# prs-eth/PCAccumulation

Hardware: AMD Instinct MI355X
Metric: LiDAR-frames/sec (5-frame seq, 160k pts) fwd+bwd (higher is better)
Workload: dtype mixed

## Files before the change

### include/pcacc.h

```cpp
#ifndef PCACC_H_
#define PCACC_H_

#include <stddef.h>
#include <stdint.h>

#ifdef __cplusplus
extern "C" {
#endif

#define PCACC_OK 0
#define PCACC_E_ARG (-1)
#define PCACC_E_WORKSPACE (-2)
#define PCACC_E_LAUNCH (-3)

#define PCACC_F32 0
#define PCACC_BF16 1

const char *pcacc_target(void);

int pcacc_cat2_rows(const void *a, int32_t a_row_bytes, const void *b, int32_t b_row_bytes, int64_t rows, void *out, void *stream);

int pcacc_reload_switches(void);

int pcacc_voxelize_workspace_bytes(int64_t n, int nx, int ny, int nz, int nt, size_t *bytes );
// ... 204 lines not shown
#define PCACC_ACCUM_TOO_SMALL 1
#define PCACC_ACCUM_BAD_STATE 2
int pcacc_accum_add_workspace_bytes(int64_t n, size_t *bytes );
int pcacc_accum_add(const float *points, int64_t n, const double *pose, const uint8_t *moving, int32_t stamp, double voxel_size,
                    const int64_t *in_keys, const int64_t *in_acc, const int32_t *in_stamps, int64_t in_capacity,
                    int64_t *out_keys, int64_t *out_acc, int32_t *out_stamps, int64_t out_capacity,
                    int64_t *state, void *workspace, size_t workspace_bytes, void *stream);
int pcacc_accum_extract_workspace_bytes(int64_t m, size_t *bytes );
int pcacc_accum_extract(const int64_t *keys, const int64_t *acc, const int32_t *stamps, int64_t capacity, int64_t m, int64_t min_count,
                        int32_t use_fraction, double max_moving_fraction, float *out_points, int32_t *out_coords, int64_t *out_count,
                        int64_t *out_moving, int32_t *out_t_first, int32_t *out_t_last, int64_t *out_n,
                        void *workspace, size_t workspace_bytes, void *stream);

int pcacc_conv3x3_prepare_weights(const float *w, int32_t c_out, int32_t c_in, int32_t kt, int32_t transpose,
                                  uint16_t *out, void *stream);
int pcacc_conv3x3_prepare_weights_pair(const float *w, int32_t c_out, int32_t c_in, int32_t kt, const int64_t *strides ,
                                       uint16_t *out_fwd, uint16_t *out_bwd, void *stream);
int pcacc_conv3x3_bf16(const uint16_t *in, const uint16_t *wp, const float *bias, uint16_t *out, int32_t n_img,
                       int32_t frames, int32_t h, int32_t w, int32_t c_in, int32_t c_out, int32_t kt, int32_t relu,
                       void *stream);
int pcacc_conv3x3_deep_supported(int32_t h, int32_t w, int32_t c_in, int32_t c_out);
int pcacc_conv3x3_deep_bf16(const uint16_t *in, const uint16_t *in_mask, const uint16_t *wp, const float *bias, uint16_t *out, int32_t n_img,
                            int32_t h, int32_t w, int32_t c_in, int32_t c_out, int32_t relu, void *stream);
int pcacc_conv3x3_masked_bf16(const uint16_t *in, const uint16_t *in_mask, const uint16_t *wp, const float *bias, uint16_t *out,
                              int32_t n_img, int32_t frames, int32_t h, int32_t w, int32_t c_in, int32_t c_out, int32_t kt,
                              int32_t relu, void *stream);
int pcacc_conv3x3_outmask_supported(int32_t h, int32_t w, int32_t c_in, int32_t c_out, int32_t kt);
int pcacc_conv3x3_outmask_bf16(const uint16_t *in, const uint16_t *wp, const uint16_t *out_mask, uint16_t *out, int32_t n_img, int32_t frames,
                               int32_t h, int32_t w, int32_t c_in, int32_t c_out, int32_t kt, void *stream);
int pcacc_conv3x3_wgrad_deep_supported(int32_t h, int32_t w, int32_t c_in, int32_t c_out);
int pcacc_conv3x3_wgrad_deep_workspace_bytes(int32_t n_img, int32_t h, int32_t w, int32_t c_in, int32_t c_out, size_t *bytes );
int pcacc_conv3x3_wgrad_deep_bf16(const uint16_t *dy, const uint16_t *dy_mask, const uint16_t *x, float *dw, float *db, int32_t n_img,
                                  int32_t h, int32_t w, int32_t c_in, int32_t c_out, void *workspace, size_t workspace_bytes, void *stream);
int pcacc_absmax256(const float *x, int64_t n, float *parts, void *stream);
int pcacc_conv3x3_split_prepare_weights(const float *w, int32_t c_out, int32_t c_in, int32_t kt, const int64_t *strides ,
                                        uint16_t *out_fwd, float *scale_fwd, uint16_t *out_bwd, float *scale_bwd, void *stream);
int pcacc_conv3x3_split_supported(int32_t h, int32_t w, int32_t c_in, int32_t c_out);
int pcacc_conv3x3_split(const float *in, const float *in_amax, const float *in_mask, const uint16_t *wp, const float *wscale,
                        const float *bias, float *out, float *out_amax, int32_t n_img, int32_t frames, int32_t h, int32_t w, int32_t c_in,
                        int32_t c_out, int32_t kt, int32_t relu, void *stream);
int pcacc_conv3x3_split_dual(const float *in, const float *in_amax, const float *in_mask, const uint16_t *wp, const float *wscale,
                             const float *bias, float *out, float *out_amax, uint16_t *out16, int32_t n_img, int32_t frames, int32_t h,
                             int32_t w, int32_t c_in, int32_t c_out, int32_t kt, int32_t relu, void *stream);

int pcacc_conv3x3_split_cat(const float *in_a, const float *in_b, int32_t c_a, const float *in_amax, const uint16_t *wp, const float *wscale,
                            const float *bias, float *out, float *out_amax, uint16_t *out16, int32_t n_img, int32_t h, int32_t w, int32_t c_in,
                            int32_t c_out, int32_t relu, void *stream);
int pcacc_conv3x3_split_outmask(const float *in, const float *in_amax, const float *in_mask, const uint16_t *wp, const float *wscale,
                                const float *out_mask, float *out, float *out_amax, int32_t n_img, int32_t frames, int32_t h, int32_t w,
                                int32_t c_in, int32_t c_out, int32_t kt, void *stream);
int pcacc_conv3x3_wgrad_split_workspace_bytes(int32_t n_img, int32_t h, int32_t w, int32_t c_in, int32_t c_out, size_t *bytes );
int pcacc_conv3x3_wgrad_split(const float *dy, const float *dy_amax, const float *dy_mask, const float *x, const float *x_amax, float *dw,
                              float *db, int32_t n_img, int32_t frames, int32_t dt, int32_t h, int32_t w, int32_t c_in, int32_t c_out,
                              void *workspace, size_t workspace_bytes, void *stream);
int pcacc_upconv2x2_split_prepare_weights(const float *w, int32_t c_in, int32_t c_up, const int64_t *strides , uint16_t *out_fwd,
                                          float *scale_fwd, uint16_t *out_bwd, float *scale_bwd, void *stream);
int pcacc_upconv2x2_split_supported(int32_t h, int32_t w, int32_t c_in, int32_t c_up);

int pcacc_upconv2x2_bf16_supported(int32_t c_in, int32_t c_up);
int pcacc_upconv2x2_bf16_prepare_weights(const float *w, int32_t c_in, int32_t c_up, const int64_t *strides , uint16_t *out_fwd,
                                         uint16_t *out_bwd, void *stream);
int pcacc_upconv2x2_bf16(const uint16_t *in, const uint16_t *wp, const float *bias, uint16_t *out, int32_t n_img, int32_t h, int32_t w,
                         int32_t c_in, int32_t c_up, int32_t direction, int32_t in_pitch, int32_t out_pitch, void *stream);
int pcacc_upconv2x2_bf16_wgrad_workspace_bytes(int32_t n_img, int32_t h, int32_t w, int32_t c_in, int32_t c_up, size_t *bytes);
int pcacc_upconv2x2_bf16_wgrad(const uint16_t *dy, int32_t dy_pitch, const uint16_t *x, int32_t x_pitch, float *dw, const int64_t *dw_strides ,
                               float *db, int32_t n_img, int32_t h, int32_t w, int32_t c_in, int32_t c_up, void *workspace, size_t workspace_bytes,
                               void *stream);

int pcacc_prepare_weights_batch(const int64_t *jobs, int32_t n_jobs, int32_t total_blocks, void *stream);
int pcacc_upconv2x2_split(const float *in, const float *in_amax, const uint16_t *wp, const float *wscale, const float *bias, float *out,
                          float *out_amax, int32_t n_img, int32_t h, int32_t w, int32_t c_in, int32_t c_up, int32_t direction, void *stream);
int pcacc_upconv2x2_split_dual(const float *in, const float *in_amax, const uint16_t *wp, const float *wscale, const float *bias, float *out,
                               float *out_amax, uint16_t *out16, int32_t n_img, int32_t h, int32_t w, int32_t c_in, int32_t c_up,
                               int32_t out_pitch, void *stream);
int pcacc_upconv2x2_wgrad_split_workspace_bytes(int32_t n_img, int32_t h, int32_t w, int32_t c_in, int32_t c_up, size_t *bytes );
int pcacc_upconv2x2_wgrad_split(const float *dy, const float *dy_amax, const float *x, const float *x_amax, float *dw, float *db4, int32_t n_img,
                                int32_t h, int32_t w, int32_t c_in, int32_t c_up, void *workspace, size_t workspace_bytes, void *stream);
int pcacc_head_conv3x3_supported(int32_t c_in, int32_t c_out);
int pcacc_head_conv3x3_forward(const void *x, int32_t x_dtype, const float *w, const int64_t *w_strides , const float *bias, float *y,
                               int32_t n_img, int32_t h, int32_t wd, int32_t c_in, int32_t c_out, void *stream);
int pcacc_head_conv3x3_dgrad(const float *dy, const float *w, const int64_t *w_strides , void *dx, int32_t dx_dtype, int32_t n_img,
                             int32_t h, int32_t wd, int32_t c_in, int32_t c_out, void *stream);
int pcacc_head_conv3x3_wgrad_workspace_bytes(int32_t n_img, int32_t h, int32_t wd, int32_t c_in, int32_t c_out, size_t *bytes );
int pcacc_head_conv3x3_wgrad(const float *dy, const void *x, int32_t x_dtype, float *dw, float *db, int32_t n_img, int32_t h, int32_t wd,
                             int32_t c_in, int32_t c_out, void *workspace, size_t workspace_bytes, void *stream);
int pcacc_rows_linear_split(const float *x, const float *x_amax, const float *in_mask, const float *w, const float *bias,
                            const float *residual, const float *out_mask, float *y, float *y_amax, int64_t rows, int32_t k, int32_t n,
                            int32_t flags, void *stream);
int pcacc_rows_linear_split_dual(const float *x, const float *x_amax, const float *in_mask, const float *w, const float *bias,
                                 const float *residual, const float *out_mask, float *y, uint16_t *y16, float *y_amax, int64_t rows, int32_t k,
                                 int32_t n, int32_t flags, void *stream);
int pcacc_rows_linear_cat_split(const float *xa, const float *xa_amax, const float *xb, const float *xb_amax, const int32_t *b_index,
                                int32_t ka, const float *in_mask, const float *w, const float *bias, const float *residual,
                                const float *out_mask_a, const float *out_mask_b, float *y, float *y2, int32_t na, float *y_amax, int64_t rows,
                                int32_t k, int32_t n, int32_t flags, void *stream);
int pcacc_rows_wgrad_split_workspace_bytes(int64_t rows, int32_t k, int32_t n, size_t *bytes );
int pcacc_rows_wgrad_split(const float *dy, const float *dy_amax, const float *dy_mask, const float *x, const float *x_amax, int32_t x_relu,
                           int64_t rows, int32_t k, int32_t n, float *dw_aug, void *workspace, size_t workspace_bytes, void *stream);
int pcacc_rows_wgrad_cat_split(const float *dy, const float *dy_amax, const float *dy_mask, const float *xa, const float *xa_amax,
                               const float *xb, const float *xb_amax, const int32_t *b_index, int32_t ka, int32_t x_relu, int64_t rows,
                               int32_t k, int32_t n, float *dw_aug, void *workspace, size_t workspace_bytes, void *stream);
int pcacc_conv3x3_wgrad_workspace_bytes(int32_t n_img, int32_t h, int32_t w, int32_t c_in, int32_t c_out, size_t *bytes );
int pcacc_conv3x3_wgrad_bf16(const uint16_t *dy, const uint16_t *x, float *dw, int32_t n_img, int32_t frames, int32_t dt,
                             int32_t h, int32_t w, int32_t c_in, int32_t c_out, void *workspace, size_t workspace_bytes,
                             void *stream);

int pcacc_prep_points(const double *points, const double *tsfm12, const double *noise, double noise_scale, double scale,
                      double crop_xy, double z_min, double z_max, int32_t remove_ground, double ground_z, int64_t m,
                      double *out_points, uint8_t *keep, void *stream);

int pcacc_seg_loss_workspace_bytes(int64_t n, size_t *bytes );
int pcacc_seg_loss_forward(const void *logits, int logits_dtype, int64_t plane, const int64_t *labels, const int64_t *rows,
                           int64_t n, float *out_loss, double *out_metric, float *lovasz_grad, float *saved,
                           void *workspace, size_t workspace_bytes, void *stream);
int pcacc_seg_loss_backward(const void *logits, int logits_dtype, int64_t plane, const int64_t *labels, const int64_t *rows,
                            int64_t n, int64_t n_total, const float *lovasz_grad, const float *saved, const float *grad_bce,
                            const float *grad_lovasz, void *grad_logits, void *stream);

int pcacc_offset_loss_workspace_bytes(int64_t m, int64_t k, size_t *bytes );
int pcacc_offset_loss_forward(const float *points, const int64_t *time_indice, const int64_t *inst_labels,
                              const int64_t *label_base, const float *ego_motion, const float *inst_motion, int32_t n_frames,
                              int64_t n, int64_t k, const float *transformed_points, const float *offset_est,
                              const int64_t *rows, int64_t m, float *out, float *offset_gt, void *workspace,
                              size_t workspace_bytes, void *stream);
int pcacc_offset_loss_backward(const float *offset_gt, const float *offset_est, const int64_t *rows, int64_t m, int64_t n,
                               const float *grad_norm, const float *grad_dir, float *grad_est, void *stream);

int pcacc_frames_max(const void *x, int dtype, int64_t n_seq, int32_t frames, int64_t plane, void *out, uint8_t *arg, void *stream);
int pcacc_frames_max_backward(const void *grad_out, const uint8_t *arg, int dtype, int64_t n_seq, int32_t frames, int64_t plane,
                              void *grad_x, void *stream);

int pcacc_bn_rows_workspace_bytes(int64_t rows, int32_t c, size_t *bytes );
int pcacc_bn_rows_forward(const void *x, int dtype, int64_t rows, int32_t c, const float *gamma, const float *beta, float eps,
                          float momentum, float *running_mean, float *running_var, void *y, float *save_mean,
                          float *save_invstd, void *workspace, size_t workspace_bytes, void *stream);
int pcacc_bn_rows_backward(const void *grad_y, const void *x, int dtype, int64_t rows, int32_t c, const float *gamma,
                           const float *save_mean, const float *save_invstd, void *grad_x, float *grad_gamma, float *grad_beta,
                           void *workspace, size_t workspace_bytes, void *stream);

int pcacc_bn_relu_rows_forward(const void *x, int dtype, int64_t rows, int32_t c, const float *gamma, const float *beta, float eps,
                               float momentum, float *running_mean, float *running_var, void *y, float *save_mean, float *save_invstd,
                               void *workspace, size_t workspace_bytes, void *stream);
int pcacc_bn_relu_rows_backward(const void *grad_y, const void *x, int dtype, int64_t rows, int32_t c, const float *gamma, const float *beta,
                                const float *save_mean, const float *save_invstd, void *grad_x, float *grad_gamma, float *grad_beta,
                                void *workspace, size_t workspace_bytes, void *stream);
int pcacc_bn_rows_forward_dual(const float *x, int64_t rows, int32_t c, const float *gamma, const float *beta, float eps, float momentum,
                               float *running_mean, float *running_var, int32_t relu, float *y, uint16_t *y16, float *y_amax, float *save_mean,
                               float *save_invstd, void *workspace, size_t workspace_bytes, void *stream);

int pcacc_bn_rows_backward_m(const void *grad_y, const void *x, int dtype, int64_t rows, int32_t c, const float *gamma, const float *beta,
                             int32_t relu, const float *save_mean, const float *save_invstd, void *grad_x, float *grad_x_amax, float *grad_gamma,
                             float *grad_beta, void *workspace, size_t workspace_bytes, void *stream);

int pcacc_pfn_block_forward(const uint16_t *xa, const uint16_t *pooled, const int32_t *p2v, const float *w0, const float *b0,
                            const float *ws, const float *w1, const float *b1, uint16_t *out, uint16_t *relu_h, int64_t rows, void *stream);
int pcacc_pfn_block_backward_workspace_bytes(int64_t rows, size_t *bytes );
int pcacc_pfn_block_backward(const uint16_t *xa, const uint16_t *pooled, const int32_t *p2v, const uint16_t *relu_h,
                             const uint16_t *grad_out, const float *w0, const float *ws, const float *w1, uint16_t *grad_xa,
                             uint16_t *grad_xb, float *grad_params, int64_t rows, void *workspace, size_t workspace_bytes, void *stream);

int pcacc_pfn_block_split_forward(const float *xa, const float *xa_amax, const float *pooled, const float *pooled_amax, const int32_t *p2v,
                                  const float *w0, const float *b0, const float *ws, const float *w1, const float *b1, float *out,
                                  float *relu_h, uint64_t *xmask, uint32_t *hmask, float *out_amax, float *hr_amax, int64_t rows,
                                  void *stream);
int pcacc_pfn_block_split_forward_dual(const float *xa, const float *xa_amax, const float *pooled, const float *pooled_amax, const int32_t *p2v,
                                       const float *w0, const float *b0, const float *ws, const float *w1, const float *b1, float *out,
                                       uint16_t *out16, uint16_t *hr16, float *out_amax, int64_t rows, void *stream);
int pcacc_pfn_block_split_dgrad(const float *grad_out, const float *grad_out_amax, const uint64_t *xmask, const uint32_t *hmask,
                                const float *w0, const float *ws, const float *w1, float *grad_xa, float *grad_xb, float *grad_h,
                                float *gx_amax, float *dh_amax, int64_t rows, void *stream);

int pcacc_maxpool2x2_bf16(const uint16_t *x, int64_t n_img, int32_t h, int32_t w, int32_t c, uint16_t *out, void *stream);
int pcacc_pool_skip_relu_backward_bf16(const uint16_t *y, const uint16_t *grad_pooled, const uint16_t *grad_skip, int64_t n_img, int32_t h,
                                       int32_t w, int32_t c, uint16_t *grad_y, void *stream);
int pcacc_maxpool2x2_f32(const float *x, int64_t n_img, int32_t h, int32_t w, int32_t c, float *out, void *stream);
int pcacc_pool_skip_relu_backward_f32(const float *y, const float *grad_pooled, const float *grad_skip, int64_t n_img, int32_t h, int32_t w,
                                      int32_t c, float *grad_y, float *out_amax, void *stream);
int pcacc_pool_skip_relu_backward_strided_bf16(const uint16_t *y, const uint16_t *grad_pooled, const uint16_t *grad_skip, int64_t skip_pitch,
                                               int64_t n_img, int32_t h, int32_t w, int32_t c, uint16_t *grad_y, void *stream);
int pcacc_pool_skip_relu_backward_strided_f32(const float *y, const float *grad_pooled, const float *grad_skip, int64_t skip_pitch,
                                              int64_t n_img, int32_t h, int32_t w, int32_t c, float *grad_y, float *out_amax, void *stream);
int pcacc_pool_skip_relu_backward_strided_y32(const float *y, const uint16_t *grad_pooled, const uint16_t *grad_skip, int64_t skip_pitch,
                                              int64_t n_img, int32_t h, int32_t w, int32_t c, uint16_t *grad_y, void *stream);

int pcacc_inv4x4(const float *m, int64_t n, float *out, void *stream);

int pcacc_rows_wgrad_few_supported(int32_t k, int32_t n);
int pcacc_rows_wgrad_few_workspace_bytes(int64_t rows, int32_t k, int32_t n, size_t *bytes );
int pcacc_rows_wgrad_few(const void *dy, const void *dy_mask, const void *x, int32_t x_relu, int64_t rows, int32_t k, int32_t n,
                         float *dw_aug, int32_t dtypes, void *workspace, size_t workspace_bytes, void *stream);

int pcacc_tube_rows(const float *xyz, const int32_t *slot, const float *slot_centre, int64_t n, int32_t n_frames, float *rows, void *stream);
int pcacc_tube_code(const float *geo, const float *motion, const float *frame, int64_t n_inst, int32_t n_frames, int32_t c, float *code,
                    void *stream);
int pcacc_tube_code_backward(const float *grad_code, int64_t n_inst, int32_t n_frames, int32_t c, float *grad_geo, float *grad_motion,
                             float *grad_frame, void *stream);
int pcacc_tube_pose_forward(const float *pose_vec, const float *remaining, const float *total_in, const float *slot_centre,
                            const float *weights, int32_t n_slots, int32_t n_frames, float *pose_c, float *gt_c, float *step,
                            float *remaining_out, float *total_out, double *loss_rt, float *wsum, void *stream);
int pcacc_tube_gap_forward(const float *rows, const int32_t *slot, const float *pose_c, const float *gt_c, int64_t n, float *pp, void *stream);
int pcacc_tube_finish(const float *slot_sums, int32_t stride, const float *count, const float *weights, const float *wsum, int32_t n_slots,
                      float *l12, void *stream);
int pcacc_tube_gap_backward(const float *rows, const int32_t *slot, const float *pose_c, const float *gt_c, const float *weights,
                            const float *count, const float *wsum, const float *grad_l1, const float *grad_l2, int64_t n,
                            float *grad_rows16, void *stream);
int pcacc_tube_pose_backward(const float *pose_vec, const float *remaining, const float *slot_centre, const float *weights, const float *wsum,
                             const float *grad_pose, int32_t stride, const double *grad_rot, const double *grad_trans, int32_t n_slots,
                             int32_t n_frames, float *grad_vec, void *stream);

int pcacc_upload_words(const uint32_t *host_words, int64_t n, uint32_t *dst, void *stream);

#ifdef __cplusplus
}
#endif
#endif
```

### pcaccumulation_amd/csrc/bn.hip

```cpp
#include "common.h"

#define BN_MAX_C 256

template <bool BF>
__device__ __forceinline__ void bn_load(const void *p, int64_t vec_index, float (&v)[BF ? 8 : 4])
{
    if (BF) {
        const uint4 r = reinterpret_cast<const uint4 *>(p)[vec_index];
        v[0] = pcacc_bf16_lo(r.x), v[1] = pcacc_bf16_hi(r.x), v[2] = pcacc_bf16_lo(r.y), v[3] = pcacc_bf16_hi(r.y);
        v[(BF ? 8 : 4) - 4] = pcacc_bf16_lo(r.z), v[(BF ? 8 : 4) - 3] = pcacc_bf16_hi(r.z);
        v[(BF ? 8 : 4) - 2] = pcacc_bf16_lo(r.w), v[(BF ? 8 : 4) - 1] = pcacc_bf16_hi(r.w);
    } else {
        const float4 r = reinterpret_cast<const float4 *>(p)[vec_index];
        v[0] = r.x, v[1] = r.y, v[2] = r.z, v[3] = r.w;
    }
}

template <bool BF>
__device__ __forceinline__ void bn_store(void *p, int64_t vec_index, const float (&v)[BF ? 8 : 4])
{
    if (BF)
        reinterpret_cast<uint4 *>(p)[vec_index] = make_uint4(pcacc_pack_bf16x2(v[0], v[1]), pcacc_pack_bf16x2(v[2], v[3]),
                                                             pcacc_pack_bf16x2(v[(BF ? 8 : 4) - 4], v[(BF ? 8 : 4) - 3]),
                                                             pcacc_pack_bf16x2(v[(BF ? 8 : 4) - 2], v[(BF ? 8 : 4) - 1]));
// ... 142 lines not shown
        rsh[k] = ((relu && relu_beta) ? relu_beta[sub * V + k] : 0.f) - mean[sub * V + k] * is_[k] * g;
    }
    for (int64_t e = (int64_t)blockIdx.x * 256 + threadIdx.x; e < total; e += (int64_t)gridDim.x * 256) {
        float x[V], o[V];
        bn_load<BF>(X, e, x);
        if (!DY) {
#pragma unroll
            for (int k = 0; k < V; ++k) o[k] = x[k] * scale[k] + shift[k];
            if (relu) {
#pragma unroll
                for (int k = 0; k < V; ++k) o[k] = fmaxf(o[k], 0.f);
            }
        } else {
            float g[V];
            bn_load<BF>(DY, e, g);
            if (relu) {
#pragma unroll
                for (int k = 0; k < V; ++k) g[k] = (x[k] * rsc[k] + rsh[k] > 0.f) ? g[k] : 0.f;
            }
#pragma unroll
            for (int k = 0; k < V; ++k) o[k] = g[k] * scale[k] + (x[k] * is_[k] - mis[k]) * kx[k] + shift[k];
        }
        bn_store<BF>(out, e, o);
        if (!BF && out16) reinterpret_cast<uint2 *>(out16)[e] = make_uint2(pcacc_pack_bf16x2(o[0], o[1]), pcacc_pack_bf16x2(o[2], o[3]));
        if (out_amax) {
#pragma unroll
            for (int k = 0; k < V; ++k) {
                omax = fmaxf(omax, fabsf(o[k]));
                if (o[k] != o[k]) omax = __builtin_inff();
            }
        }
    }
    if (out_amax) {
#pragma unroll
        for (int d = 32; d >= 1; d >>= 1) omax = fmaxf(omax, __shfl_xor(omax, d, 64));
        if ((threadIdx.x & 63) == 0) atomicMax(reinterpret_cast<unsigned *>(out_amax) + ((blockIdx.x * 4 + (threadIdx.x >> 6)) & 255), __float_as_uint(omax));
    }
}

static int bn_blocks(int64_t rows, int c, int v)
{
    const int rows_per_pass = 256 / (c / v);
    int64_t nb = (rows + (int64_t)rows_per_pass * 8 - 1) / ((int64_t)rows_per_pass * 8);
    if (nb > PCACC_CUS * 4) nb = PCACC_CUS * 4;
    return nb < 1 ? 1 : (int)nb;
}

static int bn_args(int dtype, int64_t rows, int c)
{
    if (dtype != PCACC_F32 && dtype != PCACC_BF16) return PCACC_E_ARG;
    const int v = dtype == PCACC_BF16 ? 8 : 4;
    if (rows < 1 || c < v || c > BN_MAX_C || c % v || 256 % (c / v)) return PCACC_E_ARG;
    return PCACC_OK;
}

extern "C" int pcacc_bn_rows_workspace_bytes(int64_t rows, int32_t c, size_t *bytes)
{
    if (!bytes || rows < 1 || c < 4 || c > BN_MAX_C) return PCACC_E_ARG;
    *bytes = (size_t)PCACC_CUS * 4 * 2 * c * sizeof(float);
    return PCACC_OK;
}

static int bn_forward_any(const void *x, int dtype, int64_t rows, int32_t c, const float *gamma, const float *beta, float eps,
                          float momentum, float *running_mean, float *running_var, void *y, float *save_mean,
                          float *save_invstd, void *workspace, size_t workspace_bytes, void *stream, bool relu, uint16_t *y16 = nullptr,
                          float *y_amax = nullptr)
{
    if ((y16 || y_amax) && dtype != PCACC_F32) return PCACC_E_ARG;
    if (bn_args(dtype, rows, c) != PCACC_OK || !x || !y || !save_mean || !save_invstd || !workspace) return PCACC_E_ARG;
    const bool bf = dtype == PCACC_BF16;
    const int nb = bn_blocks(rows, c, bf ? 8 : 4);
    if (workspace_bytes < (size_t)nb * 2 * c * sizeof(float)) return PCACC_E_WORKSPACE;
    hipStream_t s = pcacc_stream(stream);
    float *partial = reinterpret_cast<float *>(workspace);
    if (bf) bn_sums_kernel<true><<<nb, 256, 0, s>>>(x, nullptr, nullptr, nullptr, rows, c, partial);
    else bn_sums_kernel<false><<<nb, 256, 0, s>>>(x, nullptr, nullptr, nullptr, rows, c, partial);
    bn_finalize_fwd_kernel<<<c, 256, 0, s>>>(partial, nb, c, rows, eps, momentum, running_mean, running_var, save_mean, save_invstd);
    const int grid = pcacc_grid(rows * (c / (bf ? 8 : 4)), 256, PCACC_CUS * 16);
    if (bf) bn_apply_kernel<true><<<grid, 256, 0, s>>>(x, nullptr, save_mean, save_invstd, gamma, beta, nullptr, rows, c, y, relu);
    else bn_apply_kernel<false><<<grid, 256, 0, s>>>(x, nullptr, save_mean, save_invstd, gamma, beta, nullptr, rows, c, y, relu, nullptr, y_amax, y16);
    PCACC_CHECK_LAUNCH();
    return PCACC_OK;
}

extern "C" int pcacc_bn_rows_forward_dual(const float *x, int64_t rows, int32_t c, const float *gamma, const float *beta, float eps, float momentum,
                                          float *running_mean, float *running_var, int32_t relu, float *y, uint16_t *y16, float *y_amax,
                                          float *save_mean, float *save_invstd, void *workspace, size_t workspace_bytes, void *stream)
{
    return bn_forward_any(x, PCACC_F32, rows, c, gamma, beta, eps, momentum, running_mean, running_var, y, save_mean, save_invstd, workspace,
                          workspace_bytes, stream, relu != 0, y16, y_amax);
}

extern "C" int pcacc_bn_rows_forward(const void *x, int dtype, int64_t rows, int32_t c, const float *gamma, const float *beta, float eps,
                                     float momentum, float *running_mean, float *running_var, void *y, float *save_mean,
                                     float *save_invstd, void *workspace, size_t workspace_bytes, void *stream)
{
    return bn_forward_any(x, dtype, rows, c, gamma, beta, eps, momentum, running_mean, running_var, y, save_mean, save_invstd, workspace,
                          workspace_bytes, stream, false);
}

extern "C" int pcacc_bn_relu_rows_forward(const void *x, int dtype, int64_t rows, int32_t c, const float *gamma, const float *beta, float eps,
                                          float momentum, float *running_mean, float *running_var, void *y, float *save_mean,
                                          float *save_invstd, void *workspace, size_t workspace_bytes, void *stream)
{
    return bn_forward_any(x, dtype, rows, c, gamma, beta, eps, momentum, running_mean, running_var, y, save_mean, save_invstd, workspace,
                          workspace_bytes, stream, true);
}

static int bn_backward_any(const void *grad_y, const void *x, int dtype, int64_t rows, int32_t c, const float *gamma,
                           const float *save_mean, const float *save_invstd, void *grad_x, float *grad_gamma, float *grad_beta,
                           void *workspace, size_t workspace_bytes, void *stream, bool relu, const float *beta, float *grad_x_amax = nullptr)
{
    if (bn_args(dtype, rows, c) != PCACC_OK || !grad_y || !x || !save_mean || !save_invstd || !grad_x || !grad_gamma || !grad_beta || !workspace)
        return PCACC_E_ARG;
    const bool bf = dtype == PCACC_BF16;
    const int nb = bn_blocks(rows, c, bf ? 8 : 4);
    if (workspace_bytes < (size_t)nb * 2 * c * sizeof(float)) return PCACC_E_WORKSPACE;
    hipStream_t s = pcacc_stream(stream);
    float *partial = reinterpret_cast<float *>(workspace);
    if (bf) bn_sums_kernel<true><<<nb, 256, 0, s>>>(grad_y, x, save_mean, save_invstd, rows, c, partial, relu, gamma, beta);
    else bn_sums_kernel<false><<<nb, 256, 0, s>>>(grad_y, x, save_mean, save_invstd, rows, c, partial, relu, gamma, beta);
    bn_finalize_bwd_kernel<<<c, 256, 0, s>>>(partial, nb, c, grad_beta, grad_gamma);
    const int grid = pcacc_grid(rows * (c / (bf ? 8 : 4)), 256, PCACC_CUS * 16);
    if (bf) bn_apply_kernel<true><<<grid, 256, 0, s>>>(x, grad_y, save_mean, save_invstd, gamma, grad_beta, grad_gamma, rows, c, grad_x, relu, beta, grad_x_amax);
    else bn_apply_kernel<false><<<grid, 256, 0, s>>>(x, grad_y, save_mean, save_invstd, gamma, grad_beta, grad_gamma, rows, c, grad_x, relu, beta, grad_x_amax);
    PCACC_CHECK_LAUNCH();
    return PCACC_OK;
}

extern "C" int pcacc_bn_rows_backward_m(const void *grad_y, const void *x, int dtype, int64_t rows, int32_t c, const float *gamma, const float *beta,
                                        int32_t relu, const float *save_mean, const float *save_invstd, void *grad_x, float *grad_x_amax,
                                        float *grad_gamma, float *grad_beta, void *workspace, size_t workspace_bytes, void *stream)
{
    if (!grad_x_amax) return PCACC_E_ARG;
    return bn_backward_any(grad_y, x, dtype, rows, c, gamma, save_mean, save_invstd, grad_x, grad_gamma, grad_beta, workspace, workspace_bytes, stream,
                           relu != 0, relu ? beta : nullptr, grad_x_amax);
}

extern "C" int pcacc_bn_rows_backward(const void *grad_y, const void *x, int dtype, int64_t rows, int32_t c, const float *gamma,
                                      const float *save_mean, const float *save_invstd, void *grad_x, float *grad_gamma, float *grad_beta,
                                      void *workspace, size_t workspace_bytes, void *stream)
{
    return bn_backward_any(grad_y, x, dtype, rows, c, gamma, save_mean, save_invstd, grad_x, grad_gamma, grad_beta, workspace, workspace_bytes, stream,
                           false, nullptr);
}

extern "C" int pcacc_bn_relu_rows_backward(const void *grad_y, const void *x, int dtype, int64_t rows, int32_t c, const float *gamma,
                                           const float *beta, const float *save_mean, const float *save_invstd, void *grad_x, float *grad_gamma,
                                           float *grad_beta, void *workspace, size_t workspace_bytes, void *stream)
{
    return bn_backward_any(grad_y, x, dtype, rows, c, gamma, save_mean, save_invstd, grad_x, grad_gamma, grad_beta, workspace, workspace_bytes, stream,
                           true, beta);
}
```

### pcaccumulation_amd/csrc/canvas.hip

```cpp
#include <hip/hip_ext.h>

#include "scan.h"

template <typename T>
__global__ __launch_bounds__(256) void cell_index_kernel(const T *__restrict__ coords, int64_t m, int nx, int ny, int nt,
                                                         int64_t n_cells, int32_t *__restrict__ cell, int32_t *cell2pillar)
{
    for (int64_t i = (int64_t)blockIdx.x * 256 + threadIdx.x; i < m; i += (int64_t)gridDim.x * 256) {
        const int64_t b = (int64_t)coords[i * 5 + 0];
        const int64_t y = (int64_t)coords[i * 5 + 2];
        const int64_t x = (int64_t)coords[i * 5 + 3];
        const int64_t t = (int64_t)coords[i * 5 + 4];
        const int64_t c = ((b * nt + t) * ny + y) * nx + x;
        const bool ok = c >= 0 && c < n_cells && x >= 0 && x < nx && y >= 0 && y < ny && t >= 0 && t < nt;
        cell[i] = ok ? (int32_t)c : -1;
        if (ok) atomicMax(&cell2pillar[c], (int32_t)i);
    }
}

extern "C" int pcacc_cell_index(const void *coords, int coords_is_f64, int64_t m, int nx, int ny, int nt, int n_batch,
                                int32_t *cell, int32_t *cell2pillar, void *stream)
{
    if (m < 0 || nx <= 0 || ny <= 0 || nt <= 0 || n_batch <= 0 || !cell2pillar) return PCACC_E_ARG;
    const int64_t n_cells = (int64_t)n_batch * nt * ny * nx;
// ... 247 lines not shown
}

template <int OUT_BF16>
__global__ __launch_bounds__(256) void pillar_scatter_scalar(const float *__restrict__ feats, const int32_t *__restrict__ c2p,
                                                             int64_t n_elems, int c, void *__restrict__ canvas)
{
    for (int64_t e = (int64_t)blockIdx.x * 256 + threadIdx.x; e < n_elems; e += (int64_t)gridDim.x * 256) {
        const int64_t cell = e / c;
        const int k = (int)(e - cell * c);
        const int p = c2p[cell];
        const float v = (p >= 0) ? feats[(int64_t)p * c + k] : 0.f;
        if (OUT_BF16) static_cast<uint16_t *>(canvas)[e] = f32_to_bf16(v);
        else static_cast<float *>(canvas)[e] = v;
    }
}

static int pillar_scatter_launch(const void *feats, int feats_dtype, const int32_t *cell2pillar, int64_t n_cells, int c, void *canvas,
                                 int dtype, hipEvent_t start, hipEvent_t stop, hipStream_t s)
{
    if (n_cells < 0 || c <= 0 || !cell2pillar || !canvas || (dtype != PCACC_F32 && dtype != PCACC_BF16)) return PCACC_E_ARG;
    if (feats_dtype != PCACC_F32 && !(feats_dtype == PCACC_BF16 && dtype == PCACC_BF16 && c % 8 == 0)) return PCACC_E_ARG;
    if (n_cells == 0) return PCACC_OK;
    int64_t n;
    int width, per_lane = 1;
    const void *fn;
    if (feats_dtype == PCACC_BF16) {
        width = c / 8;
        n = n_cells * width;
        fn = reinterpret_cast<const void *>(pillar_scatter_rows16_k<1, true>);
        per_lane = 1;
        switch (pcacc_switches().scatter_variant) {
        case '0': fn = reinterpret_cast<const void *>(pillar_scatter_rows16); per_lane = 2; break;
        case '1': fn = reinterpret_cast<const void *>(pillar_scatter_rows16_k<4, true>); per_lane = 4; break;
        case '2': fn = reinterpret_cast<const void *>(pillar_scatter_rows16_k<2, true>); per_lane = 2; break;
        case '3': fn = reinterpret_cast<const void *>(pillar_scatter_rows16_k<4, false>); per_lane = 4; break;
        case '4': fn = reinterpret_cast<const void *>(pillar_scatter_rows16_k<8, true>); per_lane = 8; break;
        case '5': fn = reinterpret_cast<const void *>(pillar_scatter_rows16_k<1, true>); per_lane = 1; break;
        case '6': fn = reinterpret_cast<const void *>(pillar_scatter_rows16_k<1, true, false>); per_lane = 1; break;
        case '7': fn = reinterpret_cast<const void *>(pillar_scatter_rows16_k<2, true, false>); per_lane = 2; break;
        default: break;
        }
    } else if (dtype == PCACC_F32 ? (c % 4 == 0) : (c % 8 == 0)) {
        width = c / 4;
        n = dtype == PCACC_F32 ? n_cells * width : n_cells * (width / 2);
        fn = dtype == PCACC_F32 ? reinterpret_cast<const void *>(pillar_scatter_vec4<0>) : reinterpret_cast<const void *>(pillar_scatter_vec4<1>);
        if (dtype == PCACC_F32 && pcacc_switches().scatter_variant == 'f')
            fn = reinterpret_cast<const void *>(pillar_scatter_f32_nt);
    } else {
        width = c;
        n = n_cells * c;
        fn = dtype == PCACC_F32 ? reinterpret_cast<const void *>(pillar_scatter_scalar<0>) : reinterpret_cast<const void *>(pillar_scatter_scalar<1>);
    }
    void *args[] = {(void *)&feats, (void *)&cell2pillar, (void *)&n, (void *)&width, (void *)&canvas};
    const int64_t items = (n + per_lane - 1) / per_lane;
    const int blocks_per_cu = pcacc_switches().scatter_blocks > 0 ? pcacc_switches().scatter_blocks : 8;
    if (hipExtLaunchKernel(fn, dim3(pcacc_grid(items, 256, PCACC_CUS * blocks_per_cu)), dim3(256), args, 0, s, start, stop, 0) != hipSuccess) return PCACC_E_LAUNCH;
    PCACC_CHECK_LAUNCH();
    return PCACC_OK;
}

extern "C" int pcacc_pillar_scatter(const float *feats, const int32_t *cell2pillar, int64_t n_cells, int c,
                                    void *canvas, int dtype, void *stream)
{
    return pillar_scatter_launch(feats, PCACC_F32, cell2pillar, n_cells, c, canvas, dtype, nullptr, nullptr, pcacc_stream(stream));
}

extern "C" int pcacc_pillar_scatter_timed(const float *feats, const int32_t *cell2pillar, int64_t n_cells, int c, void *canvas, int dtype,
                                          void *start_event, void *stop_event, void *stream)
{
    if (!start_event || !stop_event) return PCACC_E_ARG;
    return pillar_scatter_launch(feats, PCACC_F32, cell2pillar, n_cells, c, canvas, dtype, reinterpret_cast<hipEvent_t>(start_event),
                                 reinterpret_cast<hipEvent_t>(stop_event), pcacc_stream(stream));
}

extern "C" int pcacc_pillar_scatter_t(const void *feats, int feats_dtype, const int32_t *cell2pillar, int64_t n_cells, int c, void *canvas,
                                      int dtype, void *start_event, void *stop_event, void *stream)
{
    if ((start_event == nullptr) != (stop_event == nullptr)) return PCACC_E_ARG;
    return pillar_scatter_launch(feats, feats_dtype, cell2pillar, n_cells, c, canvas, dtype, reinterpret_cast<hipEvent_t>(start_event),
                                 reinterpret_cast<hipEvent_t>(stop_event), pcacc_stream(stream));
}

extern "C" int pcacc_timer_create(void **start_event, void **stop_event)
{
    if (!start_event || !stop_event) return PCACC_E_ARG;
    hipEvent_t a, b;
    if (hipEventCreate(&a) != hipSuccess) return PCACC_E_LAUNCH;
    if (hipEventCreate(&b) != hipSuccess) { (void)hipEventDestroy(a); return PCACC_E_LAUNCH; }
    *start_event = a;
    *stop_event = b;
    return PCACC_OK;
}

extern "C" int pcacc_timer_elapsed_us(void *start_event, void *stop_event, float *us)
{
    if (!start_event || !stop_event || !us) return PCACC_E_ARG;
    float ms = 0.f;
    if (hipEventElapsedTime(&ms, reinterpret_cast<hipEvent_t>(start_event), reinterpret_cast<hipEvent_t>(stop_event)) != hipSuccess)
        return PCACC_E_LAUNCH;
    *us = ms * 1e3f;
    return PCACC_OK;
}

extern "C" int pcacc_timer_destroy(void *start_event, void *stop_event)
{
    if (start_event) (void)hipEventDestroy(reinterpret_cast<hipEvent_t>(start_event));
    if (stop_event) (void)hipEventDestroy(reinterpret_cast<hipEvent_t>(stop_event));
    return PCACC_OK;
}

__global__ __launch_bounds__(256) void gather_rows_kernel(const uint32_t *__restrict__ src, int words, const int32_t *__restrict__ idx,
                                                          int64_t n_idx, uint32_t *__restrict__ out)
{
    const int64_t total = n_idx * words;
    for (int64_t e = (int64_t)blockIdx.x * 256 + threadIdx.x; e < total; e += (int64_t)gridDim.x * 256) {
        const int64_t r = e / words;
        const int k = (int)(e - r * words);
        const int64_t j = idx[r];
        out[e] = (j >= 0) ? src[j * words + k] : 0u;
    }
}

__global__ __launch_bounds__(256) void gather_rows_kernel16(const uint4 *__restrict__ src, int pieces, const int32_t *__restrict__ idx,
                                                            int64_t n_idx, uint4 *__restrict__ out)
{
    const int64_t total = n_idx * pieces;
    for (int64_t e = (int64_t)blockIdx.x * 256 + threadIdx.x; e < total; e += (int64_t)gridDim.x * 256) {
        const int64_t r = e / pieces;
        const int k = (int)(e - r * pieces);
        const int64_t j = idx[r];
        out[e] = (j >= 0) ? src[j * pieces + k] : make_uint4(0u, 0u, 0u, 0u);
    }
}

extern "C" int pcacc_gather_rows(const void *src, int row_bytes, const int32_t *idx, int64_t n_idx, void *out, void *stream)
{
    if (n_idx < 0 || row_bytes <= 0 || (row_bytes % 4)) return PCACC_E_ARG;
    if (n_idx > 0 && (!src || !idx || !out)) return PCACC_E_ARG;
    if (n_idx == 0) return PCACC_OK;
    hipStream_t s = pcacc_stream(stream);
    if (row_bytes % 16 == 0 && (reinterpret_cast<uintptr_t>(src) % 16 == 0) && (reinterpret_cast<uintptr_t>(out) % 16 == 0)) {
        const int pieces = row_bytes / 16;
        gather_rows_kernel16<<<pcacc_grid(n_idx * pieces, 256), 256, 0, s>>>(static_cast<const uint4 *>(src), pieces, idx, n_idx,
                                                                            static_cast<uint4 *>(out));
    } else {
        const int words = row_bytes / 4;
        gather_rows_kernel<<<pcacc_grid(n_idx * words, 256), 256, 0, s>>>(static_cast<const uint32_t *>(src), words, idx, n_idx,
                                                                         static_cast<uint32_t *>(out));
    }
    PCACC_CHECK_LAUNCH();
    return PCACC_OK;
}

__global__ __launch_bounds__(256) void cat2_rows_kernel(const uint4 *__restrict__ a, int pa, const uint4 *__restrict__ b, int pb, int64_t rows,
                                                        uint4 *__restrict__ out)
{
    const int pr = pa + pb;
    const int64_t total = rows * pr, stride = (int64_t)gridDim.x * 256;
    for (int64_t e = (int64_t)blockIdx.x * 256 + threadIdx.x; e < total; e += 2 * stride) {
        const int64_t e2 = e + stride;
        const int64_t r0 = e / pr, r1 = e2 / pr;
        const int c0 = (int)(e - r0 * pr), c1 = (int)(e2 - r1 * pr);
        const uint4 v0 = c0 < pa ? a[r0 * pa + c0] : b[r0 * pb + (c0 - pa)];
        uint4 v1 = make_uint4(0, 0, 0, 0);
        if (e2 < total) v1 = c1 < pa ? a[r1 * pa + c1] : b[r1 * pb + (c1 - pa)];
        out[e] = v0;
        if (e2 < total) out[e2] = v1;
    }
}

extern "C" int pcacc_cat2_rows(const void *a, int32_t a_row_bytes, const void *b, int32_t b_row_bytes, int64_t rows, void *out, void *stream)
{
    if (rows < 0 || a_row_bytes <= 0 || b_row_bytes <= 0 || (a_row_bytes % 16) || (b_row_bytes % 16)) return PCACC_E_ARG;
    if (rows == 0) return PCACC_OK;
    if (!a || !b || !out || (reinterpret_cast<uintptr_t>(a) % 16) || (reinterpret_cast<uintptr_t>(b) % 16) || (reinterpret_cast<uintptr_t>(out) % 16)) return PCACC_E_ARG;
    const int pa = a_row_bytes / 16, pb = b_row_bytes / 16;
    const int64_t total = rows * (pa + pb);
    cat2_rows_kernel<<<pcacc_grid((total + 1) / 2, 256, PCACC_CUS * 16), 256, 0, pcacc_stream(stream)>>>(static_cast<const uint4 *>(a), pa, static_cast<const uint4 *>(b), pb,
                                                                                                         rows, static_cast<uint4 *>(out));
    PCACC_CHECK_LAUNCH();
    return PCACC_OK;
}

extern "C" const char *pcacc_target(void) { return "gfx950"; }

static PcaccSwitches g_switches;
static bool g_switches_read = false;

static void switches_read()
{
    const char *e = getenv("PCACC_CONV_RES");
    g_switches.conv_frame_major = getenv("PCACC_CONV_FRAME_MAJOR") != nullptr;
    g_switches.conv_swz_off = getenv("PCACC_CONV_SWZ_OFF") != nullptr;
    g_switches.rows_fm_off = getenv("PCACC_ROWS_FM_OFF") != nullptr;
    g_switches.conv_plan = getenv("PCACC_CONV_PLAN") != nullptr;
    g_switches.conv_res = e ? e[0] : 0;
    const char *xr = getenv("PCACC_XCD_REMAP");
    g_switches.xcd_off = xr && xr[0] == '0';
    const char *v = getenv("PCACC_SCATTER_VARIANT");
    g_switches.scatter_variant = v ? v[0] : 0;
    const char *b = getenv("PCACC_SCATTER_BLOCKS");
    g_switches.scatter_blocks = b ? atoi(b) : 0;
    g_switches_read = true;
}

const PcaccSwitches &pcacc_switches()
{
    if (!g_switches_read) switches_read();
    return g_switches;
}

extern "C" int pcacc_reload_switches(void)
{
    switches_read();
    return 0;
}

struct UploadWords { uint32_t w[240]; };

__global__ void upload_words_kernel(UploadWords words, int n, uint32_t *dst)
{
    if ((int)threadIdx.x < n) dst[threadIdx.x] = words.w[threadIdx.x];
}

extern "C" int pcacc_upload_words(const uint32_t *host_words, int64_t n, uint32_t *dst, void *stream)
{
    if (n < 0 || (n > 0 && (!host_words || !dst))) return PCACC_E_ARG;
    for (int64_t off = 0; off < n; off += 240) {
        UploadWords words;
        const int m = (int)((n - off) < 240 ? (n - off) : 240);
        for (int i = 0; i < m; ++i) words.w[i] = host_words[off + i];
        upload_words_kernel<<<1, 256, 0, pcacc_stream(stream)>>>(words, m, dst + off);
    }
    PCACC_CHECK_LAUNCH();
    return PCACC_OK;
}

__global__ __launch_bounds__(256) void prep_points_kernel(const double *__restrict__ pts, const double *__restrict__ tsfm,
                                                          const double *__restrict__ noise, double noise_scale, double scale,
                                                          double crop_xy, double z_min, double z_max, int remove_ground, double ground_z,
                                                          int64_t m, double *__restrict__ out, uint8_t *__restrict__ keep)
{
#pragma clang fp contract(off)
    for (int64_t i = (int64_t)blockIdx.x * 256 + threadIdx.x; i < m; i += (int64_t)gridDim.x * 256) {
        double x = pts[3 * i], y = pts[3 * i + 1], z = pts[3 * i + 2];
        if (tsfm) {
            const double nx = fma(tsfm[2], z, fma(tsfm[1], y, tsfm[0] * x)) + tsfm[9];
            const double ny = fma(tsfm[5], z, fma(tsfm[4], y, tsfm[3] * x)) + tsfm[10];
            const double nz = fma(tsfm[8], z, fma(tsfm[7], y, tsfm[6] * x)) + tsfm[11];
            x = nx; y = ny; z = nz;
        }
        if (noise) {
            x = x + (noise[3 * i] - 0.5) * noise_scale;
            y = y + (noise[3 * i + 1] - 0.5) * noise_scale;
            z = z + (noise[3 * i + 2] - 0.5) * noise_scale;
        }
        if (tsfm || noise) { x = x * scale; y = y * scale; z = z * scale; }
        out[3 * i] = x; out[3 * i + 1] = y; out[3 * i + 2] = z;
        bool k = fabs(x) < crop_xy && fabs(y) < crop_xy && z < z_max && z > z_min;
        if (remove_ground) k = k && z > ground_z;
        keep[i] = k ? 1 : 0;
    }
}

extern "C" int pcacc_prep_points(const double *points, const double *tsfm12, const double *noise, double noise_scale, double scale,
                                 double crop_xy, double z_min, double z_max, int32_t remove_ground, double ground_z, int64_t m,
                                 double *out_points, uint8_t *keep, void *stream)
{
    if (m < 0) return PCACC_E_ARG;
    if (m == 0) return PCACC_OK;
    if (!points || !out_points || !keep) return PCACC_E_ARG;
    prep_points_kernel<<<pcacc_grid(m, 256), 256, 0, pcacc_stream(stream)>>>(points, tsfm12, noise, noise_scale, scale, crop_xy, z_min,
                                                                            z_max, remove_ground, ground_z, m, out_points, keep);
    PCACC_CHECK_LAUNCH();
    return PCACC_OK;
}

template <bool BF>
__global__ __launch_bounds__(256) void frames_max_kernel(const void *__restrict__ x, int64_t n_seq, int frames, int64_t plane_vec,
                                                         void *__restrict__ out, uint8_t *__restrict__ arg)
{
    constexpr int V = BF ? 8 : 4;
    const int64_t total = n_seq * plane_vec;
    for (int64_t e = (int64_t)blockIdx.x * 256 + threadIdx.x; e < total; e += (int64_t)gridDim.x * 256) {
        const int64_t s = e / plane_vec, p = e - s * plane_vec;
        float best[V];
        uint8_t who[V];
        for (int t = 0; t < frames; ++t) {
            const uint4 raw = reinterpret_cast<const uint4 *>(x)[(s * frames + t) * plane_vec + p];
            float v[V];
            if (BF) {
                v[0] = pcacc_bf16_lo(raw.x), v[1] = pcacc_bf16_hi(raw.x), v[2] = pcacc_bf16_lo(raw.y), v[3] = pcacc_bf16_hi(raw.y);
                v[V - 4] = pcacc_bf16_lo(raw.z), v[V - 3] = pcacc_bf16_hi(raw.z), v[V - 2] = pcacc_bf16_lo(raw.w), v[V - 1] = pcacc_bf16_hi(raw.w);
            } else {
                v[0] = __uint_as_float(raw.x), v[1] = __uint_as_float(raw.y), v[2] = __uint_as_float(raw.z), v[3] = __uint_as_float(raw.w);
            }
#pragma unroll
            for (int k = 0; k < V; ++k) {
                const bool take = t == 0 || v[k] > best[k] || (v[k] != v[k] && best[k] == best[k]);
                best[k] = take ? v[k] : best[k];
                who[k] = take ? (uint8_t)t : who[k];
            }
        }
        if (BF) {
            reinterpret_cast<uint4 *>(out)[e] = make_uint4(pcacc_pack_bf16x2(best[0], best[1]), pcacc_pack_bf16x2(best[2], best[3]),
                                                           pcacc_pack_bf16x2(best[V - 4], best[V - 3]), pcacc_pack_bf16x2(best[V - 2], best[V - 1]));
// ... 77 lines not shown
```

### pcaccumulation_amd/csrc/common.h

```cpp
#pragma once
#include <hip/hip_runtime.h>
#include <stdint.h>

#include "../../include/pcacc.h"

#define PCACC_WAVE 64
#define PCACC_CUS 256

#define PCACC_CHECK_LAUNCH()                                   \
    do {                                                       \
        if (hipGetLastError() != hipSuccess) return PCACC_E_LAUNCH; \
    } while (0)

struct PcaccSwitches {
    bool conv_frame_major;
    bool conv_swz_off;
    bool rows_fm_off;
    bool conv_plan;
    char conv_res;
    bool xcd_off;
    char scatter_variant;
    int scatter_blocks;
};
const PcaccSwitches &pcacc_switches();

static inline hipStream_t pcacc_stream(void *s) { return reinterpret_cast<hipStream_t>(s); }

static inline int pcacc_grid(int64_t work_items, int block, int max_blocks = PCACC_CUS * 8)
{
    int64_t b = (work_items + block - 1) / block;
    if (b < 1) b = 1;
    if (b > max_blocks) b = max_blocks;
    return (int)b;
}

static inline size_t pcacc_align(size_t x, size_t a = 256) { return (x + a - 1) / a * a; }

__device__ __forceinline__ int pcacc_xcd_block(int b, int n)
{
    const int per = (n + 7) >> 3, rem = n & 7, x = b & 7, i = b >> 3;
    return (rem == 0 || x < rem) ? x * per + i : rem * per + (x - rem) * (per - 1) + i;
}

__device__ __forceinline__ float bf16_to_f32(uint16_t h) { return __uint_as_float(((uint32_t)h) << 16); }
__device__ __forceinline__ uint16_t f32_to_bf16(float f)
{
    uint32_t u = __float_as_uint(f);
    if ((u & 0x7fffffffu) > 0x7f800000u) return (uint16_t)((u >> 16) | 0x40);
    u += 0x7fffu + ((u >> 16) & 1u);
    return (uint16_t)(u >> 16);
}

typedef __bf16 pcacc_bf16x2 __attribute__((ext_vector_type(2)));
typedef float pcacc_f32x2 __attribute__((ext_vector_type(2)));
__device__ __forceinline__ uint32_t pcacc_pack_bf16x2(float lo, float hi)
{
    const pcacc_f32x2 f = {lo, hi};
    const pcacc_bf16x2 r = __builtin_convertvector(f, pcacc_bf16x2);
    return *reinterpret_cast<const uint32_t *>(&r);
}
__device__ __forceinline__ float pcacc_bf16_lo(uint32_t v) { return __uint_as_float(v << 16); }
__device__ __forceinline__ float pcacc_bf16_hi(uint32_t v) { return __uint_as_float(v & 0xffff0000u); }
__device__ __forceinline__ float4 pcacc_ld4(const void *p, bool bf16, int64_t i4)
{
    if (!bf16) return reinterpret_cast<const float4 *>(p)[i4];
    const uint2 v = reinterpret_cast<const uint2 *>(p)[i4];
    return make_float4(pcacc_bf16_lo(v.x), pcacc_bf16_hi(v.x), pcacc_bf16_lo(v.y), pcacc_bf16_hi(v.y));
}
__device__ __forceinline__ void pcacc_st4(void *p, bool bf16, int64_t i4, float4 v)
{
    if (!bf16) reinterpret_cast<float4 *>(p)[i4] = v;
    else reinterpret_cast<uint2 *>(p)[i4] = make_uint2(pcacc_pack_bf16x2(v.x, v.y), pcacc_pack_bf16x2(v.z, v.w));
}

__device__ __forceinline__ uint32_t pcacc_relu_mask2(uint32_t g, uint32_t y)
{
    const uint32_t lo = ((int32_t)(y << 16) > 0) ? 0x0000ffffu : 0u;
    const uint32_t hi = ((int32_t)(y & 0xffff0000u) > 0) ? 0xffff0000u : 0u;
    return g & (lo | hi);
}
__device__ __forceinline__ uint4 pcacc_relu_mask8(uint4 g, uint4 y)
{
    return make_uint4(pcacc_relu_mask2(g.x, y.x), pcacc_relu_mask2(g.y, y.y), pcacc_relu_mask2(g.z, y.z), pcacc_relu_mask2(g.w, y.w));
}

__host__ __device__ constexpr int pcacc_tr_stride(int c)
{
    return c == 32 ? 32 : (c == 64 ? 96 : (c == 96 ? 96 : (c == 128 ? 160 : c + 4)));
}

#ifdef PCACC_X3_EXPERIMENT
__device__ __forceinline__ float pcacc_x_round_bf16(float v) { return bf16_to_f32(f32_to_bf16(v)); }
__device__ __forceinline__ bool pcacc_x_apply(int f, float &a, float &b)
{
    if (f & 4) { a = pcacc_x_round_bf16(a); b = pcacc_x_round_bf16(b); }
    return (f & 5) != 0;
}
#define PCACC_X_ACT(word) ((word) & 5)
#define PCACC_X_W(word) (((word) >> 1) & 5)
#endif

__device__ __forceinline__ int lane_id() { return threadIdx.x & 63; }

template <int EL, class Store>
__device__ __forceinline__ void pcacc_reduce_partials(const float *__restrict__ partial, int n_parts, int elems, Store store)
{
    constexpr int SL = 1024 / EL;
    __shared__ float red[SL][EL + 1];
    const int el = threadIdx.x % EL, slice = threadIdx.x / EL;
    const int e = blockIdx.x * EL + el;
    float s0 = 0.f, s1 = 0.f, s2 = 0.f, s3 = 0.f;
    if (e < elems) {
        int p = slice;
        for (; p + 3 * SL < n_parts; p += 4 * SL) {
            s0 += partial[(int64_t)p * elems + e];
            s1 += partial[(int64_t)(p + SL) * elems + e];
            s2 += partial[(int64_t)(p + 2 * SL) * elems + e];
            s3 += partial[(int64_t)(p + 3 * SL) * elems + e];
        }
        for (; p < n_parts; p += SL) s0 += partial[(int64_t)p * elems + e];
    }
    red[slice][el] = (s0 + s1) + (s2 + s3);
    __syncthreads();
    if (slice == 0 && e < elems) {
        float v = 0.f;
#pragma unroll 8
        for (int k = 0; k < SL; ++k) v += red[k][el];
        store(e, v);
    }
}
static inline int pcacc_reduce_el(int elems) { return elems >= 8192 ? 64 : 16; }

__device__ __forceinline__ int wave_inclusive_scan(int v)
{
#pragma unroll
    for (int d = 1; d < 64; d <<= 1) {
        int t = __shfl_up(v, d, 64);
        if (lane_id() >= d) v += t;
    }
    return v;
}

__device__ __forceinline__ int block256_exclusive_scan(int v, int *lds, int *total)
{
    const int incl = wave_inclusive_scan(v);
    const int w = threadIdx.x >> 6;
    if (lane_id() == 63) lds[w] = incl;
    __syncthreads();
    int base = 0;
#pragma unroll
    for (int i = 0; i < 4; ++i) base += (i < w) ? lds[i] : 0;
    *total = lds[0] + lds[1] + lds[2] + lds[3];
    __syncthreads();
    return base + incl - v;
}

struct ConvTile { int img, fr, y0, x0; };
#define PCACC_WALK_OK(n_img, frames, tiles_y, tiles_x) ((n_img) < (1 << 24) && (frames) < 128 && (tiles_y) < 32768 && (tiles_x) < 65536)
struct ConvTileWalk {
    int first, stride, count;
    int tyx, tiles_x, frames, frame_fastest, th, tw;
    int v_if, v_yx;
    __device__ __forceinline__ void init(int lo, int hi, int slot, int slots, int tiles_y, int tiles_x_, int frames_, int ff, int th_, int tw_)
    {
        first = lo + slot; stride = slots; count = first < hi ? (hi - first + slots - 1) / slots : 0;
        tyx = tiles_y * tiles_x_; tiles_x = tiles_x_; frames = frames_; frame_fastest = ff; th = th_; tw = tw_;
        v_if = v_yx = 0;
    }
    __device__ __forceinline__ void refill(int k0)
    {
        const int t = first + (k0 + (int)(threadIdx.x & 63)) * stride;
        int img, pos, fr;
        if (frame_fastest) {
            const int q = t / frames, smp = q / tyx;
            fr = t - q * frames; pos = q - smp * tyx; img = smp * frames + fr;
        } else {
            img = t / tyx; pos = t - img * tyx; fr = frames > 1 ? img % frames : 0;
        }
        const int ty = pos / tiles_x;
// ... 13 lines not shown
```

### pcaccumulation_amd/csrc/head_conv.hip

```cpp
#include <type_traits>
#include "common.h"

#define HC_THREADS 256
#define HC_MAXCO 4

__device__ __forceinline__ float4 hc_ld4(const void *p, int bf16, int64_t i4) { return pcacc_ld4(p, bf16 != 0, i4); }

#define HC_TR 8
#define HC_TC 32
#define HC_PW (HC_TC + 2)
#define HC_PH (HC_TR + 2)

struct HcTile { int img, y0, x0; };
__device__ __forceinline__ HcTile hc_tile(int t, int tiles_y, int tiles_x)
{
    const int per_img = tiles_y * tiles_x, img = t / per_img, r = t - img * per_img;
    return HcTile{img, (r / tiles_x) * HC_TR, (r % tiles_x) * HC_TC};
}

template <int CI>
__device__ __forceinline__ void hc_stage(const void *__restrict__ x, int x_bf16, const HcTile &t, int h, int wd, float *patch)
{
    constexpr int LPP = CI / 4;
    for (int e = threadIdx.x; e < HC_PH * HC_PW * LPP; e += HC_THREADS) {
        const int pp = e / LPP, l4 = e - pp * LPP;
        const int py = pp / HC_PW, pxx = pp - py * HC_PW;
        const int y = t.y0 - 1 + py, xx = t.x0 - 1 + pxx;
        const bool ok = (unsigned)y < (unsigned)h && (unsigned)xx < (unsigned)wd;
        const int yc = min(max(y, 0), h - 1), xc = min(max(xx, 0), wd - 1);
        float4 v = hc_ld4(x, x_bf16, (((int64_t)t.img * h + yc) * wd + xc) * LPP + l4);
        if (!ok) v = make_float4(0.f, 0.f, 0.f, 0.f);
        *reinterpret_cast<float4 *>(patch + pp * CI + l4 * 4) = v;
    }
}

template <int CI, bool BF> struct HcRaw { typedef typename std::conditional<BF, uint2, float4>::type T; };
template <int CI> struct HcPieces { static constexpr int N = (HC_PH * HC_PW * (CI / 4) + HC_THREADS - 1) / HC_THREADS; };

template <int CI, bool BF>
__device__ __forceinline__ void hc_fetch(const void *__restrict__ x, const HcTile &t, int h, int wd, typename HcRaw<CI, BF>::T (&r)[HcPieces<CI>::N])
{
    constexpr int LPP = CI / 4;
    const typename HcRaw<CI, BF>::T *src = static_cast<const typename HcRaw<CI, BF>::T *>(x);
#pragma unroll
    for (int q = 0; q < HcPieces<CI>::N; ++q) {
        const int e = min((int)threadIdx.x + q * HC_THREADS, HC_PH * HC_PW * LPP - 1);
        const int pp = e / LPP, l4 = e - pp * LPP;
        const int py = pp / HC_PW, pxx = pp - py * HC_PW;
        const int yc = min(max(t.y0 - 1 + py, 0), h - 1), xc = min(max(t.x0 - 1 + pxx, 0), wd - 1);
        r[q] = src[(((int64_t)t.img * h + yc) * wd + xc) * LPP + l4];
    }
}

template <int CI, bool BF>
__device__ __forceinline__ void hc_put(const typename HcRaw<CI, BF>::T (&r)[HcPieces<CI>::N], const HcTile &t, int h, int wd, float *patch)
{
    constexpr int LPP = CI / 4;
#pragma unroll
    for (int q = 0; q < HcPieces<CI>::N; ++q) {
        const int e = threadIdx.x + q * HC_THREADS;
        if (e >= HC_PH * HC_PW * LPP) break;
        const int pp = e / LPP, l4 = e - pp * LPP;
        const int py = pp / HC_PW, pxx = pp - py * HC_PW;
        const int y = t.y0 - 1 + py, xx = t.x0 - 1 + pxx;
        const bool ok = (unsigned)y < (unsigned)h && (unsigned)xx < (unsigned)wd;
        float4 v;
        if constexpr (BF) v = make_float4(pcacc_bf16_lo(r[q].x), pcacc_bf16_hi(r[q].x), pcacc_bf16_lo(r[q].y), pcacc_bf16_hi(r[q].y));
        else v = r[q];
        if (!ok) v = make_float4(0.f, 0.f, 0.f, 0.f);
        *reinterpret_cast<float4 *>(patch + pp * CI + l4 * 4) = v;
    }
}

template <int CI, int COM, bool BF>
__global__ __launch_bounds__(HC_THREADS) void head_conv_fwd_kernel(const void *__restrict__ x, int x_bf16, const float *__restrict__ w,
                                                                   const float *__restrict__ bias, float *__restrict__ y, int n_img, int h,
                                                                   int wd, int co, int64_t ws_o, int64_t ws_i, int64_t ws_y, int64_t ws_x,
                                                                   int tiles_y, int tiles_x)
{
    constexpr int LPP = CI / 4, PPB = HC_THREADS / LPP;
    extern __shared__ __attribute__((aligned(16))) float hc_lds[];
    float *patch = hc_lds;
    const int l = threadIdx.x % LPP, slot = threadIdx.x / LPP;
    float4 wr[9][COM];
#pragma unroll
    for (int tap = 0; tap < 9; ++tap)
#pragma unroll
        for (int c = 0; c < COM; ++c) {
            const float *wp = w + c * ws_o + (4 * l) * ws_i + (tap / 3) * ws_y + (tap % 3) * ws_x;
            wr[tap][c] = c < co ? make_float4(wp[0], wp[ws_i], wp[2 * ws_i], wp[3 * ws_i]) : make_float4(0.f, 0.f, 0.f, 0.f);
        }
    const int n_tiles = n_img * tiles_y * tiles_x;
    constexpr bool PIPE = CI == 32;
    typename HcRaw<CI, BF>::T raw[HcPieces<CI>::N];
    if (PIPE && (int)blockIdx.x < n_tiles) hc_fetch<CI, BF>(x, hc_tile(blockIdx.x, tiles_y, tiles_x), h, wd, raw);
    for (int t = blockIdx.x; t < n_tiles; t += gridDim.x) {
        const HcTile tl = hc_tile(t, tiles_y, tiles_x);
        __syncthreads();
        if constexpr (PIPE) hc_put<CI, BF>(raw, tl, h, wd, patch); else hc_stage<CI>(x, x_bf16, tl, h, wd, patch);
        __syncthreads();
        if (PIPE && t + (int)gridDim.x < n_tiles) hc_fetch<CI, BF>(x, hc_tile(t + gridDim.x, tiles_y, tiles_x), h, wd, raw);
        for (int q = slot; q < HC_TR * HC_TC; q += PPB) {
            const int row = q / HC_TC, col = q % HC_TC;
            float acc[COM];
#pragma unroll
            for (int c = 0; c < COM; ++c) acc[c] = 0.f;
#pragma unroll
            for (int tap = 0; tap < 9; ++tap) {
                const float4 v = *reinterpret_cast<const float4 *>(patch + ((row + tap / 3) * HC_PW + col + tap % 3) * CI + 4 * l);
#pragma unroll
                for (int c = 0; c < COM; ++c) acc[c] += v.x * wr[tap][c].x + v.y * wr[tap][c].y + v.z * wr[tap][c].z + v.w * wr[tap][c].w;
            }
#pragma unroll
            for (int d = 1; d < LPP; d <<= 1)
#pragma unroll
                for (int c = 0; c < COM; ++c) acc[c] += __shfl_xor(acc[c], d, 64);
            const int yy = tl.y0 + row, xx = tl.x0 + col;
            if (l < co && yy < h && xx < wd) {
                float r = acc[0];
#pragma unroll
                for (int c = 1; c < COM; ++c) r = l == c ? acc[c] : r;
                y[(((int64_t)tl.img * h + yy) * wd + xx) * co + l] = r + (bias ? bias[l] : 0.f);
            }
        }
    }
}

template <int CI, int COM>
__global__ __launch_bounds__(HC_THREADS) void head_conv_dgrad_kernel(const float *__restrict__ dy, const float *__restrict__ w, void *__restrict__ dx,
                                                                     int dx_bf16, int n_img, int h, int wd, int co, int64_t ws_o, int64_t ws_i,
                                                                     int64_t ws_y, int64_t ws_x, int tiles_y, int tiles_x)
{
    constexpr int LPP = CI / 4, PPB = HC_THREADS / LPP;
    __shared__ float gp[HC_PH * HC_PW * COM];
    const int l = threadIdx.x % LPP, slot = threadIdx.x / LPP;
    float4 wr[9][COM];
#pragma unroll
    for (int tap = 0; tap < 9; ++tap)
#pragma unroll
        for (int c = 0; c < COM; ++c) {
            const float *wp = w + c * ws_o + (4 * l) * ws_i + (tap / 3) * ws_y + (tap % 3) * ws_x;
            wr[tap][c] = c < co ? make_float4(wp[0], wp[ws_i], wp[2 * ws_i], wp[3 * ws_i]) : make_float4(0.f, 0.f, 0.f, 0.f);
        }
    const int n_tiles = n_img * tiles_y * tiles_x;
    for (int t = blockIdx.x; t < n_tiles; t += gridDim.x) {
        const HcTile tl = hc_tile(t, tiles_y, tiles_x);
        __syncthreads();
        for (int e = threadIdx.x; e < HC_PH * HC_PW * COM; e += HC_THREADS) {
            const int pp = e / COM, c = e - pp * COM;
            const int py = pp / HC_PW, pxx = pp - py * HC_PW;
            const int y = tl.y0 - 1 + py, xx = tl.x0 - 1 + pxx;
            const bool ok = (unsigned)y < (unsigned)h && (unsigned)xx < (unsigned)wd && c < co;
            const int yc = min(max(y, 0), h - 1), xc = min(max(xx, 0), wd - 1);
            const float v = dy[(((int64_t)tl.img * h + yc) * wd + xc) * co + (c < co ? c : 0)];
            gp[e] = ok ? v : 0.f;
        }
        __syncthreads();
        for (int q = slot; q < HC_TR * HC_TC; q += PPB) {
            const int row = q / HC_TC, col = q % HC_TC;
            const int yy = tl.y0 + row, xx = tl.x0 + col;
            float4 acc = make_float4(0.f, 0.f, 0.f, 0.f);
#pragma unroll
            for (int tap = 0; tap < 9; ++tap) {
                const float *g = gp + ((row + 2 - tap / 3) * HC_PW + col + 2 - tap % 3) * COM;
#pragma unroll
                for (int c = 0; c < COM; ++c) {
                    const float gv = g[c];
                    acc.x += gv * wr[tap][c].x; acc.y += gv * wr[tap][c].y; acc.z += gv * wr[tap][c].z; acc.w += gv * wr[tap][c].w;
                }
            }
            if (yy < h && xx < wd) pcacc_st4(dx, dx_bf16 != 0, (((int64_t)tl.img * h + yy) * wd + xx) * LPP + l, acc);
        }
    }
}

template <int CI, int COM, bool BF>
__global__ __launch_bounds__(HC_THREADS) void head_conv_wgrad_kernel(const float *__restrict__ dy, const void *__restrict__ x, int x_bf16,
                                                                     float *__restrict__ partial, int n_img, int h, int wd, int co, int tiles_y,
                                                                     int tiles_x)
{
    constexpr int LPP = CI / 4, PPB = HC_THREADS / LPP;
    extern __shared__ __attribute__((aligned(16))) float hc_lds[];
    float *patch = hc_lds;
    constexpr int RED = 9 * COM * 4 + COM;
    static_assert(4 * LPP * RED <= HC_PH * HC_PW * CI, "reduction scratch fits the patch");
    const int l = threadIdx.x % LPP, slot = threadIdx.x / LPP, wave = threadIdx.x >> 6;
    float acc[9][COM][4], bs[COM];
#pragma unroll
    for (int c = 0; c < COM; ++c) bs[c] = 0.f;
#pragma unroll
    for (int t = 0; t < 9; ++t)
#pragma unroll
        for (int c = 0; c < COM; ++c)
#pragma unroll
            for (int q = 0; q < 4; ++q) acc[t][c][q] = 0.f;
    const int n_tiles = n_img * tiles_y * tiles_x;
    constexpr bool PIPE = CI == 32 && COM == 4;
    typename HcRaw<CI, BF>::T raw[HcPieces<CI>::N];
    if (PIPE && (int)blockIdx.x < n_tiles) hc_fetch<CI, BF>(x, hc_tile(blockIdx.x, tiles_y, tiles_x), h, wd, raw);
    for (int t = blockIdx.x; t < n_tiles; t += gridDim.x) {
        const HcTile tl = hc_tile(t, tiles_y, tiles_x);
        __syncthreads();
        if constexpr (PIPE) hc_put<CI, BF>(raw, tl, h, wd, patch); else hc_stage<CI>(x, x_bf16, tl, h, wd, patch);
        __syncthreads();
        if (PIPE && t + (int)gridDim.x < n_tiles) hc_fetch<CI, BF>(x, hc_tile(t + gridDim.x, tiles_y, tiles_x), h, wd, raw);
        auto dy_at = [&](int q) {
            const int yy = tl.y0 + q / HC_TC, xx = tl.x0 + q % HC_TC;
            return dy + (((int64_t)tl.img * h + min(yy, h - 1)) * wd + min(xx, wd - 1)) * co;
        };
#ifndef HC_DY_AHEAD
#define HC_DY_AHEAD 0
#endif
        constexpr bool AHEAD = COM == 2 && HC_DY_AHEAD;
        float2 g_next = make_float2(0.f, 0.f);
        if (AHEAD && co == 2) g_next = *reinterpret_cast<const float2 *>(dy_at(slot));
        for (int q = slot; q < HC_TR * HC_TC; q += PPB) {
            const int row = q / HC_TC, col = q % HC_TC;
            const int yy = tl.y0 + row, xx = tl.x0 + col;
            const bool ok = yy < h && xx < wd;
            const float *gp = dy_at(q);
            float g[COM];
            if (AHEAD && co == 2) {
                const float2 g2 = g_next;
                if (q + PPB < HC_TR * HC_TC) g_next = *reinterpret_cast<const float2 *>(dy_at(q + PPB));
                g[0] = ok ? g2.x : 0.f;
                g[1] = ok ? g2.y : 0.f;
            } else {
#pragma unroll
                for (int c = 0; c < COM; ++c) g[c] = (c < co && ok) ? gp[c < co ? c : 0] : 0.f;
            }
#pragma unroll
            for (int c = 0; c < COM; ++c) bs[c] += g[c];
#pragma unroll
            for (int tap = 0; tap < 9; ++tap) {
                const float4 v = *reinterpret_cast<const float4 *>(patch + ((row + tap / 3) * HC_PW + col + tap % 3) * CI + 4 * l);
#pragma unroll
                for (int c = 0; c < COM; ++c) {
                    acc[tap][c][0] += g[c] * v.x; acc[tap][c][1] += g[c] * v.y; acc[tap][c][2] += g[c] * v.z; acc[tap][c][3] += g[c] * v.w;
                }
            }
        }
    }
#pragma unroll
    for (int d = LPP; d < 64; d <<= 1) {
#pragma unroll
        for (int t = 0; t < 9; ++t)
#pragma unroll
            for (int c = 0; c < COM; ++c)
#pragma unroll
                for (int q = 0; q < 4; ++q) acc[t][c][q] += __shfl_xor(acc[t][c][q], d, 64);
#pragma unroll
        for (int c = 0; c < COM; ++c) bs[c] += __shfl_xor(bs[c], d, 64);
    }
    __syncthreads();
    float *red = patch;
    if ((threadIdx.x & 63) < LPP) {
        float *r = red + (wave * LPP + l) * RED;
#pragma unroll
        for (int t = 0; t < 9; ++t)
#pragma unroll
            for (int c = 0; c < COM; ++c)
#pragma unroll
                for (int q = 0; q < 4; ++q) r[(t * COM + c) * 4 + q] = acc[t][c][q];
#pragma unroll
        for (int c = 0; c < COM; ++c) r[9 * COM * 4 + c] = bs[c];
    }
    __syncthreads();
    float *mine = partial + (int64_t)blockIdx.x * (co * CI * 9 + co);
    for (int e = threadIdx.x; e < co * CI * 9; e += HC_THREADS) {
        const int tap = e % 9, ci = (e / 9) % CI, c = e / (9 * CI);
        float s = 0.f;
#pragma unroll
        for (int wv = 0; wv < HC_THREADS / 64; ++wv) s += red[(wv * LPP + ci / 4) * RED + (tap * COM + c) * 4 + (ci & 3)];
        mine[e] = s;
    }
    if (threadIdx.x < co) {
        float s = 0.f;
#pragma unroll
        for (int wv = 0; wv < HC_THREADS / 64; ++wv) s += red[(wv * LPP) * RED + 9 * COM * 4 + threadIdx.x];
        mine[co * CI * 9 + threadIdx.x] = s;
    }
}

__global__ __launch_bounds__(256) void head_conv_wgrad_reduce_kernel(const float *__restrict__ partial, int n_parts, int n_w, int co,
                                                                     float *__restrict__ dw, float *__restrict__ db)
{
    const int e = blockIdx.x * 64 + (threadIdx.x & 63), grp = threadIdx.x >> 6, elems = n_w + co;
    __shared__ float sm[4][64];
    float s0 = 0.f, s1 = 0.f;
    if (e < elems) {
        int p = grp;
        for (; p + 4 < n_parts; p += 8) {
            s0 += partial[(int64_t)p * elems + e];
            s1 += partial[(int64_t)(p + 4) * elems + e];
        }
        if (p < n_parts) s0 += partial[(int64_t)p * elems + e];
    }
    sm[grp][threadIdx.x & 63] = s0 + s1;
    __syncthreads();
    if (grp == 0 && e < elems) {
        const float t = (sm[0][threadIdx.x] + sm[1][threadIdx.x]) + (sm[2][threadIdx.x] + sm[3][threadIdx.x]);
        if (e < n_w) dw[e] = t;
        else if (db) db[e - n_w] = t;
    }
}

static bool hc_ok(int n_img, int h, int w, int c_in, int c_out)
{
    return n_img >= 1 && h >= 1 && w >= 1 && (int64_t)n_img * h * w < 0x7fffffffLL && (c_in == 32 || c_in == 64) && c_out >= 1 && c_out <= HC_MAXCO;
}

extern "C" int pcacc_head_conv3x3_supported(int32_t c_in, int32_t c_out) { return hc_ok(1, 1, 1, c_in, c_out) ? 1 : 0; }

extern "C" int pcacc_head_conv3x3_forward(const void *x, int32_t x_dtype, const float *w, const int64_t *w_strides, const float *bias, float *y,
                                          int32_t n_img, int32_t h, int32_t wd, int32_t c_in, int32_t c_out, void *stream)
{
    if (!x || !w || !w_strides || !y || !hc_ok(n_img, h, wd, c_in, c_out)) return PCACC_E_ARG;
    const int tiles_y = (h + HC_TR - 1) / HC_TR, tiles_x = (wd + HC_TC - 1) / HC_TC;
    const int64_t n_tiles = (int64_t)n_img * tiles_y * tiles_x;
    const int grid = (int)(n_tiles < PCACC_CUS * 6 ? n_tiles : PCACC_CUS * 6);
#define HC_FWD(CIV, COV)                                                                                                                        \
    do {                                                                                                                                        \
        const size_t lds = (size_t)(HC_PH * HC_PW * CIV) * sizeof(float);                                                       \
        auto kern = x_dtype ? head_conv_fwd_kernel<CIV, COV, true> : head_conv_fwd_kernel<CIV, COV, false>;                                     \
        if (hipFuncSetAttribute(reinterpret_cast<const void *>(kern), hipFuncAttributeMaxDynamicSharedMemorySize, (int)lds) != hipSuccess)     \
            return PCACC_E_LAUNCH;                                                                                                              \
        hipLaunchKernelGGL(kern, dim3(grid), dim3(HC_THREADS), lds, pcacc_stream(stream), x, x_dtype, w, bias, y, n_img, h, wd, c_out, w_strides[0], \
                           w_strides[1], w_strides[2], w_strides[3], tiles_y, tiles_x);                                                         \
    } while (0)
    if (c_in == 32 && c_out <= 2) HC_FWD(32, 2); else if (c_in == 32) HC_FWD(32, 4); else if (c_out <= 2) HC_FWD(64, 2); else HC_FWD(64, 4);
#undef HC_FWD
    PCACC_CHECK_LAUNCH();
    return PCACC_OK;
}

extern "C" int pcacc_head_conv3x3_dgrad(const float *dy, const float *w, const int64_t *w_strides, void *dx, int32_t dx_dtype, int32_t n_img, int32_t h,
                                        int32_t wd, int32_t c_in, int32_t c_out, void *stream)
{
    if (!dy || !w || !w_strides || !dx || !hc_ok(n_img, h, wd, c_in, c_out)) return PCACC_E_ARG;
    const int tiles_y = (h + HC_TR - 1) / HC_TR, tiles_x = (wd + HC_TC - 1) / HC_TC;
    const int64_t n_tiles = (int64_t)n_img * tiles_y * tiles_x;
    const int grid = (int)(n_tiles < PCACC_CUS * 8 ? n_tiles : PCACC_CUS * 8);
#define HC_DG(CIV, COV) hipLaunchKernelGGL((head_conv_dgrad_kernel<CIV, COV>), dim3(grid), dim3(HC_THREADS), 0, pcacc_stream(stream), dy, w, dx, dx_dtype, n_img, \
                                           h, wd, c_out, w_strides[0], w_strides[1], w_strides[2], w_strides[3], tiles_y, tiles_x)
    if (c_in == 32 && c_out <= 2) HC_DG(32, 2); else if (c_in == 32) HC_DG(32, 4); else if (c_out <= 2) HC_DG(64, 2); else HC_DG(64, 4);
#undef HC_DG
    PCACC_CHECK_LAUNCH();
    return PCACC_OK;
}

static int hc_wgrad_grid(int n_img, int h, int wd)
{
    const int64_t n_tiles = (int64_t)n_img * ((h + HC_TR - 1) / HC_TR) * ((wd + HC_TC - 1) / HC_TC);
    return (int)(n_tiles < PCACC_CUS * 3 ? n_tiles : PCACC_CUS * 3);
}

extern "C" int pcacc_head_conv3x3_wgrad_workspace_bytes(int32_t n_img, int32_t h, int32_t wd, int32_t c_in, int32_t c_out, size_t *bytes)
{
    if (!bytes || !hc_ok(n_img, h, wd, c_in, c_out)) return PCACC_E_ARG;
    *bytes = (size_t)hc_wgrad_grid(n_img, h, wd) * (c_out * c_in * 9 + c_out) * sizeof(float);
    return PCACC_OK;
}

extern "C" int pcacc_head_conv3x3_wgrad(const float *dy, const void *x, int32_t x_dtype, float *dw, float *db, int32_t n_img, int32_t h, int32_t wd,
                                        int32_t c_in, int32_t c_out, void *workspace, size_t workspace_bytes, void *stream)
{
    size_t need;
    if (!dy || !x || !dw || !workspace || pcacc_head_conv3x3_wgrad_workspace_bytes(n_img, h, wd, c_in, c_out, &need) != PCACC_OK) return PCACC_E_ARG;
    if (workspace_bytes < need) return PCACC_E_WORKSPACE;
    hipStream_t st = pcacc_stream(stream);
    const int grid = hc_wgrad_grid(n_img, h, wd);
    const int tiles_y = (h + HC_TR - 1) / HC_TR, tiles_x = (wd + HC_TC - 1) / HC_TC;
    float *partial = static_cast<float *>(workspace);
#define HC_WG(CIV, COV)                                                                                                                         \
    do {                                                                                                                                        \
        const size_t lds = (size_t)(HC_PH * HC_PW * CIV) * sizeof(float);                                                                       \
        auto kern = x_dtype ? head_conv_wgrad_kernel<CIV, COV, true> : head_conv_wgrad_kernel<CIV, COV, false>;                                 \
        if (hipFuncSetAttribute(reinterpret_cast<const void *>(kern), hipFuncAttributeMaxDynamicSharedMemorySize, (int)lds) != hipSuccess)     \
            return PCACC_E_LAUNCH;                                                                                                              \
        hipLaunchKernelGGL(kern, dim3(grid), dim3(HC_THREADS), lds, st, dy, x, x_dtype, partial, n_img, h, wd, c_out, tiles_y, tiles_x);        \
    } while (0)
    if (c_in == 32 && c_out <= 2) HC_WG(32, 2); else if (c_in == 32) HC_WG(32, 4); else if (c_out <= 2) HC_WG(64, 2); else HC_WG(64, 4);
#undef HC_WG
    const int n_w = c_out * c_in * 9;
    hipLaunchKernelGGL(head_conv_wgrad_reduce_kernel, dim3((n_w + c_out + 63) / 64), dim3(256), 0, st, partial, grid, n_w, c_out, dw, db);
    PCACC_CHECK_LAUNCH();
    return PCACC_OK;
}
```

### pcaccumulation_amd/native.py

```python
import ctypes
import os
import re

import torch

_HERE = os.path.dirname(os.path.abspath(__file__))
LIB_PATH = os.environ.get('PCACC_LIB') or os.path.join(_HERE, 'csrc', 'libpcacc_hip.so')

F32, BF16 = 0, 1
_ERR = {-1: 'PCACC_E_ARG', -2: 'PCACC_E_WORKSPACE', -3: 'PCACC_E_LAUNCH'}

_lib = None


class NativeError(RuntimeError):
    pass


_CTYPES = {'int': ctypes.c_int, 'int32_t': ctypes.c_int, 'int64_t': ctypes.c_int64, 'uint64_t': ctypes.c_uint64, 'size_t': ctypes.c_size_t,
           'float': ctypes.c_float, 'double': ctypes.c_double}


def _prototypes():
    text = re.sub(r'/\*.*?\*/', '', open(os.path.join(_HERE, os.pardir, 'include', 'pcacc.h')).read(), flags=re.S)
# ... 196 lines not shown
    offs = torch.empty((m + 1,), dtype=torch.int32, device=dev)
    order = torch.empty((n,), dtype=torch.int32, device=dev)
    ws = _workspace(lib().pcacc_csr_workspace_bytes, dev, n, m)
    _check(lib().pcacc_csr_build(_dev(p2v, torch.int32, 'p2v'), n, m, _dev(offs), _dev(order), _dev(ws), ws.numel(), _stream()), 'csr_build')
    return offs, order


def segment_mean3_maxlabel(points, labels, offs, order, m):
    dev = points.device
    mean = torch.empty((m, 3), dtype=torch.float32, device=dev)
    lab_out = torch.empty((m,), dtype=torch.int64, device=dev) if labels is not None else None
    _check(lib().pcacc_segment_mean3_maxlabel(
        _dev(points, torch.float32, 'points'), _dev(labels, torch.int64, 'labels') if labels is not None else None,
        _dev(offs, torch.int32), _dev(order, torch.int32), m, _dev(mean), _dev(lab_out) if lab_out is not None else None, _stream()), 'segment_mean3_maxlabel')
    return mean, lab_out


def _segment_ws(n, m, c, dev):
    return _workspace(lib().pcacc_segment_workspace_bytes, dev, n, m, int(c))


def _seg_two_level(n, m):
    return m > 0 and n // m > 16


def segment_max(src, offs, order, m):
    n, c = src.shape
    if src.dtype not in (torch.float32, torch.bfloat16):
        src = src.float()
    out_dtype = torch.float32 if _seg_two_level(n, m) else src.dtype
    out = torch.empty((m, c), dtype=out_dtype, device=src.device)
    arg = torch.empty((m, c), dtype=torch.int32, device=src.device)
    ws = _segment_ws(n, m, c, src.device)
    _check(lib().pcacc_segment_max_t(_dev(src, None, 'src'), _dtype_code(src), int(c), _dev(offs, torch.int32), _dev(order, torch.int32),
                                     n, m, _dev(out), _dev(arg), _dev(ws), ws.numel(), _stream()), 'segment_max')
    return out, arg


def segment_max_dual(src, offs, order, m):
    n, c = src.shape
    if _seg_two_level(n, m):
        raise NativeError('segment_max_dual: long segments (n / m > 16) have no second output')
    out = torch.empty((m, c), dtype=torch.float32, device=src.device)
    out16 = torch.empty((m, c), dtype=torch.bfloat16, device=src.device)
    arg = torch.empty((m, c), dtype=torch.int32, device=src.device)
    ws = _segment_ws(n, m, c, src.device)
    _check(lib().pcacc_segment_max_dual(_dev(src, torch.float32, 'src'), int(c), _dev(offs, torch.int32), _dev(order, torch.int32), n, m,
                                        _dev(out), _dev(out16), _dev(arg), _dev(ws), ws.numel(), _stream()), 'segment_max_dual')
    return out, out16, arg


def segment_max_backward(grad_out, arg, p2v, n, out_dtype=None):
    c = grad_out.shape[1]
    if grad_out.dtype not in (torch.float32, torch.bfloat16):
        grad_out = grad_out.float()
    out_dtype = out_dtype or grad_out.dtype
    g = torch.empty((n, c), dtype=out_dtype, device=grad_out.device)
    _check(lib().pcacc_segment_max_backward_t(_dev(grad_out, None, 'grad_out'), _dtype_code(grad_out), _dev(arg, torch.int32),
                                              _dev(p2v, torch.int32), n, int(c), _dev(g), _dtype_code(g), _stream()), 'segment_max_backward')
    return g


def segment_max_backward_acc(grad_out, arg, p2v, grad_src, want_amax=False):
    n, c = grad_src.shape
    if grad_out.dtype not in (torch.float32, torch.bfloat16):
        grad_out = grad_out.float()
    amax = _zero256(grad_src.device) if want_amax else None
    _check(lib().pcacc_segment_max_backward_acc(_dev(grad_out, None, 'grad_out'), _dtype_code(grad_out), _dev(arg, torch.int32), _dev(p2v, torch.int32),
                                                n, int(c), _dev(grad_src, None, 'grad_src'), _dtype_code(grad_src),
                                                _dev(amax) if want_amax else None, _stream()), 'segment_max_backward_acc')
    return amax


def segment_max_canvas(src, offs, order, m, cell2pillar):
    n, c = src.shape
    n_cells = cell2pillar.numel()
    dev = src.device
    canvas32 = torch.empty((n_cells, c), dtype=torch.float32, device=dev)
    canvas16 = torch.empty((n_cells, c), dtype=torch.bfloat16, device=dev)
    arg = torch.empty((m, c), dtype=torch.int32, device=dev)
    t = None
    if scatter_timer is not None and c >= 32:
        t = KernelTimer()
        scatter_timer.append((t, n_cells, c, m, 'fused', n))
    _check(lib().pcacc_segment_max_canvas(_dev(src, torch.float32, 'src'), int(c), _dev(offs, torch.int32), _dev(order, torch.int32), n, m,
                                          _dev(cell2pillar, torch.int32), n_cells, _dev(canvas32), _dev(canvas16), _dev(arg),
                                          t.start if t else None, t.stop if t else None, _stream()), 'segment_max_canvas')
    return canvas32, canvas16, arg


def segment_max_canvas_backward(grad_canvas, arg, p2v, cell, n, out_dtype=None):
    c = grad_canvas.shape[1]
    out_dtype = out_dtype or grad_canvas.dtype
    out = torch.empty((n, c), dtype=out_dtype, device=grad_canvas.device)
    _check(lib().pcacc_segment_max_canvas_backward(_dev(grad_canvas, None, 'grad_canvas'), _dtype_code(grad_canvas), _dev(arg, torch.int32), _dev(p2v, torch.int32),
                                                   _dev(cell, torch.int32), n, int(c), _dev(out), _dtype_code(out), _stream()), 'segment_max_canvas_backward')
    return out


def segment_sum(src, offs, order, m):
    n, c = src.shape
    if src.dtype not in (torch.float32, torch.bfloat16):
        src = src.float()
    out_dtype = torch.float32 if _seg_two_level(n, m) else src.dtype
    out = torch.empty((m, c), dtype=out_dtype, device=src.device)
    ws = _segment_ws(n, m, c, src.device)
    _check(lib().pcacc_segment_sum_t(_dev(src, None, 'src'), _dtype_code(src), int(c), _dev(offs, torch.int32), _dev(order, torch.int32),
                                     n, m, _dev(out), _dev(ws), ws.numel(), _stream()), 'segment_sum')
    return out


scatter_timer = None


class KernelTimer(object):

    def __init__(self):
        self.start, self.stop = ctypes.c_void_p(), ctypes.c_void_p()
        _check(lib().pcacc_timer_create(ctypes.byref(self.start), ctypes.byref(self.stop)), 'timer_create')

    def elapsed_us(self):
        us = ctypes.c_float(0.0)
        _check(lib().pcacc_timer_elapsed_us(self.start, self.stop, ctypes.byref(us)), 'timer_elapsed_us')
        return us.value

    def __del__(self):
        try:
            lib().pcacc_timer_destroy(self.start, self.stop)
        except Exception:
            pass


def pillar_scatter(feats, cell2pillar, out_dtype=torch.float32):
    c = feats.shape[1]
    n_cells = cell2pillar.numel()
    canvas = torch.empty((n_cells, c), dtype=out_dtype, device=feats.device)
    t = None
    if scatter_timer is not None and c >= 32:
        t = KernelTimer()
        scatter_timer.append((t, n_cells, c, feats.shape[0], out_dtype, feats.dtype))
    _check(lib().pcacc_pillar_scatter_t(_dev(feats, None, 'feats'), _dtype_code(feats), _dev(cell2pillar, torch.int32), n_cells,
                                        int(c), _dev(canvas), _dtype_code(canvas), t.start if t else None, t.stop if t else None, _stream()), 'pillar_scatter')
    return canvas


def cat2_rows(a, b):
    ca, cb = a.shape[-1], b.shape[-1]
    rows = a.numel() // ca
    if a.dtype != b.dtype or tuple(a.shape[:-1]) != tuple(b.shape[:-1]) or not a.is_contiguous() or not b.is_contiguous():
        raise NativeError('cat2_rows: two contiguous tensors of one dtype and equal leading dimensions expected')
    out = torch.empty(tuple(a.shape[:-1]) + (ca + cb,), dtype=a.dtype, device=a.device)
    _check(lib().pcacc_cat2_rows(_dev(a, None, 'a'), int(ca * a.element_size()), _dev(b, None, 'b'), int(cb * b.element_size()), rows, _dev(out),
                                 _stream()), 'cat2_rows')
    return out


def gather_rows(src, idx):
    row_bytes = src.shape[1] * src.element_size()
    out = torch.empty((idx.shape[0], src.shape[1]), dtype=src.dtype, device=src.device)
    _check(lib().pcacc_gather_rows(_dev(src, None, 'src'), int(row_bytes), _dev(idx, torch.int32, 'idx'), idx.shape[0], _dev(out), _stream()), 'gather_rows')
    return out


def bilinear_gather(fmap, points, map_idx, x_scale, y_scale):
    n_maps, h, w, c = fmap.shape
    k = points.shape[0]
    out = torch.empty((k, c), dtype=torch.float32, device=fmap.device)
    _check(lib().pcacc_bilinear_gather(_dev(fmap, None, 'fmap'), _dtype_code(fmap), n_maps, h, w, c,
                                       _dev(points, torch.float32, 'points'), _dev(map_idx, torch.int32, 'map_idx'), k, x_scale, y_scale, _dev(out), _stream()),
           'bilinear_gather')
    return out


def bilinear_gather_backward(grad_out, shape, points, map_idx, x_scale, y_scale):
    n_maps, h, w, c = shape
    g = torch.zeros(shape, dtype=torch.float32, device=grad_out.device)
    _check(lib().pcacc_bilinear_gather_backward(_dev(grad_out, torch.float32, 'grad_out'), n_maps, h, w, c, _dev(points, torch.float32), _dev(map_idx, torch.int32),
                                                points.shape[0], x_scale, y_scale, _dev(g), _stream()), 'bilinear_gather_backward')
    return g


def bev_warp(bev, inv_pose, x_reso, y_reso, x_min, y_min):
    b, t, h, w, c = bev.shape
    out = torch.empty_like(bev)
    _check(lib().pcacc_bev_warp(_dev(bev, None, 'bev'), _dtype_code(bev), b, t, h, w, c, _dev(inv_pose, torch.float32, 'inv_pose'), x_reso, y_reso,
                                x_min, y_min, _dev(out), _stream()), 'bev_warp')
    return out



def bev_warp_dual(bev, inv_pose, x_reso, y_reso, x_min, y_min):
    b, nt, h, w, c = bev.shape
    out = torch.empty_like(bev)
    out16 = torch.empty(bev.shape, dtype=torch.bfloat16, device=bev.device)
    _check(lib().pcacc_bev_warp_dual(_dev(bev, torch.float32, 'bev'), b, nt, h, w, c, _dev(inv_pose, torch.float32, 'inv_pose'), x_reso,
                                     y_reso, x_min, y_min, _dev(out), _dev(out16), _stream()), 'bev_warp_dual')
    return out, out16


def rigid_transform(points, frame_idx, tsfm):
    out = torch.empty_like(points)
    _check(lib().pcacc_rigid_transform(_dev(points, torch.float32, 'points'), _dev(frame_idx, torch.int32, 'frame_idx'),
                                       _dev(tsfm, torch.float32, 'tsfm'), points.shape[0], _dev(out), _stream()), 'rigid_transform')
    return out


def chamfer_forward(xyz1, xyz2):
    b, n, _ = xyz1.shape
    m = xyz2.shape[1]
    dev = xyz1.device
    d1 = torch.empty((b, n), dtype=torch.float32, device=dev)
    d2 = torch.empty((b, m), dtype=torch.float32, device=dev)
    i1 = torch.empty((b, n), dtype=torch.int32, device=dev)
    i2 = torch.empty((b, m), dtype=torch.int32, device=dev)
    ws = _workspace(lib().pcacc_chamfer_workspace_bytes, dev, b, n, m)
    _check(lib().pcacc_chamfer_forward(_dev(xyz1, torch.float32, 'xyz1'), _dev(xyz2, torch.float32, 'xyz2'), b, n, m,
                                       _dev(d1), _dev(i1), _dev(d2), _dev(i2), _dev(ws), ws.numel(), _stream()), 'chamfer_forward')
    return d1, d2, i1, i2


def chamfer_backward(xyz1, xyz2, gd1, gd2, i1, i2):
    b, n, _ = xyz1.shape
    m = xyz2.shape[1]
    g1 = torch.empty_like(xyz1)
    g2 = torch.empty_like(xyz2)
    _check(lib().pcacc_chamfer_backward(_dev(xyz1, torch.float32), _dev(xyz2, torch.float32), b, n, m,
                                        _dev(gd1, torch.float32, 'grad_dist1'), _dev(i1, torch.int32),
                                        _dev(gd2, torch.float32, 'grad_dist2'), _dev(i2, torch.int32),
                                        _dev(g1), _dev(g2), _stream()), 'chamfer_backward')
    return g1, g2


ROWS_LINEAR_K = (2, 3, 4, 9, 32, 64, 128)


def rows_linear_supported(k, n):
    return k in ROWS_LINEAR_K and 1 <= n <= 128


def _row_dtype_bit(t, bit, what):
    if t is None or t.dtype == torch.float32:
        return 0
    if t.dtype == torch.bfloat16:
        return bit
    raise NativeError('%s must be float32 or bfloat16, got %s' % (what, t.dtype))


def rows_linear(x, w, bias=None, residual=None, pre_relu=False, post_relu=False, in_mask=None, out_mask=None, out_dtype=None):
    rows, k = x.shape
    n = w.shape[0]
    out_dtype = out_dtype or x.dtype
    y = torch.empty((rows, n), dtype=out_dtype, device=x.device)
    opt = lambda t, what: _dev(t, None, what) if t is not None else None
    flags = (1 if pre_relu else 0) | (2 if post_relu else 0)
    tensors = (x, in_mask, residual, out_mask, y)
    all_bf16 = all(t is None or t.dtype == torch.bfloat16 for t in tensors)
    if all_bf16 and k in (32, 64, 128) and n in (32, 64, 128):
        _check(lib().pcacc_rows_linear_bf16(_dev(x, torch.bfloat16, 'x'), opt(in_mask, 'in_mask'), _dev(w, torch.float32, 'w'),
                                            _dev(bias, torch.float32, 'bias') if bias is not None else None, opt(residual, 'residual'),
                                            opt(out_mask, 'out_mask'), _dev(y), rows, int(k), int(n), flags, _stream()), 'rows_linear_bf16')
        return y
    dt = (_row_dtype_bit(x, 1, 'x') | _row_dtype_bit(in_mask, 2, 'in_mask') | _row_dtype_bit(residual, 4, 'residual')
          | _row_dtype_bit(out_mask, 8, 'out_mask') | _row_dtype_bit(y, 16, 'y'))
    _check(lib().pcacc_rows_linear_mixed(_dev(x, None, 'x'), opt(in_mask, 'in_mask'), _dev(w, torch.float32, 'w'),
                                         _dev(bias, torch.float32, 'bias') if bias is not None else None, opt(residual, 'residual'),
                                         opt(out_mask, 'out_mask'), _dev(y), rows, int(k), int(n), flags, dt, _stream()), 'rows_linear')
    return y


def _split_aug(out, n, k, split, native_split):
    if not split:
        return out
    if native_split:
        flat = out.view(-1)
        return flat[:n * k].view(n, k), flat[n * k:]
    return out[:, :-1], out[:, -1]


def rows_wgrad(dy, x, dy_mask=None, x_relu=False, split=False):
    rows, n = dy.shape
    k = x.shape[1]
    out = torch.empty((n, k + 1), dtype=torch.float32, device=dy.device)
    flags = (1 if x_relu else 0) | (2 if split else 0)
    if all(t is None or t.dtype == torch.bfloat16 for t in (dy, dy_mask, x)) and k % 32 == 0 and n % 32 == 0:
        ws = _workspace(lib().pcacc_rows_wgrad_bf16_workspace_bytes, dy.device, rows, int(k), int(n))
        _check(lib().pcacc_rows_wgrad_bf16(_dev(dy, torch.bfloat16, 'dy'), _dev(dy_mask, torch.bfloat16, 'dy_mask') if dy_mask is not None else None,
                                           _dev(x, torch.bfloat16, 'x'), flags, rows, int(k), int(n), _dev(out), _dev(ws), ws.numel(), _stream()), 'rows_wgrad_bf16')
        return _split_aug(out, n, k, split, True)
    dt = _row_dtype_bit(dy, 1, 'dy') | _row_dtype_bit(dy_mask, 2, 'dy_mask') | _row_dtype_bit(x, 4, 'x')
    if lib().pcacc_rows_wgrad_few_supported(int(k), int(n)):
        ws = _workspace(lib().pcacc_rows_wgrad_few_workspace_bytes, dy.device, rows, int(k), int(n))
        _check(lib().pcacc_rows_wgrad_few(_dev(dy, None, 'dy'), _dev(dy_mask, None, 'dy_mask') if dy_mask is not None else None, _dev(x, None, 'x'),
                                          flags, rows, int(k), int(n), _dev(out), dt, _dev(ws), ws.numel(), _stream()), 'rows_wgrad_few')
        return _split_aug(out, n, k, split, rows > 0)
    _check(lib().pcacc_rows_wgrad_mixed(_dev(dy, None, 'dy'), _dev(dy_mask, None, 'dy_mask') if dy_mask is not None else None,
                                        _dev(x, None, 'x'), 1 if x_relu else 0, rows, int(k), int(n), _dev(out), dt, _stream()), 'rows_wgrad')
    return _split_aug(out, n, k, split, False)


def pfn_features(points, p2v, pillar_mean, coords, time_indice, vx, vy, x_offset, y_offset, scale, n_frames, order=None):
    n = points.shape[0]
    out = torch.empty((n, 9), dtype=torch.float32, device=points.device)
    if coords.dtype == torch.float64:
        is_f64 = 1
    elif coords.dtype == torch.int32:
        is_f64 = 0
# ... 377 lines not shown
    if not weight.is_cuda or weight.dtype != torch.float32 or tuple(weight.shape[2:]) != (2, 2):
        raise NativeError('upconv2x2_bf16_prepare_weights: float32 GPU weight [c_in, c_up, 2, 2] expected')
    fwd = torch.empty((4 * cu, ci), dtype=torch.bfloat16, device=weight.device)
    bwd = torch.empty((ci, 4 * cu), dtype=torch.bfloat16, device=weight.device)
    strides = (ctypes.c_int64 * 4)(*weight.stride())
    _check(lib().pcacc_upconv2x2_bf16_prepare_weights(ctypes.c_void_p(weight.data_ptr()), int(ci), int(cu), strides, _dev(fwd), _dev(bwd), _stream()),
           'upconv2x2_bf16_prepare_weights')
    return fwd, bwd


def _rows_pitch(rows, what):
    n, h, w, c = rows.shape
    st = rows.stride()
    pitch = st[2]
    if st[3] != 1 or pitch < c or st[1] != w * pitch or st[0] != h * w * pitch or pitch % 8 or rows.data_ptr() % 16:
        return None
    return pitch


def upconv2x2_bf16(x_rows, wp, bias, direction):
    if x_rows.dtype != torch.bfloat16 or not x_rows.is_cuda:
        raise NativeError('upconv2x2_bf16: bf16 GPU rows expected')
    pitch = _rows_pitch(x_rows, 'x')
    if pitch is None:
        x_rows = x_rows.contiguous()
        pitch = x_rows.shape[3]
    n = x_rows.shape[0]
    if direction == 0:
        h, w, c_in = x_rows.shape[1:]
        c_up = wp.shape[0] // 4
        out = torch.empty((n, 2 * h, 2 * w, c_up), dtype=torch.bfloat16, device=x_rows.device)
        out_pitch = c_up
    else:
        h, w, c_up = x_rows.shape[1] // 2, x_rows.shape[2] // 2, x_rows.shape[3]
        c_in = wp.shape[0]
        out = torch.empty((n, h, w, c_in), dtype=torch.bfloat16, device=x_rows.device)
        out_pitch = c_in
    _check(lib().pcacc_upconv2x2_bf16(ctypes.c_void_p(x_rows.data_ptr()), _dev(wp, torch.bfloat16, 'wp'), _opt(bias, torch.float32, 'bias') if direction == 0 else None,
                                      _dev(out), int(n), int(h), int(w), int(c_in), int(c_up), int(direction), int(pitch), int(out_pitch), _stream()),
           'upconv2x2_bf16')
    return out


def upconv2x2_bf16_wgrad(dy_rows, x_rows, want_bias=True, like=None):
    n, h, w, c_in = x_rows.shape
    c_up = dy_rows.shape[3]
    dp, xp = _rows_pitch(dy_rows, 'dy'), _rows_pitch(x_rows, 'x')
    if dp is None:
        dy_rows, dp = dy_rows.contiguous(), c_up
    if xp is None:
        x_rows, xp = x_rows.contiguous(), c_in
    if dy_rows.dtype != torch.bfloat16 or x_rows.dtype != torch.bfloat16 or tuple(dy_rows.shape[:3]) != (n, 2 * h, 2 * w):
        raise NativeError('upconv2x2_bf16_wgrad: bf16 rows [n,2h,2w,c_up] and [n,h,w,c_in] expected')
    if like is not None and tuple(like.shape) == (c_in, c_up, 2, 2):
        dw = torch.empty_strided(like.shape, like.stride(), dtype=torch.float32, device=x_rows.device)
    else:
        dw = torch.empty((c_in, c_up, 2, 2), dtype=torch.float32, device=x_rows.device)
    dws = (ctypes.c_int64 * 4)(*dw.stride())
    db = torch.empty((c_up,), dtype=torch.float32, device=x_rows.device) if want_bias else None
    ws = _workspace(lib().pcacc_upconv2x2_bf16_wgrad_workspace_bytes, x_rows.device, int(n), int(h), int(w), int(c_in), int(c_up))
    _check(lib().pcacc_upconv2x2_bf16_wgrad(ctypes.c_void_p(dy_rows.data_ptr()), int(dp), ctypes.c_void_p(x_rows.data_ptr()), int(xp), ctypes.c_void_p(dw.data_ptr()),
                                            dws, _dev(db) if db is not None else None, int(n), int(h), int(w), int(c_in), int(c_up), _dev(ws),
                                            ws.numel(), _stream()), 'upconv2x2_bf16_wgrad')
    return dw, db


def prepare_weights_batch(jobs, n_jobs, total_blocks):
    if not jobs.is_cuda or jobs.dtype != torch.int64 or not jobs.is_contiguous() or jobs.numel() != 16 * n_jobs:
        raise NativeError('prepare_weights_batch: jobs must be a contiguous int64 GPU tensor [n_jobs, 16]')
    _check(lib().pcacc_prepare_weights_batch(ctypes.c_void_p(jobs.data_ptr()), int(n_jobs), int(total_blocks), _stream()), 'prepare_weights_batch')


def upconv2x2_split(x_rows, amax, wps, bias, direction, want_bf16=False, into=None):
    wp, wscale = wps
    n = x_rows.shape[0]
    if direction == 0:
        h, w, c_in = x_rows.shape[1:]
        c_up = wp.shape[1] // 4
        out = torch.empty((n, 2 * h, 2 * w, c_up), dtype=torch.float32, device=x_rows.device) if into is None else None
    else:
        h, w, c_up = x_rows.shape[1] // 2, x_rows.shape[2] // 2, x_rows.shape[3]
        c_in = wp.shape[1]
        out = torch.empty((n, h, w, c_in), dtype=torch.float32, device=x_rows.device)
    out_amax = _zero256(x_rows.device)
    if want_bf16:
        if direction != 0:
            raise NativeError('upconv2x2_split: the bf16 second output goes with direction 0')
        pitch = 0
        if into is not None:
            out, out16 = into
            pitch = out.shape[3]
            if tuple(out.shape) != (n, 2 * h, 2 * w, pitch) or tuple(out16.shape) != tuple(out.shape) or not out.is_contiguous() or not out16.is_contiguous():
                raise NativeError('upconv2x2_split: concatenation buffers must be contiguous [n,2h,2w,wide] tensors of one shape')
        else:
            out16 = torch.empty(out.shape, dtype=torch.bfloat16, device=x_rows.device)
        _check(lib().pcacc_upconv2x2_split_dual(_dev(x_rows, torch.float32, 'x'), _dev(amax, torch.float32, 'amax'), _dev(wp, torch.float16, 'wp'),
                                                _dev(wscale, torch.float32, 'wscale'), _opt(bias, torch.float32, 'bias'), _dev(out), _dev(out_amax),
                                                _dev(out16), int(n), int(h), int(w), int(c_in), int(c_up), int(pitch), _stream()), 'upconv2x2_split_dual')
        return out, out_amax, out16
    _check(lib().pcacc_upconv2x2_split(_dev(x_rows, torch.float32, 'x'), _dev(amax, torch.float32, 'amax'), _dev(wp, torch.float16, 'wp'),
                                       _dev(wscale, torch.float32, 'wscale'), _opt(bias, torch.float32, 'bias'), _dev(out), _dev(out_amax), int(n),
                                       int(h), int(w), int(c_in), int(c_up), int(direction), _stream()), 'upconv2x2_split')
    return out, out_amax


def upconv2x2_wgrad_split(dy_rows, dy_amax, x_rows, x_amax):
    n, h, w, c_in = x_rows.shape
    c_up = dy_rows.shape[3]
    dw = torch.empty((4 * c_up, c_in), dtype=torch.float32, device=x_rows.device)
    db4 = torch.empty((4 * c_up,), dtype=torch.float32, device=x_rows.device)
    ws = _workspace(lib().pcacc_upconv2x2_wgrad_split_workspace_bytes, x_rows.device, int(n), int(h), int(w), int(c_in), int(c_up))
    _check(lib().pcacc_upconv2x2_wgrad_split(_dev(dy_rows, torch.float32, 'dy'), _dev(dy_amax, torch.float32, 'dy_amax'), _dev(x_rows, torch.float32, 'x'),
                                             _dev(x_amax, torch.float32, 'x_amax'), _dev(dw), _dev(db4), int(n), int(h), int(w), int(c_in), int(c_up),
                                             _dev(ws), ws.numel(), _stream()), 'upconv2x2_wgrad_split')
    return dw.view(2, 2, c_up, c_in).permute(3, 2, 0, 1), db4.view(4, c_up).sum(0)


def head_conv3x3_supported(c_in, c_out):
    return bool(lib().pcacc_head_conv3x3_supported(int(c_in), int(c_out)))


def head_conv3x3_forward(x_rows, weight, bias):
    n, h, w, c_in = x_rows.shape
    c_out = weight.shape[0]
    y = torch.empty((n, h, w, c_out), dtype=torch.float32, device=x_rows.device)
    strides = (ctypes.c_int64 * 4)(*weight.stride())
    _check(lib().pcacc_head_conv3x3_forward(_dev(x_rows, None, 'x'), _dtype_code(x_rows), ctypes.c_void_p(weight.data_ptr()), strides,
                                            _opt(bias, torch.float32, 'bias'), _dev(y), int(n), int(h), int(w), int(c_in), int(c_out), _stream()),
           'head_conv3x3_forward')
    return y


def head_conv3x3_dgrad(dy_rows, weight, c_in, out_dtype):
    n, h, w, c_out = dy_rows.shape
    dx = torch.empty((n, h, w, c_in), dtype=out_dtype, device=dy_rows.device)
    strides = (ctypes.c_int64 * 4)(*weight.stride())
    _check(lib().pcacc_head_conv3x3_dgrad(_dev(dy_rows, torch.float32, 'dy'), ctypes.c_void_p(weight.data_ptr()), strides, _dev(dx), _dtype_code(dx),
                                          int(n), int(h), int(w), int(c_in), int(c_out), _stream()), 'head_conv3x3_dgrad')
    return dx


def head_conv3x3_wgrad(dy_rows, x_rows, want_bias=True):
    n, h, w, c_out = dy_rows.shape
    c_in = x_rows.shape[3]
    dw = torch.empty((c_out, c_in, 3, 3), dtype=torch.float32, device=dy_rows.device)
    db = torch.empty((c_out,), dtype=torch.float32, device=dy_rows.device) if want_bias else None
    ws = _workspace(lib().pcacc_head_conv3x3_wgrad_workspace_bytes, dy_rows.device, int(n), int(h), int(w), int(c_in), int(c_out))
    _check(lib().pcacc_head_conv3x3_wgrad(_dev(dy_rows, torch.float32, 'dy'), _dev(x_rows, None, 'x'), _dtype_code(x_rows), _dev(dw),
                                          _dev(db) if db is not None else None, int(n), int(h), int(w), int(c_in), int(c_out), _dev(ws),
                                          ws.numel(), _stream()), 'head_conv3x3_wgrad')
    return dw, db


def rows_split_supported(k, n):
    return k in (32, 64, 128) and n in (32, 64, 128)


def rows_linear_split(x, x_amax, w, bias=None, residual=None, pre_relu=False, post_relu=False, in_mask=None, out_mask=None, want_amax=False,
                      want_bf16=False):
    rows, k = x.shape
    n = w.shape[0]
    y = torch.empty((rows, n), dtype=torch.float32, device=x.device)
    y_amax = _zero256(x.device) if want_amax or want_bf16 else None
    flags = (1 if pre_relu else 0) | (2 if post_relu else 0)
    if want_bf16:
        y16 = torch.empty((rows, n), dtype=torch.bfloat16, device=x.device)
        _check(lib().pcacc_rows_linear_split_dual(_dev(x, torch.float32, 'x'), _dev(x_amax, torch.float32, 'x_amax'), _opt(in_mask, torch.float32, 'in_mask'),
                                                  _dev(w, torch.float32, 'w'), _opt(bias, torch.float32, 'bias'), _opt(residual, torch.float32, 'residual'),
                                                  _opt(out_mask, torch.float32, 'out_mask'), _dev(y), _dev(y16), _dev(y_amax), rows, int(k),
                                                  int(n), flags, _stream()), 'rows_linear_split_dual')
        return y, y_amax, y16
    _check(lib().pcacc_rows_linear_split(_dev(x, torch.float32, 'x'), _dev(x_amax, torch.float32, 'x_amax'), _opt(in_mask, torch.float32, 'in_mask'),
                                         _dev(w, torch.float32, 'w'), _opt(bias, torch.float32, 'bias'), _opt(residual, torch.float32, 'residual'),
                                         _opt(out_mask, torch.float32, 'out_mask'), _dev(y), _opt(y_amax, torch.float32, 'y_amax'), rows, int(k),
                                         int(n), flags, _stream()), 'rows_linear_split')
    return (y, y_amax) if want_amax else y


def rows_linear_few_dual(x, w, bias=None, residual=None, pre_relu=False, post_relu=False):
    rows, k = x.shape
    n = w.shape[0]
    y = torch.empty((rows, n), dtype=torch.float32, device=x.device)
    y16 = torch.empty((rows, n), dtype=torch.bfloat16, device=x.device)
    y_amax = _zero256(x.device)
    flags = (1 if pre_relu else 0) | (2 if post_relu else 0)
    _check(lib().pcacc_rows_linear_few_dual(_dev(x, torch.float32, 'x'), _dev(w, torch.float32, 'w'), _opt(bias, torch.float32, 'bias'),
                                            _opt(residual, torch.float32, 'residual'), _dev(y), _dev(y16), _dev(y_amax), rows, int(k), int(n),
                                            flags, _stream()), 'rows_linear_few_dual')
    return y, y_amax, y16


def rows_wgrad_split(dy, dy_amax, x, x_amax, dy_mask=None, x_relu=False, split=False):
    rows, n = dy.shape
    k = x.shape[1]
    out = torch.empty((n, k + 1), dtype=torch.float32, device=dy.device)
    ws = _workspace(lib().pcacc_rows_wgrad_split_workspace_bytes, dy.device, rows, int(k), int(n))
    _check(lib().pcacc_rows_wgrad_split(_dev(dy, torch.float32, 'dy'), _dev(dy_amax, torch.float32, 'dy_amax'), _opt(dy_mask, torch.float32, 'dy_mask'),
                                        _dev(x, torch.float32, 'x'), _dev(x_amax, torch.float32, 'x_amax'), (1 if x_relu else 0) | (2 if split else 0),
                                        rows, int(k), int(n), _dev(out), _dev(ws), ws.numel(), _stream()), 'rows_wgrad_split')
    return _split_aug(out, n, k, split, rows > 0)


def rows_linear_cat_split(xa, xa_amax, xb, xb_amax, b_index, w, bias=None, residual=None, pre_relu=False, post_relu=False, want_amax=False):
    rows, ka = xa.shape
    k, n = ka + xb.shape[1], w.shape[0]
    y = torch.empty((rows, n), dtype=torch.float32, device=xa.device)
    y_amax = _zero256(xa.device) if want_amax else None
    flags = (1 if pre_relu else 0) | (2 if post_relu else 0)
    _check(lib().pcacc_rows_linear_cat_split(_dev(xa, torch.float32, 'xa'), _dev(xa_amax, torch.float32, 'xa_amax'), _dev(xb, torch.float32, 'xb'),
                                             _dev(xb_amax, torch.float32, 'xb_amax'), _opt(b_index, torch.int32, 'b_index'), int(ka), None,
                                             _dev(w, torch.float32, 'w'), _opt(bias, torch.float32, 'bias'), _opt(residual, torch.float32, 'residual'),
                                             None, None, _dev(y), None, 0, _opt(y_amax, torch.float32, 'y_amax'), rows, int(k), int(n), flags,
                                             _stream()), 'rows_linear_cat_split')
    return (y, y_amax) if want_amax else y


def rows_linear_cat_backward_split(gy, gy_amax, w_t, dy_mask, xa, xb, b_index, pre_relu):
    rows, n = gy.shape
    ka, kb = xa.shape[1], xb.shape[1]
    ga = torch.empty((rows, ka), dtype=torch.float32, device=gy.device)
    gb = torch.empty((rows, kb), dtype=torch.float32, device=gy.device)
    g_amax = _zero256(gy.device)
    _check(lib().pcacc_rows_linear_cat_split(_dev(gy, torch.float32, 'gy'), _dev(gy_amax, torch.float32, 'gy_amax'), None, None,
                                             _opt(b_index, torch.int32, 'b_index'), 0, _opt(dy_mask, torch.float32, 'dy_mask'),
                                             _dev(w_t, torch.float32, 'w_t'), None, None,
                                             _dev(xa, torch.float32, 'xa') if pre_relu else None, _dev(xb, torch.float32, 'xb') if pre_relu else None,
                                             _dev(ga), _dev(gb), int(ka), _dev(g_amax), rows, int(n), int(ka + kb), 0, _stream()), 'rows_linear_cat_backward_split')
    return ga, gb, g_amax


def rows_wgrad_cat_split(dy, dy_amax, xa, xa_amax, xb, xb_amax, b_index, dy_mask=None, x_relu=False, split=False):
    rows, n = dy.shape
    ka = xa.shape[1]
    k = ka + xb.shape[1]
    out = torch.empty((n, k + 1), dtype=torch.float32, device=dy.device)
    ws = _workspace(lib().pcacc_rows_wgrad_split_workspace_bytes, dy.device, rows, int(k), int(n))
    _check(lib().pcacc_rows_wgrad_cat_split(_dev(dy, torch.float32, 'dy'), _dev(dy_amax, torch.float32, 'dy_amax'), _opt(dy_mask, torch.float32, 'dy_mask'),
                                            _dev(xa, torch.float32, 'xa'), _dev(xa_amax, torch.float32, 'xa_amax'), _dev(xb, torch.float32, 'xb'),
                                            _dev(xb_amax, torch.float32, 'xb_amax'), _opt(b_index, torch.int32, 'b_index'), int(ka),
                                            (1 if x_relu else 0) | (2 if split else 0), rows, int(k), int(n), _dev(out), _dev(ws),
                                            ws.numel(), _stream()), 'rows_wgrad_cat_split')
    return _split_aug(out, n, k, split, rows > 0)


def upload_small(values, dtype, device):
    host = torch.as_tensor(values, dtype=dtype).contiguous()
    if device.type != 'cuda':
        return host
    out = torch.empty(host.shape, dtype=dtype, device=device)
    nbytes = host.numel() * host.element_size()
    if nbytes == 0:
        return out
    if nbytes % 4:
        raise NativeError('upload_small: byte size must be a multiple of 4')
    _check(lib().pcacc_upload_words(ctypes.c_void_p(host.data_ptr()), nbytes // 4, _dev(out), _stream()), 'upload_words')
    return out


def bilinear_gather_backward_sorted(grad_out, shape, points, map_idx, x_scale, y_scale, out_dtype=torch.float32):
    n_maps, h, w, c = shape
    k = points.shape[0]
    dev = grad_out.device
    out = torch.empty((n_maps, h, w, c), dtype=out_dtype, device=dev)
    if k == 0:
        return out.zero_()
    cells = torch.empty((k,), dtype=torch.int32, device=dev)
    _check(lib().pcacc_bilinear_base_cells(_dev(points, torch.float32, 'points'), _dev(map_idx, torch.int32, 'map_idx'), k,
                                           int(n_maps), int(h), int(w), x_scale, y_scale, _dev(cells), _stream()), 'bilinear_base_cells')
    offs, order = csr_build(cells, n_maps * h * w + 1)
    ws = _workspace(lib().pcacc_bilinear_sorted_workspace_bytes, dev, k, int(c), _dtype_code(grad_out))
    _check(lib().pcacc_bilinear_gather_backward_sorted(_dev(grad_out, None, 'grad_out'), _dtype_code(grad_out), int(n_maps), int(h),
                                                       int(w), int(c), _dev(points, torch.float32, 'points'), _dev(offs, torch.int32),
                                                       _dev(order, torch.int32), k, x_scale, y_scale, _dev(out), _dtype_code(out), _dev(ws), ws.numel(), _stream()),
           'bilinear_gather_backward_sorted')
    return out


def prep_points(points, tsfm12, noise, noise_scale, scale, crop_xy, z_min, z_max, remove_ground, ground_z):
    m = points.shape[0]
    out = torch.empty_like(points)
    keep = torch.empty((m,), dtype=torch.uint8, device=points.device)
    _check(lib().pcacc_prep_points(_dev(points, torch.float64, 'points'), _dev(tsfm12, torch.float64, 'tsfm12') if tsfm12 is not None else None,
                                   _dev(noise, torch.float64, 'noise') if noise is not None else None, noise_scale, scale, crop_xy, z_min, z_max,
                                   1 if remove_ground else 0, ground_z, m, _dev(out), _dev(keep), _stream()), 'prep_points')
    return out, keep


def _sinkhorn_ws(P, k, dev):
    return _workspace(lib().pcacc_sinkhorn_train_workspace_bytes, dev, int(P), int(k))


def sinkhorn_forward(log_alpha, n_iters):
    P, k, _ = log_alpha.shape
    dev = log_alpha.device
    out = torch.empty_like(log_alpha)
    lr = torch.empty((n_iters, P, k), dtype=torch.float32, device=dev)
    lc = torch.empty((n_iters, P, k), dtype=torch.float32, device=dev)
    ws = _sinkhorn_ws(P, k, dev)
    _check(lib().pcacc_sinkhorn_forward(_dev(log_alpha, torch.float32, 'log_alpha'), int(P), int(k), int(n_iters), _dev(out), _dev(lr),
                                        _dev(lc), _dev(ws), ws.numel(), _stream()), 'sinkhorn_forward')
    return out, lr, lc


def sinkhorn_backward(grad_log_perm, log_alpha, lse_rows, lse_cols):
    P, k, _ = log_alpha.shape
    n_iters = lse_rows.shape[0]
# ... 18 lines not shown
    ws = _workspace(lib().pcacc_seg_loss_workspace_bytes, dev, n)
    _check(lib().pcacc_seg_loss_forward(_dev(logits, None, 'logits'), _dtype_code(logits), plane, _dev(labels, torch.int64, 'labels'),
                                        _opt(rows, torch.int64, 'rows'), n, _dev(loss), _dev(metric), _dev(lov), _dev(saved), _dev(ws),
                                        ws.numel(), _stream()), 'seg_loss_forward')
    return loss, metric, lov, saved


def seg_loss_backward(logits, plane, labels, rows, n, lovasz_grad, saved, grad_bce, grad_lovasz):
    grad = torch.empty_like(logits)
    _check(lib().pcacc_seg_loss_backward(_dev(logits, None, 'logits'), _dtype_code(logits), plane, _dev(labels, torch.int64, 'labels'),
                                         _opt(rows, torch.int64, 'rows'), n, logits.numel() // 2, _dev(lovasz_grad, torch.float32),
                                         _dev(saved, torch.float32), _opt(grad_bce, torch.float32, 'grad_bce'),
                                         _opt(grad_lovasz, torch.float32, 'grad_lovasz'), _dev(grad), _stream()), 'seg_loss_backward')
    return grad


def offset_loss_forward(points, time_indice, inst_labels, label_base, ego_motion, inst_motion, n_frames, transformed_points, offset_est, rows):
    dev = points.device
    n, k = points.shape[0], inst_motion.shape[0]
    m = rows.shape[0] if rows is not None else n
    out = torch.empty((3,), dtype=torch.float32, device=dev)
    gt = torch.empty((m, 2), dtype=torch.float32, device=dev)
    ws = _workspace(lib().pcacc_offset_loss_workspace_bytes, dev, m, k)
    _check(lib().pcacc_offset_loss_forward(_dev(points, torch.float32, 'points'), _dev(time_indice, torch.int64, 'time_indice'),
                                           _dev(inst_labels, torch.int64, 'inst_labels'), _dev(label_base, torch.int64, 'label_base'),
                                           _dev(ego_motion, torch.float32, 'ego_motion'), _dev(inst_motion, torch.float32, 'inst_motion'),
                                           int(n_frames), n, k, _dev(transformed_points, torch.float32, 'transformed_points'),
                                           _dev(offset_est, torch.float32, 'offset_est'), _opt(rows, torch.int64, 'rows'), m, _dev(out),
                                           _dev(gt), _dev(ws), ws.numel(), _stream()), 'offset_loss_forward')
    return out, gt


def offset_loss_backward(offset_gt, offset_est, rows, grad_norm, grad_dir):
    grad = torch.empty_like(offset_est)
    m = offset_gt.shape[0]
    _check(lib().pcacc_offset_loss_backward(_dev(offset_gt, torch.float32), _dev(offset_est, torch.float32, 'offset_est'),
                                            _opt(rows, torch.int64, 'rows'), m, offset_est.shape[0],
                                            _opt(grad_norm, torch.float32, 'grad_norm'), _opt(grad_dir, torch.float32, 'grad_dir'), _dev(grad),
                                            _stream()), 'offset_loss_backward')
    return grad


def frames_max(x):
    S, T = x.shape[0], x.shape[1]
    plane = x[0, 0].numel()
    out = torch.empty((S,) + tuple(x.shape[2:]), dtype=x.dtype, device=x.device)
    arg = torch.empty((S,) + tuple(x.shape[2:]), dtype=torch.uint8, device=x.device)
    _check(lib().pcacc_frames_max(_dev(x, None, 'x'), _dtype_code(x), S, int(T), plane, _dev(out), _dev(arg), _stream()), 'frames_max')
    return out, arg


def frames_max_backward(grad_out, arg, frames):
    S = grad_out.shape[0]
    plane = grad_out[0].numel()
    g = torch.empty((S, frames) + tuple(grad_out.shape[1:]), dtype=grad_out.dtype, device=grad_out.device)
    _check(lib().pcacc_frames_max_backward(_dev(grad_out, None, 'grad_out'), _dev(arg, torch.uint8), _dtype_code(grad_out), S, int(frames),
                                           plane, _dev(g), _stream()), 'frames_max_backward')
    return g


def rows_linear_cat_supported(ka, kb, n):
    return (ka + kb) in (32, 64, 128) and n in (32, 64, 128) and ka % 8 == 0 and kb % 8 == 0


def rows_linear_cat(xa, xb, b_index, w, bias=None, residual=None, pre_relu=False, post_relu=False):
    rows, ka = xa.shape
    k, n = ka + xb.shape[1], w.shape[0]
    y = torch.empty((rows, n), dtype=torch.bfloat16, device=xa.device)
    flags = (1 if pre_relu else 0) | (2 if post_relu else 0)
    _check(lib().pcacc_rows_linear_cat_bf16(_dev(xa, torch.bfloat16, 'xa'), _dev(xb, torch.bfloat16, 'xb'), _opt(b_index, torch.int32, 'b_index'),
                                            int(ka), None, _dev(w, torch.float32, 'w'), _opt(bias, torch.float32, 'bias'),
                                            _opt(residual, torch.bfloat16, 'residual'), None, None, _dev(y), None, 0, rows, int(k), int(n),
                                            flags, _stream()), 'rows_linear_cat')
    return y


def rows_linear_cat_backward(gy, w_t, dy_mask, xa, xb, b_index, pre_relu):
    rows, n = gy.shape
    ka, kb = xa.shape[1], xb.shape[1]
    ga = torch.empty((rows, ka), dtype=torch.bfloat16, device=gy.device)
    gb = torch.empty((rows, kb), dtype=torch.bfloat16, device=gy.device)
    _check(lib().pcacc_rows_linear_cat_bf16(_dev(gy, torch.bfloat16, 'gy'), None, _opt(b_index, torch.int32, 'b_index'), 0,
                                            _opt(dy_mask, torch.bfloat16, 'dy_mask'), _dev(w_t, torch.float32, 'w_t'), None, None,
                                            _dev(xa, torch.bfloat16, 'xa') if pre_relu else None, _dev(xb, torch.bfloat16, 'xb') if pre_relu else None,
                                            _dev(ga), _dev(gb), int(ka), rows, int(n), int(ka + kb), 0, _stream()), 'rows_linear_cat_backward')
    return ga, gb


def rows_wgrad_cat(dy, xa, xb, b_index, dy_mask=None, x_relu=False, split=False):
    rows, n = dy.shape
    ka = xa.shape[1]
    k = ka + xb.shape[1]
    out = torch.empty((n, k + 1), dtype=torch.float32, device=dy.device)
    ws = _workspace(lib().pcacc_rows_wgrad_bf16_workspace_bytes, dy.device, rows, int(k), int(n))
    _check(lib().pcacc_rows_wgrad_cat_bf16(_dev(dy, torch.bfloat16, 'dy'), _opt(dy_mask, torch.bfloat16, 'dy_mask'), _dev(xa, torch.bfloat16, 'xa'),
                                           _dev(xb, torch.bfloat16, 'xb'), _opt(b_index, torch.int32, 'b_index'), int(ka),
                                           (1 if x_relu else 0) | (2 if split else 0),
                                           rows, int(k), int(n), _dev(out), _dev(ws), ws.numel(), _stream()), 'rows_wgrad_cat')
    return _split_aug(out, n, k, split, rows > 0)


def svd3(a):
    n = a.shape[0]
    u, v = torch.empty_like(a), torch.empty_like(a)
    s = torch.empty((n, 3), dtype=torch.float32, device=a.device)
    _check(lib().pcacc_svd3(_dev(a, torch.float32, 'a'), n, _dev(u), _dev(s), _dev(v), _stream()), 'svd3')
    return u, s, v


def svd3_backward(u, s, v, gu, gs, gv):
    ga = torch.empty_like(u)
    _check(lib().pcacc_svd3_backward(_dev(u, torch.float32), _dev(s, torch.float32), _dev(v, torch.float32), _opt(gu, torch.float32, 'grad_u'),
                                     _opt(gs, torch.float32, 'grad_s'), _opt(gv, torch.float32, 'grad_v'), u.shape[0], _dev(ga), _stream()), 'svd3_backward')
    return ga


def bn_rows_supported(x):
    c = x.shape[1] if x.dim() == 2 else 0
    v = 8 if x.dtype == torch.bfloat16 else 4
    return x.dim() == 2 and x.dtype in (torch.float32, torch.bfloat16) and x.shape[0] >= 1 and 0 < c <= 256 and c % v == 0 and 256 % (c // v) == 0


def _bn_ws(rows, c, dev):
    return _workspace(lib().pcacc_bn_rows_workspace_bytes, dev, rows, int(c))


def bn_rows_forward(x, gamma, beta, eps, momentum, running_mean, running_var, relu=False):
    rows, c = x.shape
    y = torch.empty_like(x)
    mean = torch.empty((c,), dtype=torch.float32, device=x.device)
    invstd = torch.empty((c,), dtype=torch.float32, device=x.device)
    ws = _bn_ws(rows, c, x.device)
    fn = lib().pcacc_bn_relu_rows_forward if relu else lib().pcacc_bn_rows_forward
    _check(fn(_dev(x, None, 'x'), _dtype_code(x), rows, int(c), _opt(gamma, torch.float32, 'gamma'),
                                       _opt(beta, torch.float32, 'beta'), eps, momentum,
                                       _opt(running_mean, torch.float32, 'running_mean'), _opt(running_var, torch.float32, 'running_var'),
                                       _dev(y), _dev(mean), _dev(invstd), _dev(ws), ws.numel(), _stream()), 'bn_rows_forward')
    return y, mean, invstd


def bn_rows_forward_dual(x, gamma, beta, eps, momentum, running_mean, running_var, relu=False):
    rows, c = x.shape
    y = torch.empty_like(x)
    y16 = torch.empty((rows, c), dtype=torch.bfloat16, device=x.device)
    am = _zero256(x.device)
    mean = torch.empty((c,), dtype=torch.float32, device=x.device)
    invstd = torch.empty((c,), dtype=torch.float32, device=x.device)
    ws = _bn_ws(rows, c, x.device)
    _check(lib().pcacc_bn_rows_forward_dual(_dev(x, torch.float32, 'x'), rows, int(c), _opt(gamma, torch.float32, 'gamma'), _opt(beta, torch.float32, 'beta'),
                                            eps, momentum, _opt(running_mean, torch.float32, 'running_mean'),
                                            _opt(running_var, torch.float32, 'running_var'), 1 if relu else 0, _dev(y), _dev(y16), _dev(am), _dev(mean),
                                            _dev(invstd), _dev(ws), ws.numel(), _stream()), 'bn_rows_forward_dual')
    return y, y16, am, mean, invstd


def bn_rows_backward(grad_y, x, gamma, save_mean, save_invstd, relu_beta=None, relu=False, want_amax=False):
    rows, c = x.shape
    gx = torch.empty_like(x)
    gg = torch.empty((c,), dtype=torch.float32, device=x.device)
    gb = torch.empty((c,), dtype=torch.float32, device=x.device)
    ws = _bn_ws(rows, c, x.device)
    if grad_y.dtype != x.dtype:
        raise NativeError('bn_rows_backward: grad_y must have the type of x')
    if want_amax:
        am = _zero256(x.device)
        _check(lib().pcacc_bn_rows_backward_m(_dev(grad_y, None, 'grad_y'), _dev(x, None, 'x'), _dtype_code(x), rows, int(c),
                                              _opt(gamma, torch.float32, 'gamma'), _opt(relu_beta, torch.float32, 'beta') if relu else None, 1 if relu else 0,
                                              _dev(save_mean, torch.float32), _dev(save_invstd, torch.float32), _dev(gx), _dev(am), _dev(gg), _dev(gb),
                                              _dev(ws), ws.numel(), _stream()), 'bn_rows_backward_m')
        return gx, gg, gb, am
    if relu:
        _check(lib().pcacc_bn_relu_rows_backward(_dev(grad_y, None, 'grad_y'), _dev(x, None, 'x'), _dtype_code(x), rows, int(c),
                                                 _opt(gamma, torch.float32, 'gamma'), _opt(relu_beta, torch.float32, 'beta'),
                                                 _dev(save_mean, torch.float32), _dev(save_invstd, torch.float32), _dev(gx), _dev(gg), _dev(gb),
                                                 _dev(ws), ws.numel(), _stream()), 'bn_relu_rows_backward')
        return gx, gg, gb
    _check(lib().pcacc_bn_rows_backward(_dev(grad_y, None, 'grad_y'), _dev(x, None, 'x'), _dtype_code(x), rows, int(c),
                                        _opt(gamma, torch.float32, 'gamma'), _dev(save_mean, torch.float32), _dev(save_invstd, torch.float32),
                                        _dev(gx), _dev(gg), _dev(gb), _dev(ws), ws.numel(), _stream()), 'bn_rows_backward')
    return gx, gg, gb


def tube_rows(xyz, slot, slot_centre, n_frames):
    n = xyz.shape[0]
    rows = torch.empty((n, 4), dtype=torch.float32, device=xyz.device)
    _check(lib().pcacc_tube_rows(_dev(xyz, torch.float32, 'xyz'), _dev(slot, torch.int32, 'slot'), _dev(slot_centre, torch.float32, 'slot_centre'),
                                 n, int(n_frames), _dev(rows), _stream()), 'tube_rows')
    return rows


def tube_code(geo, motion, frame, n_frames):
    n_inst, c = geo.shape
    code = torch.empty((n_inst * n_frames, 4 * c), dtype=torch.float32, device=geo.device)
    _check(lib().pcacc_tube_code(_dev(geo, torch.float32, 'geo'), _dev(motion, torch.float32, 'motion'), _dev(frame, torch.float32, 'frame'),
                                 n_inst, int(n_frames), int(c), _dev(code), _stream()), 'tube_code')
    return code


def tube_code_backward(grad_code, n_inst, n_frames, c):
    dev = grad_code.device
    g_geo = torch.empty((n_inst, c), dtype=torch.float32, device=dev)
    g_motion = torch.empty((n_inst, c), dtype=torch.float32, device=dev)
    g_frame = torch.empty((n_inst * n_frames, c), dtype=torch.float32, device=dev)
    _check(lib().pcacc_tube_code_backward(_dev(grad_code, torch.float32, 'grad_code'), n_inst, int(n_frames), int(c), _dev(g_geo),
                                          _dev(g_motion), _dev(g_frame), _stream()), 'tube_code_backward')
    return g_geo, g_motion, g_frame


def tube_pose_forward(pose_vec, remaining, total, slot_centre, weights, n_frames):
    s = pose_vec.shape[0]
    dev = pose_vec.device
    f = lambda *shape: torch.empty(shape, dtype=torch.float32, device=dev)
    pose_c, gt_c, step, rem_out, total_out, wsum = f(s, 12), f(s, 12), f(s, 4, 4), f(s, 4, 4), f(s, 4, 4), f(1)
    loss_rt = torch.empty((2,), dtype=torch.float64, device=dev)
    _check(lib().pcacc_tube_pose_forward(_dev(pose_vec, torch.float32, 'pose_vec'), _dev(remaining, torch.float32, 'remaining'),
                                         _opt(total, torch.float32, 'total'), _dev(slot_centre, torch.float32, 'slot_centre'),
                                         _dev(weights, torch.float32, 'weights'), int(s), int(n_frames), _dev(pose_c), _dev(gt_c), _dev(step),
                                         _dev(rem_out), _dev(total_out), _dev(loss_rt), _dev(wsum), _stream()), 'tube_pose_forward')
    return pose_c, gt_c, step, rem_out, total_out, loss_rt, wsum


def tube_gap_forward(rows, slot, pose_c, gt_c):
    n = rows.shape[0]
    pp = torch.empty((n, 4), dtype=torch.float32, device=rows.device)
    _check(lib().pcacc_tube_gap_forward(_dev(rows, torch.float32, 'rows'), _dev(slot, torch.int32, 'slot'), _dev(pose_c, torch.float32, 'pose_c'),
                                        _dev(gt_c, torch.float32, 'gt_c'), n, _dev(pp), _stream()), 'tube_gap_forward')
    return pp


def tube_finish(slot_sums, count, weights, wsum):
    l12 = torch.empty((2,), dtype=torch.float32, device=slot_sums.device)
    _check(lib().pcacc_tube_finish(_dev(slot_sums, torch.float32, 'slot_sums'), int(slot_sums.shape[1]), _dev(count, torch.float32, 'count'),
                                   _dev(weights, torch.float32, 'weights'), _dev(wsum, torch.float32, 'wsum'), int(slot_sums.shape[0]),
                                   _dev(l12), _stream()), 'tube_finish')
    return l12


def tube_gap_backward(rows, slot, pose_c, gt_c, weights, count, wsum, grad_l1, grad_l2):
    n = rows.shape[0]
    g16 = torch.empty((n, 16), dtype=torch.float32, device=rows.device)
    _check(lib().pcacc_tube_gap_backward(_dev(rows, torch.float32, 'rows'), _dev(slot, torch.int32, 'slot'), _dev(pose_c, torch.float32, 'pose_c'),
                                         _dev(gt_c, torch.float32, 'gt_c'), _dev(weights, torch.float32, 'weights'),
                                         _dev(count, torch.float32, 'count'), _dev(wsum, torch.float32, 'wsum'),
                                         _opt(grad_l1, torch.float32, 'grad_l1'), _opt(grad_l2, torch.float32, 'grad_l2'), n, _dev(g16),
                                         _stream()), 'tube_gap_backward')
    return g16


def tube_pose_backward(pose_vec, remaining, slot_centre, weights, wsum, grad_pose, grad_rot, grad_trans, n_frames):
    s = pose_vec.shape[0]
    g_vec = torch.empty((s, 7), dtype=torch.float32, device=pose_vec.device)
    _check(lib().pcacc_tube_pose_backward(_dev(pose_vec, torch.float32, 'pose_vec'), _dev(remaining, torch.float32, 'remaining'),
                                          _dev(slot_centre, torch.float32, 'slot_centre'), _dev(weights, torch.float32, 'weights'),
                                          _dev(wsum, torch.float32, 'wsum'), _dev(grad_pose, torch.float32, 'grad_pose'), int(grad_pose.shape[1]),
                                          _opt(grad_rot, torch.float64, 'grad_rot'), _opt(grad_trans, torch.float64, 'grad_trans'), int(s),
                                          int(n_frames), _dev(g_vec), _stream()), 'tube_pose_backward')
    return g_vec


def maxpool2x2(x_rows):
    n, h, w, c = x_rows.shape
    out = torch.empty((n, h // 2, w // 2, c), dtype=x_rows.dtype, device=x_rows.device)
    if x_rows.dtype == torch.float32:
        _check(lib().pcacc_maxpool2x2_f32(_dev(x_rows, torch.float32, 'x'), n, int(h), int(w), int(c), _dev(out), _stream()), 'maxpool2x2')
    else:
        _check(lib().pcacc_maxpool2x2_bf16(_dev(x_rows, torch.bfloat16, 'x'), n, int(h), int(w), int(c), _dev(out), _stream()), 'maxpool2x2')
    return out


def _pixel_pitch(g, shape):
    n, h, w, c = shape
    if tuple(g.shape) != tuple(shape) or g.stride(3) != 1:
        return None
    p = g.stride(2)
    if p < c or g.stride(1) != w * p or g.stride(0) != h * w * p or g.data_ptr() % 16:
        return None
    return p


def pool_skip_relu_backward(y_rows, grad_pooled, grad_skip, want_amax=False):
    n, h, w, c = y_rows.shape
    if y_rows.dtype == torch.float32 and any(g is not None and g.dtype == torch.bfloat16 for g in (grad_pooled, grad_skip)):
        out = torch.empty(y_rows.shape, dtype=torch.bfloat16, device=y_rows.device)
        pitch, gs_ptr = c, None
        if grad_skip is not None:
            pitch = _pixel_pitch(grad_skip, y_rows.shape)
            if pitch is None or pitch % 8:
                grad_skip, pitch = grad_skip.contiguous(), c
            gs_ptr = ctypes.c_void_p(grad_skip.data_ptr())
        _check(lib().pcacc_pool_skip_relu_backward_strided_y32(_dev(y_rows, torch.float32, 'y'), _opt(grad_pooled, torch.bfloat16, 'grad_pooled'), gs_ptr,
                                                               pitch, n, int(h), int(w), int(c), _dev(out), _stream()), 'pool_skip_relu_backward')
        return out
    out = torch.empty_like(y_rows)
    f32 = y_rows.dtype == torch.float32
    dt = torch.float32 if f32 else torch.bfloat16
    pitch, gs_ptr = c, None
    if grad_skip is not None:
        if grad_skip.dtype != dt or not grad_skip.is_cuda:
            raise NativeError('pool_skip_relu_backward: grad_skip must be a %s GPU tensor' % dt)
        pitch = _pixel_pitch(grad_skip, y_rows.shape)
        if pitch is None or pitch % (4 if f32 else 8):
            grad_skip, pitch = grad_skip.contiguous(), c
        gs_ptr = ctypes.c_void_p(grad_skip.data_ptr())
    if f32:
        amax = _zero256(y_rows.device) if want_amax else None
        _check(lib().pcacc_pool_skip_relu_backward_strided_f32(_dev(y_rows, torch.float32, 'y'), _opt(grad_pooled, torch.float32, 'grad_pooled'), gs_ptr,
# ... 170 lines not shown
```

### pcaccumulation_amd/ops.py

```python
import weakref

import os

import torch

from . import native


class PillarIndex(object):

    def __init__(self, coordinates, point_to_voxel_map, batch_size, input_shape, cell_order=False):
        nx, ny, nz, nt = (int(v) for v in input_shape[:4])
        self.nx, self.ny, self.nt, self.batch_size = nx, ny, nt, int(batch_size)
        self.m = int(coordinates.shape[0])
        self.n_cells = self.batch_size * nt * ny * nx
        self.cells_per_frame = ny * nx
        coords = coordinates.contiguous()
        if coords.dtype not in (torch.float64, torch.int32):
            coords = coords.to(torch.float64)
        self.cell, self.cell2pillar = native.cell_index(coords, nx, ny, nt, self.batch_size)
        self.coordinates, self.perm, self._frames = coordinates, None, None
        p2v = point_to_voxel_map
        if p2v is not None:
            p2v = (p2v[:, 0] if p2v.dim() == 2 else p2v).to(torch.int32)
# ... 1344 lines not shown
            gw = gw.to(weight.dtype)
            gb = gb if ctx.has_bias and ctx.needs_input_grad[2] else None
        return gx, gw, gb


_PREPARED_UPB = {}


def prepared_upconv_weights_bf16(weight):
    key = id(weight)
    hit = _PREPARED_UPB.get(key)
    if hit is not None and hit[0]() is weight and hit[1] == _weight_key(weight):
        return hit[2], hit[3]
    got = _batch_hit(_PREPARED_UPB, weight, 3)
    if got is not None:
        return got
    _batch_note(weight, 3)
    fwd, bwd = native.upconv2x2_bf16_prepare_weights(weight.detach())
    if len(_PREPARED_UPB) > 4096:
        _PREPARED_UPB.clear()
    _PREPARED_UPB[key] = (_weight_ref(_PREPARED_UPB, key, weight), _weight_key(weight), fwd, bwd)
    return fwd, bwd


def _upconv_bf16_backward(ctx, gy, x_rows, weight):
    c_in, c_up = weight.shape[0], weight.shape[1]
    if gy.dtype != torch.bfloat16:
        gy = gy.to(torch.bfloat16)
    if native.upconv2x2_bf16_supported(c_in, c_up) and weight.dtype == torch.float32 and os.environ.get('PCACC_UPCONV_BF16', '1') != '0':
        gx = native.upconv2x2_bf16(gy, prepared_upconv_weights_bf16(weight)[1], None, 1) if ctx.needs_input_grad[0] else None
        gw = gb = None
        if ctx.needs_input_grad[1] or (ctx.has_bias and ctx.needs_input_grad[2]):
            gw, gb = native.upconv2x2_bf16_wgrad(gy, x_rows, want_bias=ctx.has_bias and ctx.needs_input_grad[2], like=weight)
        return gx, gw, gb
    gy = gy.contiguous()
    w16 = weight.detach().to(torch.bfloat16).contiguous(memory_format=torch.channels_last)
    gx, gw, _ = torch.ops.aten.convolution_backward(
        gy.permute(0, 3, 1, 2), x_rows.permute(0, 3, 1, 2), w16, None, [2, 2], [0, 0], [1, 1], True, [0, 0], 1,
        [ctx.needs_input_grad[0], ctx.needs_input_grad[1], False])
    gb = gy.reshape(-1, gy.shape[-1]).sum(0, dtype=torch.float32) if ctx.has_bias and ctx.needs_input_grad[2] else None
    if gx is not None:
        gx = gx.permute(0, 2, 3, 1).contiguous()
    return gx, (gw.float().contiguous(memory_format=torch.channels_last) if gw is not None else None), gb


class _UpConv2x2Bf16(torch.autograd.Function):

    @staticmethod
    def forward(ctx, x_rows, weight, bias):
        ctx.save_for_backward(x_rows, weight)
        ctx.has_bias = bias is not None
        return native.upconv2x2_bf16(x_rows, prepared_upconv_weights_bf16(weight)[0], bias.detach().float() if bias is not None else None, 0)

    @staticmethod
    def backward(ctx, gy):
        x_rows, weight = ctx.saved_tensors
        return _upconv_bf16_backward(ctx, gy, x_rows, weight)


class _UpConv2x2Mixed(torch.autograd.Function):

    @staticmethod
    def forward(ctx, x_rows, weight, bias):
        x32 = twin(x_rows)
        y32, y_amax, y16 = native.upconv2x2_split(x32, amax_of(x32), prepared_upconv_weights_split(weight)[0], bias.detach() if bias is not None else None, 0,
                                                  want_bf16=True)
        set_amax_tag(y32, y_amax)
        ctx.save_for_backward(x_rows, weight)
        ctx.has_bias = bias is not None
        return shadow(y32, y16)

    @staticmethod
    def backward(ctx, gy):
        x_rows, weight = ctx.saved_tensors
        return _upconv_bf16_backward(ctx, gy, x_rows, weight)


class _UpConvCatMixed(torch.autograd.Function):

    @staticmethod
    def forward(ctx, x_rows, skip_rows, weight, bias):
        x32, s32 = twin(x_rows), twin(skip_rows)
        n, h, w, _ = x_rows.shape
        c_up, c_skip = weight.shape[1], skip_rows.shape[3]
        if c_skip != c_up or tuple(skip_rows.shape[:3]) != (n, 2 * h, 2 * w):
            raise native.NativeError('upconv + concatenation: the skip map must have the up-sampled map\'s shape')
        buf32 = torch.empty((n, 2 * h, 2 * w, 2 * c_up), dtype=torch.float32, device=x_rows.device)
        buf16 = torch.empty((n, 2 * h, 2 * w, 2 * c_up), dtype=torch.bfloat16, device=x_rows.device)
        _, up_amax, _ = native.upconv2x2_split(x32, amax_of(x32), prepared_upconv_weights_split(weight)[0], bias.detach() if bias is not None else None, 0,
                                               want_bf16=True, into=(buf32, buf16))
        buf32[..., c_up:].copy_(s32)
        if _POISON:
            buf16.fill_(float('nan'))
        else:
            buf16[..., c_up:].copy_(skip_rows)
        set_amax_tag(buf32, torch.maximum(up_amax, amax_of(s32)))
        ctx.save_for_backward(x_rows, weight)
        ctx.has_bias, ctx.c_up = bias is not None, c_up
        return shadow(buf32, buf16)

    @staticmethod
    def backward(ctx, g):
        x_rows, weight = ctx.saved_tensors
        c_up = ctx.c_up
        gy = g[..., :c_up].contiguous()
        w16 = weight.detach().to(torch.bfloat16).contiguous(memory_format=torch.channels_last)
        gx, gw, _ = torch.ops.aten.convolution_backward(
            gy.permute(0, 3, 1, 2), x_rows.permute(0, 3, 1, 2), w16, None, [2, 2], [0, 0], [1, 1], True, [0, 0], 1,
            [ctx.needs_input_grad[0], ctx.needs_input_grad[2], False])
        gb = gy.reshape(-1, c_up).sum(0, dtype=torch.float32) if ctx.has_bias and ctx.needs_input_grad[3] else None
        if gx is not None:
            gx = gx.permute(0, 2, 3, 1).contiguous()
        return (gx, g[..., c_up:] if ctx.needs_input_grad[1] else None,
                gw.float().contiguous(memory_format=torch.channels_last) if gw is not None else None, gb)


def upconv_cat(from_up, from_down, conv):
    if (_MIXED and from_up.is_cuda and from_up.dtype == torch.bfloat16 and from_down.dtype == torch.bfloat16
            and conv.kernel_size == (2, 2) and conv.stride == (2, 2) and conv.padding == (0, 0) and conv.output_padding == (0, 0) and conv.groups == 1
            and conv.dilation == (1, 1) and conv.weight.dtype == torch.float32 and conv.out_channels == from_down.shape[1]
            and os.environ.get('PCACC_UPCONV_CAT', '0') == '1'):
        xr, sr = from_up.permute(0, 2, 3, 1), from_down.permute(0, 2, 3, 1)
        if xr.is_contiguous() and sr.is_contiguous() and native.upconv2x2_split_supported(from_up.shape[-2], from_up.shape[-1], conv.in_channels, conv.out_channels):
            return _UpConvCatMixed.apply(xr, sr, conv.weight, conv.bias).permute(0, 3, 1, 2)
    return cat_maps((upconv2x2(from_up, conv), from_down), 1)


def upconv2x2(x, conv):
    plain = (conv.kernel_size == (2, 2) and conv.stride == (2, 2) and conv.padding == (0, 0) and conv.output_padding == (0, 0) and conv.groups == 1
             and conv.dilation == (1, 1) and conv.weight.dtype == torch.float32)
    if _MIXED and x.is_cuda and x.dtype == torch.bfloat16:
        xr = x.permute(0, 2, 3, 1)
        if not (plain and xr.is_contiguous() and native.upconv2x2_split_supported(x.shape[-2], x.shape[-1], conv.in_channels, conv.out_channels)):
            raise native.NativeError('mixed mode: transposed convolution outside the split kernels (%s)' % (tuple(x.shape),))
        return _UpConv2x2Mixed.apply(xr, conv.weight, conv.bias).permute(0, 3, 1, 2)
    if (_SPLIT and x.is_cuda and x.dtype == torch.float32 and not torch.is_autocast_enabled() and plain
            and native.upconv2x2_split_supported(x.shape[-2], x.shape[-1], conv.in_channels, conv.out_channels)):
        xr = x.permute(0, 2, 3, 1)
        if xr.is_contiguous():
            set_amax_tag(xr, amax_of(x))
            y = _UpConv2x2Split.apply(xr, conv.weight, conv.bias)
            return carry_amax(y, y.permute(0, 3, 1, 2))
    if (x.is_cuda and plain and (x.dtype == torch.bfloat16 or (torch.is_autocast_enabled() and torch.get_autocast_dtype('cuda') == torch.bfloat16))
            and native.upconv2x2_bf16_supported(conv.in_channels, conv.out_channels) and os.environ.get('PCACC_UPCONV_BF16', '1') != '0'):
        xr = x.permute(0, 2, 3, 1)
        if xr.is_contiguous():
            return _UpConv2x2Bf16.apply(xr if xr.dtype == torch.bfloat16 else xr.to(torch.bfloat16), conv.weight, conv.bias).permute(0, 3, 1, 2)
    return conv(x)


class _HeadConv3x3(torch.autograd.Function):

    @staticmethod
    def forward(ctx, x_rows, weight, bias):
        ctx.save_for_backward(x_rows, weight)
        ctx.has_bias = bias is not None
        return native.head_conv3x3_forward(twin_or_self(x_rows), weight.detach(), bias.detach() if bias is not None else None)

    @staticmethod
    def backward(ctx, gy):
        x_rows, weight = ctx.saved_tensors
        gy = gy.contiguous().float()
        gx = gw = gb = None
        if ctx.needs_input_grad[0]:
            gx = native.head_conv3x3_dgrad(gy, weight.detach(), x_rows.shape[3], x_rows.dtype)
        if ctx.needs_input_grad[1] or (ctx.has_bias and ctx.needs_input_grad[2]):
            gw, gb = native.head_conv3x3_wgrad(gy, x_rows, want_bias=ctx.has_bias)
            gw = gw.to(weight.dtype)
        return gx, gw, gb


def head_conv3x3_available(x, conv):
    return (x.is_cuda and x.dim() == 4 and x.dtype in (torch.float32, torch.bfloat16) and conv.kernel_size == (3, 3) and conv.stride == (1, 1)
            and conv.padding == (1, 1) and conv.dilation == (1, 1) and conv.groups == 1 and conv.weight.dtype == torch.float32
            and native.head_conv3x3_supported(conv.in_channels, conv.out_channels) and x.permute(0, 2, 3, 1).is_contiguous())


def _stack_frames(rows, frames):
    n, h, w, c = rows.shape
    r = rows.view(n // frames, frames, h, w, c)
    prev = torch.nn.functional.pad(r[:, :-1], (0, 0, 0, 0, 0, 0, 1, 0))
    nxt = torch.nn.functional.pad(r[:, 1:], (0, 0, 0, 0, 0, 0, 0, 1))
    return torch.cat([prev, r, nxt], dim=-1).view(n, h, w, 3 * c)


def conv3x3_preferred(c_in, c_out, h=None, w=None):
    if not native.conv3x3_supported(c_in, c_out):
        return False
    if c_in <= 64:
        return True
    return h is not None and native.conv3x3_deep_supported(h, w, c_in, c_out)


def conv3x3_available(x, weight):
    if not x.is_cuda:
        return None
    if _MIXED and x.dtype == torch.bfloat16:
        if not (weight.dtype == torch.float32 and native.conv3x3_split_supported(x.shape[-2], x.shape[-1], weight.shape[1], weight.shape[0])):
            raise native.NativeError('mixed mode: 3x3 convolution outside the split kernels (%s, weight %s)' % (tuple(x.shape), tuple(weight.shape)))
        return 'mixed'
    if x.dtype == torch.bfloat16 or (torch.is_autocast_enabled() and torch.get_autocast_dtype('cuda') == torch.bfloat16):
        return 'bf16' if conv3x3_preferred(weight.shape[1], weight.shape[0], x.shape[-2], x.shape[-1]) else None
    if _SPLIT and x.dtype == torch.float32 and weight.dtype == torch.float32 \
            and native.conv3x3_split_supported(x.shape[-2], x.shape[-1], weight.shape[1], weight.shape[0]):
        return 'split'
    return None


def conv3x3_rows(x_rows, weight, bias, frames=1, relu=False, premasked=False, input_relu=False):
    if _MIXED and x_rows.dtype == torch.bfloat16:
        return _Conv3x3Mixed.apply(x_rows.contiguous(), weight, bias, int(frames), bool(relu), bool(premasked), bool(input_relu))
    if _SPLIT and x_rows.dtype == torch.float32 and not torch.is_autocast_enabled():
        xc = x_rows.contiguous()
        if xc is not x_rows:
            carry_amax(x_rows, xc)
        return _Conv3x3Split.apply(xc, weight, bias, int(frames), bool(relu), bool(premasked), bool(input_relu))
    if x_rows.dtype != torch.bfloat16:
        x_rows = x_rows.to(torch.bfloat16)
    return _Conv3x3.apply(x_rows.contiguous(), weight, bias, int(frames), bool(relu), bool(premasked), bool(input_relu))


def conv3x3_native(x, conv):
    if conv.kernel_size == (3, 3) and conv.stride == (1, 1) and conv.padding == (1, 1) and conv.dilation == (1, 1) and conv.groups == 1:
        return conv3x3_available(x, conv.weight)
    return None


def conv_pair_fusable(x, conv1, conv2):
    mode = conv3x3_native(x, conv1)
    if mode not in ('bf16', 'split', 'mixed') or conv2.in_channels != conv1.out_channels or os.environ.get('PCACC_CONV_PAIR', '1') == '0':
        return False
    probe = torch.empty((0, conv1.out_channels, x.shape[-2], x.shape[-1]), dtype=torch.float32 if mode == 'split' else torch.bfloat16, device=x.device)
    return conv3x3_native(probe, conv2) == mode


def conv3x3(x, conv, relu=False, premasked=False, input_relu=False):
    if not relu and head_conv3x3_available(x, conv):
        return _HeadConv3x3.apply(x.permute(0, 2, 3, 1), conv.weight, conv.bias).permute(0, 3, 1, 2)
    mode = conv3x3_native(x, conv)
    if mode:
        xr = x.permute(0, 2, 3, 1)
        if mode == 'split' and xr.is_contiguous():
            set_amax_tag(xr, amax_of(x))
        y = conv3x3_rows(xr, conv.weight, conv.bias, 1, relu, premasked=premasked, input_relu=input_relu)
        return carry_amax(y, y.permute(0, 3, 1, 2))
    assert not premasked and not input_relu
    y = conv(x)
    return torch.relu(y) if relu else y


class _PoolSkip(torch.autograd.Function):

    @staticmethod
    def forward(ctx, y_rows):
        if _MIXED and y_rows.dtype == torch.bfloat16:
            y32 = twin(y_rows)
            ctx.save_for_backward(y32)
            ctx.mixed = True
            return shadow(carry_amax(y32, native.maxpool2x2(y32))), y_rows.view_as(y_rows)
        ctx.save_for_backward(y_rows)
        ctx.mixed = False
        pooled = native.maxpool2x2(y_rows)
        skip = y_rows.view_as(y_rows)
        if y_rows.dtype == torch.float32:
            carry_amax(y_rows, pooled)
            carry_amax(y_rows, skip)
        return pooled, skip

    @staticmethod
    def backward(ctx, g_pool, g_skip):
        y_rows, = ctx.saved_tensors
        if ctx.mixed:
            b16 = lambda g: g.to(torch.bfloat16) if g is not None else None
            return native.pool_skip_relu_backward(y_rows, b16(g_pool.contiguous() if g_pool is not None else None), b16(g_skip))
        c = lambda g: g.contiguous().to(y_rows.dtype) if g is not None else None
        gs = g_skip.to(y_rows.dtype) if g_skip is not None else None
        if y_rows.dtype == torch.float32:
            g, g_amax = native.pool_skip_relu_backward(y_rows, c(g_pool), gs, want_amax=True)
            return set_amax_tag(g, g_amax)
        return native.pool_skip_relu_backward(y_rows, c(g_pool), gs)


def conv3x3_relu_pool(x, conv, input_relu=False):
    y = conv3x3_rows(x.permute(0, 2, 3, 1), conv.weight, conv.bias, 1, True, premasked=True, input_relu=input_relu)
    pooled, skip = _PoolSkip.apply(y)
    return pooled.permute(0, 3, 1, 2), skip.permute(0, 3, 1, 2)


class _SparseConv3x3(torch.autograd.Function):

    @staticmethod
    def forward(ctx, h_rows, weight, bias, cells):
        n, H, W, C = h_rows.shape
        cells = cells.reshape(-1).long()
        x, y, img = cells % W, (cells // W) % H, cells // (W * H)
        d = torch.arange(-1, 2, device=cells.device)
        yy, xx = (y[:, None, None] + d[None, :, None]).expand(-1, 3, 3), (x[:, None, None] + d[None, None, :]).expand(-1, 3, 3)
        ok = (yy >= 0) & (yy < H) & (xx >= 0) & (xx < W)
        idx = torch.where(ok, (img[:, None, None] * H + yy) * W + xx, torch.full_like(yy, -1)).reshape(-1).to(torch.int32)
        patches = native.gather_rows(h_rows.reshape(-1, C), idx).view(-1, 9 * C)
        w2 = weight.detach().float().permute(2, 3, 1, 0).reshape(9 * C, -1)
        out = torch.addmm(bias.detach().float(), patches, w2) if bias is not None else patches @ w2
        ctx.save_for_backward(patches, w2, idx)
        ctx.meta = (tuple(h_rows.shape), tuple(weight.shape), bias is not None)
        return out

    @staticmethod
    def backward(ctx, g):
        patches, w2, idx = ctx.saved_tensors
        (n, H, W, C), wshape, has_bias = ctx.meta
        g = g.contiguous().float()
        gh = gw = gb = None
        if ctx.needs_input_grad[0]:
            gp = (g @ w2.t()).view(-1, C)
            cells = n * H * W
            if DETERMINISTIC and C % 4 == 0:
                key = torch.where(idx >= 0, idx, cells).to(torch.int32)
                offs, order = native.csr_build(key, cells + 1)
                gh = native.segment_sum(gp.contiguous(), offs, order, cells + 1)[:cells].view(n, H, W, C)
            else:
                gh = torch.zeros((cells + 1, C), dtype=torch.float32, device=g.device)
                gh.index_add_(0, torch.where(idx >= 0, idx, cells).long(), gp)
                gh = gh[:cells].view(n, H, W, C)
        if ctx.needs_input_grad[1]:
            k = g.shape[0]
            if k % 16 == 0 and k >= 4096:
                gw2 = torch.bmm(patches.view(16, k // 16, -1).transpose(1, 2), g.view(16, k // 16, -1)).sum(0)
            else:
                gw2 = patches.t() @ g
            gw = gw2.view(3, 3, wshape[1], wshape[0]).permute(3, 2, 0, 1).contiguous()
        if has_bias and ctx.needs_input_grad[2]:
            gb = g.sum(0)
        return gh, gw, gb, None


class SparseConvRows(object):

    def __init__(self, h, conv):
        self.h, self.conv = h, conv
        self.is_cuda, self.device = h.is_cuda, h.device

    def at(self, cells):
        rows = self.h.permute(0, 2, 3, 1)
        out = _SparseConv3x3.apply(rows if rows.is_contiguous() else rows.contiguous(), self.conv.weight, self.conv.bias, cells)
        return out.view(tuple(cells.shape) + (out.shape[-1],))

    def dense(self):
        return nchw_as_rows(exit_mixed(conv3x3(self.h, self.conv)))


def sparse_conv_available(h, conv):
    return (h.is_cuda and h.dtype == torch.float32 and h.dim() == 4 and conv.kernel_size == (3, 3) and conv.stride == (1, 1) and conv.padding == (1, 1)
            and conv.dilation == (1, 1) and conv.groups == 1 and conv.weight.dtype == torch.float32 and h.shape[1] % 4 == 0
            and os.environ.get('PCACC_SPARSE_EGO', '1') != '0')


class _Sinkhorn(torch.autograd.Function):

    @staticmethod
    def forward(ctx, log_alpha, n_iters):
        log_alpha = log_alpha.contiguous().float()
        out, lr, lc = native.sinkhorn_forward(log_alpha, n_iters)
        ctx.save_for_backward(log_alpha, lr, lc)
        return out

    @staticmethod
    def backward(ctx, grad):
        log_alpha, lr, lc = ctx.saved_tensors
        return native.sinkhorn_backward(grad.contiguous().float(), log_alpha, lr, lc), None


class _EgoAffinity(torch.autograd.Function):

    @staticmethod
    def forward(ctx, feats_s, feats_t, params):
        fs, ft = feats_s.contiguous().float(), feats_t.contiguous().float()
        aff = native.ego_affinity_forward(fs, ft, params)
        ctx.save_for_backward(fs, ft, aff, params)
        return aff

    @staticmethod
    def backward(ctx, g):
        fs, ft, aff, params = ctx.saved_tensors
        gd, gp = native.ego_affinity_backward(g.contiguous().float(), aff, params)
        return torch.bmm(gd, ft), torch.bmm(gd.transpose(1, 2), fs), gp


def ego_affinity(feats_s, feats_t, softplus_alpha, denom):
    params = torch.stack([softplus_alpha.reshape(()), denom.reshape(())]).float()
    return _EgoAffinity.apply(feats_s, feats_t, params)


class _EgoPerm(torch.autograd.Function):

    @staticmethod
    def forward(ctx, log_perm, coor_s, coor_t, thr2):
        ct = coor_t.contiguous().float()
        perm, rowsum, wt, colsum = native.ego_perm_forward(log_perm.contiguous().float(), coor_s.contiguous().float(), ct, thr2.contiguous().float())
        ctx.save_for_backward(perm, ct, rowsum, wt)
        ctx.set_materialize_grads(False)
        return perm, rowsum.unsqueeze(2), wt, colsum

    @staticmethod
    def backward(ctx, g_perm, g_rowsum, g_wt, g_colsum):
        perm, ct, rowsum, wt = ctx.saved_tensors
        c = lambda t: t.contiguous().float() if t is not None else None
        g = native.ego_perm_backward(c(g_perm), c(g_rowsum.squeeze(2)) if g_rowsum is not None else None, c(g_wt), c(g_colsum), perm, ct, rowsum, wt)
        return g, None, None, None


def ego_perm(log_perm, coor_s, coor_t, thr2):
    return _EgoPerm.apply(log_perm, coor_s, coor_t, thr2)


class _KabschCov(torch.autograd.Function):

    @staticmethod
    def forward(ctx, x1, x2, w):
        x1, x2, w = x1.contiguous().float(), x2.contiguous().float(), w.contiguous().float()
        cov, m1, m2, norm = native.kabsch_cov_forward(x1, x2, w)
        ctx.save_for_backward(x1, x2, w, m1, m2, norm)
        ctx.set_materialize_grads(False)
        return cov, m1.unsqueeze(1), m2.unsqueeze(1)

    @staticmethod
    def backward(ctx, g_cov, g_m1, g_m2):
        x1, x2, w, m1, m2, norm = ctx.saved_tensors
        c = lambda t: t.contiguous().float() if t is not None else None
        gx2, gw = native.kabsch_cov_backward(x1, x2, w, m1, m2, norm, c(g_cov), c(g_m1.squeeze(1)) if g_m1 is not None else None,
                                             c(g_m2.squeeze(1)) if g_m2 is not None else None)
        return None, gx2, gw


def kabsch_cov(x1, x2, w):
    return _KabschCov.apply(x1, x2, w)


class _KabschRT(torch.autograd.Function):

    @staticmethod
    def forward(ctx, u, v, m1, m2):
        u, v = u.contiguous().float(), v.contiguous().float()
        m1c, m2c = m1.reshape(-1, 3).contiguous().float(), m2.reshape(-1, 3).contiguous().float()
        rot, trans = native.kabsch_rt_forward(u, v, m1c, m2c)
        ctx.save_for_backward(u, v, m1c)
        ctx.shapes = (m1.shape, m2.shape)
        ctx.set_materialize_grads(False)
        return rot, trans.unsqueeze(2)

    @staticmethod
    def backward(ctx, g_rot, g_trans):
        u, v, m1c = ctx.saved_tensors
        c = lambda t: t.contiguous().float() if t is not None else None
        gu, gv, gm1, gm2 = native.kabsch_rt_backward(u, v, m1c, c(g_rot), c(g_trans.squeeze(2)) if g_trans is not None else None)
        return gu, gv, gm1.view(ctx.shapes[0]), gm2.view(ctx.shapes[1])


def kabsch_rt(u, v, x1_mean, x2_mean):
    return _KabschRT.apply(u, v, x1_mean, x2_mean)


def sinkhorn(log_alpha, n_iters):
    return _Sinkhorn.apply(log_alpha, int(n_iters))


class _SegLoss(torch.autograd.Function):

    @staticmethod
    def forward(ctx, logits, labels, rows, plane):
        n = rows.shape[0] if rows is not None else logits.numel() // 2
        terms, metric, lov, saved = native.seg_loss_forward(logits, plane, labels, rows, n)
        ctx.save_for_backward(logits, labels, rows, lov, saved)
        ctx.plane, ctx.n = plane, n
        ctx.mark_non_differentiable(metric)
        return terms, metric

    @staticmethod
    def backward(ctx, grad_terms, _):
        logits, labels, rows, lov, saved = ctx.saved_tensors
        g = grad_terms.contiguous().float()
        return native.seg_loss_backward(logits, ctx.plane, labels, rows, ctx.n, lov, saved, g[0:1], g[1:2]), None, None, None


def seg_loss(logits, labels, rows=None):
    if logits.dim() >= 3 and not logits.is_contiguous() and logits.movedim(-3, -1).is_contiguous():
        logits = logits.movedim(-3, -1).reshape(-1, 2)
    if logits.dim() >= 3:
        plane = logits.shape[-1] * logits.shape[-2]
        assert logits.shape[-3] == 2
    else:
        plane = 0
        assert logits.dim() == 2 and logits.shape[1] == 2
    if logits.dtype not in (torch.float32, torch.bfloat16):
        logits = logits.float()
    labels = labels.reshape(-1)
    if labels.dtype != torch.int64:
        labels = labels.long()
    if rows is not None and rows.dtype != torch.int64:
        rows = rows.long()
    return _SegLoss.apply(logits.contiguous(), labels.contiguous(), rows, plane)


class _OffsetLoss(torch.autograd.Function):

    @staticmethod
    def forward(ctx, offset_est, points, time_indice, inst_labels, label_base, ego_motion, inst_motion, transformed_points, rows):
        out, gt = native.offset_loss_forward(points, time_indice, inst_labels, label_base, ego_motion, inst_motion, ego_motion.shape[1],
                                             transformed_points, offset_est, rows)
        ctx.save_for_backward(gt, offset_est, rows)
        ctx.mark_non_differentiable(gt)
        return out, gt

    @staticmethod
    def backward(ctx, grad_out, _):
        gt, est, rows = ctx.saved_tensors
        g = grad_out.contiguous().float()
        return (native.offset_loss_backward(gt, est, rows, g[0:1], g[1:2]),) + (None,) * 8


def offset_loss(offset_est, points, time_indice, inst_labels, label_base, ego_motion, inst_motion, transformed_points, rows):
    f = lambda t: t.detach().float().contiguous()
    return _OffsetLoss.apply(offset_est.float().contiguous(), f(points), time_indice.long().contiguous(), inst_labels.long().contiguous(),
                             label_base, f(ego_motion), f(inst_motion), f(transformed_points), rows)


class _FramesMax(torch.autograd.Function):

    @staticmethod
    def forward(ctx, x):
        mixed = _MIXED and x.dtype == torch.bfloat16
        x32 = twin(x) if mixed else x
        out, arg = native.frames_max(x32)
        ctx.save_for_backward(arg)
        ctx.frames = x.shape[1]
        return shadow(carry_amax(x32, out)) if mixed else out

    @staticmethod
    def backward(ctx, grad):
        arg, = ctx.saved_tensors
        return native.frames_max_backward(grad.contiguous(), arg, ctx.frames)


def frames_max(x):
    return _FramesMax.apply(x.contiguous())


class _Svd3(torch.autograd.Function):

    @staticmethod
    def forward(ctx, a):
        u, s, v = native.svd3(a.contiguous().float())
        ctx.save_for_backward(u, s, v)
        return u, s, v

    @staticmethod
    def backward(ctx, gu, gs, gv):
        u, s, v = ctx.saved_tensors
        c = lambda g: g.contiguous().float() if g is not None else None
        return native.svd3_backward(u, s, v, c(gu), c(gs), c(gv))


def svd3(a):
    return _Svd3.apply(a)


class _BatchNormRows(torch.autograd.Function):

    @staticmethod
    def forward(ctx, x, gamma, beta, eps, momentum, running_mean, running_var, relu=False):
        x = x.contiguous()
        mixed = _MIXED and x.dtype == torch.bfloat16
        if mixed and twin(x).dim() == 2 and twin(x).is_contiguous():
            y, y16, am, mean, invstd = native.bn_rows_forward_dual(twin(x), gamma, beta, eps, momentum, running_mean, running_var, relu=relu)
            set_amax_tag(y, am)
            out = shadow(y, y16)
        else:
            y, mean, invstd = native.bn_rows_forward(twin(x) if mixed else x, gamma, beta, eps, momentum, running_mean, running_var, relu=relu)
            out = shadow(y) if mixed else y
        ctx.save_for_backward(x, gamma, mean, invstd, beta if relu else None)
        ctx.relu = relu
        return out

    @staticmethod
    def backward(ctx, gy):
        x, gamma, mean, invstd, beta = ctx.saved_tensors
        if _SPLIT and x.dtype == torch.float32:
            gx, gg, gb, am = native.bn_rows_backward(gy.contiguous().to(x.dtype), x, gamma, mean, invstd, relu_beta=beta, relu=ctx.relu, want_amax=True)
            set_amax_tag(gx, am)
        else:
            gx, gg, gb = native.bn_rows_backward(gy.contiguous().to(x.dtype), x, gamma, mean, invstd, relu_beta=beta, relu=ctx.relu)
        return gx, (gg if gamma is not None else None), (gb if gamma is not None else None), None, None, None, None, None


def batch_norm_rows(x, bn):
    if not (bn.training and x.is_cuda and x.dim() == 2 and bn.momentum is not None and native.bn_rows_supported(x)
            and x.shape[0] >= MIN_ROWS_FUSED_LINEAR and not torch.is_autocast_enabled()
            and (bn.weight is None or bn.weight.dtype == torch.float32)):
        return bn(x)
    if bn.track_running_stats and bn.num_batches_tracked is not None:
        bn.num_batches_tracked.add_(1)
    rm, rv = (bn.running_mean, bn.running_var) if bn.track_running_stats else (None, None)
    return _BatchNormRows.apply(x, bn.weight, bn.bias, float(bn.eps), float(bn.momentum), rm, rv)


def batch_norm_nchw(x, bn, relu=False):
    def module(t):
        return torch.relu(bn(t)) if relu else bn(t)

    def replay(t):
        y = torch.nn.functional.batch_norm(t, None if bn.training else bn.running_mean, None if bn.training else bn.running_var, bn.weight, bn.bias,
                                           bn.training, 0.0, bn.eps)
        return torch.relu(y) if relu else y

    def fallback():
        if _MIXED and x.dtype == torch.bfloat16:
            return on_twin(x, module, [p for p in (bn.weight, bn.bias) if p is not None], replay)
        return module(x)
    if not (bn.training and x.is_cuda and x.dim() == 4 and bn.momentum is not None and x.dtype in (torch.float32, torch.bfloat16)
            and (bn.weight is None or bn.weight.dtype == torch.float32)):
        return fallback()
    rows = x.permute(0, 2, 3, 1)
    if not rows.is_contiguous():
        return fallback()
    n, h, w, c = rows.shape
    rows = rows.reshape(n * h * w, c)
    if not native.bn_rows_supported(rows) or rows.shape[0] < MIN_ROWS_FUSED_LINEAR:
        return fallback()
    if bn.track_running_stats and bn.num_batches_tracked is not None:
        bn.num_batches_tracked.add_(1)
    rm, rv = (bn.running_mean, bn.running_var) if bn.track_running_stats else (None, None)
    y = _BatchNormRows.apply(rows, bn.weight, bn.bias, float(bn.eps), float(bn.momentum), rm, rv, relu)
    return y.view(n, h, w, c).permute(0, 3, 1, 2)
```

### pcaccumulation_amd/unet.py

```python
import os

import torch
import torch.nn as nn
import torch.nn.functional as F
from torch.nn import init

from . import ops


def conv3x3(in_channels, out_channels):
    return nn.Conv2d(in_channels, out_channels, kernel_size=3, stride=1, padding=1, bias=True)


class DownConv(nn.Module):

    def __init__(self, in_channels, out_channels, pooling=True):
        super(DownConv, self).__init__()
        self.in_channels, self.out_channels, self.pooling = in_channels, out_channels, pooling
        self.conv1 = conv3x3(in_channels, out_channels)
        self.conv2 = conv3x3(out_channels, out_channels)
        if pooling:
            self.pool = nn.MaxPool2d(kernel_size=2, stride=2)

    def forward(self, x):
        pair = ops.conv_pair_fusable(x, self.conv1, self.conv2)
        x = ops.conv3x3(x, self.conv1, relu=True, premasked=pair)
        if self.pooling and ops.conv3x3_native(x, self.conv2) in ('bf16', 'split', 'mixed') and self.out_channels % 8 == 0:
            return ops.conv3x3_relu_pool(x, self.conv2, input_relu=pair)
        x = ops.conv3x3(x, self.conv2, relu=True, input_relu=pair)
        return (ops.carry_amax(x, self.pool(x)) if self.pooling else x), x


class UpConv(nn.Module):

    def __init__(self, in_channels, out_channels, merge_mode='concat', up_mode='transpose'):
        super(UpConv, self).__init__()
        assert up_mode == 'transpose', 'only the transpose-conv decoder the released weights use'
        self.in_channels, self.out_channels, self.merge_mode, self.up_mode = in_channels, out_channels, merge_mode, up_mode
        self.upconv = nn.ConvTranspose2d(in_channels, out_channels, kernel_size=2, stride=2)
        self.conv1 = conv3x3(2 * out_channels if merge_mode == 'concat' else out_channels, out_channels)
        self.conv2 = conv3x3(out_channels, out_channels)

    def forward(self, from_down, from_up):
        if self.merge_mode == 'concat' and os.environ.get('PCACC_UPCONV_CAT', '0') != '1':
            up = ops.upconv2x2(from_up, self.upconv)
            probe = up.new_empty((0, self.conv1.in_channels) + tuple(up.shape[2:]))
            pair = ops.conv_pair_fusable(probe, self.conv1, self.conv2)
            x = ops.conv3x3_cat(up, from_down, self.conv1, relu=True, premasked=pair)
            return ops.conv3x3(x, self.conv2, relu=True, input_relu=pair)
        if self.merge_mode == 'concat':
            x = ops.upconv_cat(from_up, from_down, self.upconv)
        else:
            x = ops.upconv2x2(from_up, self.upconv) + from_down
        pair = ops.conv_pair_fusable(x, self.conv1, self.conv2)
        return ops.conv3x3(ops.conv3x3(x, self.conv1, relu=True, premasked=pair), self.conv2, relu=True, input_relu=pair)


class UNet(nn.Module):

    def __init__(self, in_channels=3, depth=5, start_filts=64, up_mode='transpose', merge_mode='concat', **kwargs):
        super(UNet, self).__init__()
        if up_mode not in ('transpose', 'upsample') or merge_mode not in ('concat', 'add'):
            raise ValueError('unsupported up_mode / merge_mode: %s / %s' % (up_mode, merge_mode))
        self.up_mode, self.merge_mode = up_mode, merge_mode
        self.in_channels, self.start_filts, self.depth = in_channels, start_filts, depth
        downs, ups = [], []
        outs = in_channels
        for i in range(depth):
            ins = in_channels if i == 0 else outs
            outs = start_filts * (2 ** i)
            downs.append(DownConv(ins, outs, pooling=i < depth - 1))
        for i in range(depth - 1):
            ins = outs
            outs = ins // 2
            ups.append(UpConv(ins, outs, up_mode=up_mode, merge_mode=merge_mode))
        self.down_convs = nn.ModuleList(downs)
        self.up_convs = nn.ModuleList(ups)
        self.conv_final = conv3x3(outs, in_channels)
        self.reset_params()

    @staticmethod
    def weight_init(m):
        if isinstance(m, nn.Conv2d):
            init.xavier_normal_(m.weight)
            init.constant_(m.bias, 0)

    def reset_params(self):
        for m in self.modules():
            self.weight_init(m)

    def forward(self, x):
        skips = []
        with ops.stage('unet_enc'):
            for module in self.down_convs:
                x, before_pool = module(x)
                skips.append(before_pool)
        with ops.stage('unet_dec'):
            for i, module in enumerate(self.up_convs):
                x = module(skips[-(i + 2)], x)
        with ops.stage('unet_dec'):
            return ops.conv3x3(ops.exit_mixed(x), self.conv_final)


class SegHead1D(nn.Module):

    def __init__(self, in_channel, out_channel, bias=True):
        super(SegHead1D, self).__init__()
        mid = max(in_channel, out_channel)
        self.seg_head = nn.Sequential(nn.Linear(in_channel, mid, bias=bias), nn.BatchNorm1d(mid), nn.ReLU(),
                                      nn.Linear(mid, out_channel, bias=bias))

    def forward(self, feats):
        return self.seg_head(feats)


class SegHead2D(nn.Module):

    def __init__(self, in_channel, out_channel, kernel_size=3, stride=1, padding=1, bias=True, groups=1):
        super(SegHead2D, self).__init__()
        mid = max(in_channel, out_channel)
        self.seg_head = nn.Sequential(
            nn.Conv2d(in_channel, mid, kernel_size=kernel_size, stride=stride, padding=padding, bias=bias, groups=groups),
            nn.BatchNorm2d(mid), nn.ReLU(),
            nn.Conv2d(mid, out_channel, kernel_size=kernel_size, stride=stride, padding=padding, bias=bias, groups=groups))

    def forward(self, feats):
        conv0, bn, act, conv1 = self.seg_head
        fused = isinstance(act, nn.ReLU)
        h = self.hidden(feats)
        return ops.conv3x3(h, conv1)

    def hidden(self, feats):
        conv0, bn, act, conv1 = self.seg_head
        fused = isinstance(act, nn.ReLU)
        h = ops.batch_norm_nchw(ops.exit_mixed(ops.conv3x3(feats, conv0)), bn, relu=fused)
        return h if fused else act(h)

    def sparse_rows(self, feats):
        h = self.hidden(feats)
        conv1 = self.seg_head[3]
        return ops.SparseConvRows(h, conv1) if ops.sparse_conv_available(h, conv1) else ops.nchw_as_rows(ops.exit_mixed(ops.conv3x3(h, conv1)))
```

Measured before the change: 661.5.

## Fold seg-head BatchNorm+ReLU into the following conv's input load

The seg head no longer writes a normalised activation map. It computes only the BN statistics, then applies scale, shift and ReLU on the fly while staging inputs in the head 3x3 conv kernels (forward and wgrad) and in a new sparse gather-rows kernel. The backward pass recomputes the BN input gradient from the saved raw rows. This removes a full-map write and re-read for each seg head, at the cost of extra template variants, LDS space for a per-channel table, and a materialise fallback path.

Result: no change. 656.6 (-0.7%).

```diff
diff --git a/include/pcacc.h b/include/pcacc.h
--- a/include/pcacc.h
+++ b/include/pcacc.h
@@ -380,6 +380,19 @@
                              int32_t relu, const float *save_mean, const float *save_invstd, void *grad_x, float *grad_x_amax, float *grad_gamma,
                              float *grad_beta, void *workspace, size_t workspace_bytes, void *stream);
 
+int pcacc_bn_rows_stats(const float *x, int64_t rows, int32_t c, float eps, float momentum, float *running_mean, float *running_var,
+                        float *save_mean, float *save_invstd, void *workspace, size_t workspace_bytes, void *stream);
+int pcacc_bn_rows_apply(const float *x, int64_t rows, int32_t c, const float *mean, const float *invstd, const float *gamma, const float *beta,
+                        int32_t relu, float *y, void *stream);
+int pcacc_head_conv3x3_forward_bn(const float *x, const float *mean, const float *invstd, const float *gamma, const float *beta, int32_t relu,
+                                  const float *w, const int64_t *w_strides , const float *bias, float *y, int32_t n_img, int32_t h,
+                                  int32_t wd, int32_t c_in, int32_t c_out, void *stream);
+int pcacc_head_conv3x3_wgrad_bn(const float *dy, const float *x, const float *mean, const float *invstd, const float *gamma, const float *beta,
+                                int32_t relu, float *dw, float *db, int32_t n_img, int32_t h, int32_t wd, int32_t c_in, int32_t c_out,
+                                void *workspace, size_t workspace_bytes, void *stream);
+int pcacc_gather_rows_bn(const float *src, int32_t c, const int32_t *idx, int64_t n_idx, const float *mean, const float *invstd,
+                         const float *gamma, const float *beta, int32_t relu, float *out, void *stream);
+
 int pcacc_pfn_block_forward(const uint16_t *xa, const uint16_t *pooled, const int32_t *p2v, const float *w0, const float *b0,
                             const float *ws, const float *w1, const float *b1, uint16_t *out, uint16_t *relu_h, int64_t rows, void *stream);
 int pcacc_pfn_block_backward_workspace_bytes(int64_t rows, size_t *bytes );
diff --git a/pcaccumulation_amd/csrc/bn.hip b/pcaccumulation_amd/csrc/bn.hip
--- a/pcaccumulation_amd/csrc/bn.hip
+++ b/pcaccumulation_amd/csrc/bn.hip
@@ -318,3 +318,27 @@
     return bn_backward_any(grad_y, x, dtype, rows, c, gamma, save_mean, save_invstd, grad_x, grad_gamma, grad_beta, workspace, workspace_bytes, stream,
                            true, beta);
 }
+
+extern "C" int pcacc_bn_rows_stats(const float *x, int64_t rows, int32_t c, float eps, float momentum, float *running_mean, float *running_var,
+                                   float *save_mean, float *save_invstd, void *workspace, size_t workspace_bytes, void *stream)
+{
+    if (bn_args(PCACC_F32, rows, c) != PCACC_OK || !x || !save_mean || !save_invstd || !workspace) return PCACC_E_ARG;
+    const int nb = bn_blocks(rows, c, 4);
+    if (workspace_bytes < (size_t)nb * 2 * c * sizeof(float)) return PCACC_E_WORKSPACE;
+    hipStream_t s = pcacc_stream(stream);
+    float *partial = reinterpret_cast<float *>(workspace);
+    bn_sums_kernel<false><<<nb, 256, 0, s>>>(x, nullptr, nullptr, nullptr, rows, c, partial);
+    bn_finalize_fwd_kernel<<<c, 256, 0, s>>>(partial, nb, c, rows, eps, momentum, running_mean, running_var, save_mean, save_invstd);
+    PCACC_CHECK_LAUNCH();
+    return PCACC_OK;
+}
+
+extern "C" int pcacc_bn_rows_apply(const float *x, int64_t rows, int32_t c, const float *mean, const float *invstd, const float *gamma,
+                                   const float *beta, int32_t relu, float *y, void *stream)
+{
+    if (bn_args(PCACC_F32, rows, c) != PCACC_OK || !x || !mean || !invstd || !y) return PCACC_E_ARG;
+    const int grid = pcacc_grid(rows * (c / 4), 256, PCACC_CUS * 16);
+    bn_apply_kernel<false><<<grid, 256, 0, pcacc_stream(stream)>>>(x, nullptr, mean, invstd, gamma, beta, nullptr, rows, c, y, relu != 0);
+    PCACC_CHECK_LAUNCH();
+    return PCACC_OK;
+}
diff --git a/pcaccumulation_amd/csrc/canvas.hip b/pcaccumulation_amd/csrc/canvas.hip
--- a/pcaccumulation_amd/csrc/canvas.hip
+++ b/pcaccumulation_amd/csrc/canvas.hip
@@ -423,6 +423,47 @@
     return PCACC_OK;
 }
 
+__global__ __launch_bounds__(256) void gather_rows_bn_kernel(const float4 *__restrict__ src, int pieces, const int32_t *__restrict__ idx, int64_t n_idx,
+                                                             const float *__restrict__ mean, const float *__restrict__ invstd,
+                                                             const float *__restrict__ gamma, const float *__restrict__ beta, int relu,
+                                                             float4 *__restrict__ out)
+{
+    const int64_t total = n_idx * pieces;
+    for (int64_t e = (int64_t)blockIdx.x * 256 + threadIdx.x; e < total; e += (int64_t)gridDim.x * 256) {
+        const int64_t r = e / pieces;
+        const int k = (int)(e - r * pieces);
+        const int64_t j = idx[r];
+        float4 o = make_float4(0.f, 0.f, 0.f, 0.f);
+        if (j >= 0) {
+            const float4 x4 = src[j * pieces + k];
+            const float x[4] = {x4.x, x4.y, x4.z, x4.w};
+            float v[4];
+#pragma unroll
+            for (int q = 0; q < 4; ++q) {
+                const int ch = 4 * k + q;
+                float scale, shift;
+                pcacc_bn_scale_shift(mean[ch], invstd[ch], gamma ? gamma[ch] : 1.f, beta ? beta[ch] : 0.f, scale, shift);
+                v[q] = pcacc_bn_value(x[q], scale, shift, relu);
+            }
+            o = make_float4(v[0], v[1], v[2], v[3]);
+        }
+        out[e] = o;
+    }
+}
+
+extern "C" int pcacc_gather_rows_bn(const float *src, int32_t c, const int32_t *idx, int64_t n_idx, const float *mean, const float *invstd,
+                                    const float *gamma, const float *beta, int32_t relu, float *out, void *stream)
+{
+    if (n_idx < 0 || c < 4 || (c % 4) || !mean || !invstd) return PCACC_E_ARG;
+    if (n_idx > 0 && (!src || !idx || !out)) return PCACC_E_ARG;
+    if (n_idx == 0) return PCACC_OK;
+    gather_rows_bn_kernel<<<pcacc_grid(n_idx * (c / 4), 256), 256, 0, pcacc_stream(stream)>>>(reinterpret_cast<const float4 *>(src), c / 4, idx, n_idx, mean,
+                                                                                             invstd, gamma, beta, relu != 0,
+                                                                                             reinterpret_cast<float4 *>(out));
+    PCACC_CHECK_LAUNCH();
+    return PCACC_OK;
+}
+
 __global__ __launch_bounds__(256) void cat2_rows_kernel(const uint4 *__restrict__ a, int pa, const uint4 *__restrict__ b, int pb, int64_t rows,
                                                         uint4 *__restrict__ out)
 {
diff --git a/pcaccumulation_amd/csrc/common.h b/pcaccumulation_amd/csrc/common.h
--- a/pcaccumulation_amd/csrc/common.h
+++ b/pcaccumulation_amd/csrc/common.h
@@ -25,6 +25,17 @@
 const PcaccSwitches &pcacc_switches();
 
 static inline hipStream_t pcacc_stream(void *s) { return reinterpret_cast<hipStream_t>(s); }
+
+__device__ __forceinline__ void pcacc_bn_scale_shift(float mean, float invstd, float gamma, float beta, float &scale, float &shift)
+{
+    scale = invstd * gamma;
+    shift = __builtin_fmaf(-(mean * invstd), gamma, beta);
+}
+__device__ __forceinline__ float pcacc_bn_value(float x, float scale, float shift, int relu)
+{
+    const float o = __builtin_fmaf(x, scale, shift);
+    return relu ? fmaxf(o, 0.f) : o;
+}
 
 static inline int pcacc_grid(int64_t work_items, int block, int max_blocks = PCACC_CUS * 8)
 {
diff --git a/pcaccumulation_amd/csrc/head_conv.hip b/pcaccumulation_amd/csrc/head_conv.hip
--- a/pcaccumulation_amd/csrc/head_conv.hip
+++ b/pcaccumulation_amd/csrc/head_conv.hip
@@ -18,8 +18,27 @@
     return HcTile{img, (r / tiles_x) * HC_TR, (r % tiles_x) * HC_TC};
 }
 
+struct HcBn { const float *mean, *invstd, *gamma, *beta; int relu; };
+
 template <int CI>
-__device__ __forceinline__ void hc_stage(const void *__restrict__ x, int x_bf16, const HcTile &t, int h, int wd, float *patch)
+__device__ __forceinline__ void hc_bn_table(const HcBn &bn, float *tab)
+{
+    for (int ch = threadIdx.x; ch < CI; ch += HC_THREADS) {
+        pcacc_bn_scale_shift(bn.mean[ch], bn.invstd[ch], bn.gamma ? bn.gamma[ch] : 1.f, bn.beta ? bn.beta[ch] : 0.f, tab[ch], tab[CI + ch]);
+    }
+}
+
+template <int CI>
+__device__ __forceinline__ float4 hc_bn4(float4 x, const float *tab, int l4, int relu)
+{
+    const float4 sc = *reinterpret_cast<const float4 *>(tab + 4 * l4), sh = *reinterpret_cast<const float4 *>(tab + CI + 4 * l4);
+    return make_float4(pcacc_bn_value(x.x, sc.x, sh.x, relu), pcacc_bn_value(x.y, sc.y, sh.y, relu), pcacc_bn_value(x.z, sc.z, sh.z, relu),
+                       pcacc_bn_value(x.w, sc.w, sh.w, relu));
+}
+
+template <int CI, bool BN = false>
+__device__ __forceinline__ void hc_stage(const void *__restrict__ x, int x_bf16, const HcTile &t, int h, int wd, float *patch,
+                                         const float *tab = nullptr, int relu = 0)
 {
     constexpr int LPP = CI / 4;
     for (int e = threadIdx.x; e < HC_PH * HC_PW * LPP; e += HC_THREADS) {
@@ -29,6 +48,7 @@
         const bool ok = (unsigned)y < (unsigned)h && (unsigned)xx < (unsigned)wd;
         const int yc = min(max(y, 0), h - 1), xc = min(max(xx, 0), wd - 1);
         float4 v = hc_ld4(x, x_bf16, (((int64_t)t.img * h + yc) * wd + xc) * LPP + l4);
+        if constexpr (BN) v = hc_bn4<CI>(v, tab, l4, relu);
         if (!ok) v = make_float4(0.f, 0.f, 0.f, 0.f);
         *reinterpret_cast<float4 *>(patch + pp * CI + l4 * 4) = v;
     }
@@ -52,8 +72,9 @@
     }
 }
 
-template <int CI, bool BF>
-__device__ __forceinline__ void hc_put(const typename HcRaw<CI, BF>::T (&r)[HcPieces<CI>::N], const HcTile &t, int h, int wd, float *patch)
+template <int CI, bool BF, bool BN = false>
+__device__ __forceinline__ void hc_put(const typename HcRaw<CI, BF>::T (&r)[HcPieces<CI>::N], const HcTile &t, int h, int wd, float *patch,
+                                       const float *tab = nullptr, int relu = 0)
 {
     constexpr int LPP = CI / 4;
 #pragma unroll
@@ -67,20 +88,23 @@
         float4 v;
         if constexpr (BF) v = make_float4(pcacc_bf16_lo(r[q].x), pcacc_bf16_hi(r[q].x), pcacc_bf16_lo(r[q].y), pcacc_bf16_hi(r[q].y));
         else v = r[q];
+        if constexpr (BN) v = hc_bn4<CI>(v, tab, l4, relu);
         if (!ok) v = make_float4(0.f, 0.f, 0.f, 0.f);
         *reinterpret_cast<float4 *>(patch + pp * CI + l4 * 4) = v;
     }
 }
 
-template <int CI, int COM, bool BF>
+template <int CI, int COM, bool BF, bool BN = false>
 __global__ __launch_bounds__(HC_THREADS) void head_conv_fwd_kernel(const void *__restrict__ x, int x_bf16, const float *__restrict__ w,
                                                                    const float *__restrict__ bias, float *__restrict__ y, int n_img, int h,
                                                                    int wd, int co, int64_t ws_o, int64_t ws_i, int64_t ws_y, int64_t ws_x,
-                                                                   int tiles_y, int tiles_x)
+                                                                   int tiles_y, int tiles_x, HcBn bn)
 {
     constexpr int LPP = CI / 4, PPB = HC_THREADS / LPP;
     extern __shared__ __attribute__((aligned(16))) float hc_lds[];
     float *patch = hc_lds;
+    float *tab = hc_lds + HC_PH * HC_PW * CI;
+    if constexpr (BN) hc_bn_table<CI>(bn, tab);
     const int l = threadIdx.x % LPP, slot = threadIdx.x / LPP;
     float4 wr[9][COM];
 #pragma unroll
@@ -97,7 +121,7 @@
     for (int t = blockIdx.x; t < n_tiles; t += gridDim.x) {
         const HcTile tl = hc_tile(t, tiles_y, tiles_x);
         __syncthreads();
-        if constexpr (PIPE) hc_put<CI, BF>(raw, tl, h, wd, patch); else hc_stage<CI>(x, x_bf16, tl, h, wd, patch);
+        if constexpr (PIPE) hc_put<CI, BF, BN>(raw, tl, h, wd, patch, tab, bn.relu); else hc_stage<CI, BN>(x, x_bf16, tl, h, wd, patch, tab, bn.relu);
         __syncthreads();
         if (PIPE && t + (int)gridDim.x < n_tiles) hc_fetch<CI, BF>(x, hc_tile(t + gridDim.x, tiles_y, tiles_x), h, wd, raw);
         for (int q = slot; q < HC_TR * HC_TC; q += PPB) {
@@ -174,14 +198,16 @@
     }
 }
 
-template <int CI, int COM, bool BF>
+template <int CI, int COM, bool BF, bool BN = false>
 __global__ __launch_bounds__(HC_THREADS) void head_conv_wgrad_kernel(const float *__restrict__ dy, const void *__restrict__ x, int x_bf16,
                                                                      float *__restrict__ partial, int n_img, int h, int wd, int co, int tiles_y,
-                                                                     int tiles_x)
+                                                                     int tiles_x, HcBn bn)
 {
     constexpr int LPP = CI / 4, PPB = HC_THREADS / LPP;
     extern __shared__ __attribute__((aligned(16))) float hc_lds[];
     float *patch = hc_lds;
+    float *tab = hc_lds + HC_PH * HC_PW * CI;
+    if constexpr (BN) hc_bn_table<CI>(bn, tab);
     constexpr int RED = 9 * COM * 4 + COM;
     static_assert(4 * LPP * RED <= HC_PH * HC_PW * CI, "reduction scratch fits the patch");
     const int l = threadIdx.x % LPP, slot = threadIdx.x / LPP, wave = threadIdx.x >> 6;
@@ -201,7 +227,7 @@
     for (int t = blockIdx.x; t < n_tiles; t += gridDim.x) {
         const HcTile tl = hc_tile(t, tiles_y, tiles_x);
         __syncthreads();
-        if constexpr (PIPE) hc_put<CI, BF>(raw, tl, h, wd, patch); else hc_stage<CI>(x, x_bf16, tl, h, wd, patch);
+        if constexpr (PIPE) hc_put<CI, BF, BN>(raw, tl, h, wd, patch, tab, bn.relu); else hc_stage<CI, BN>(x, x_bf16, tl, h, wd, patch, tab, bn.relu);
         __syncthreads();
         if (PIPE && t + (int)gridDim.x < n_tiles) hc_fetch<CI, BF>(x, hc_tile(t + gridDim.x, tiles_y, tiles_x), h, wd, raw);
         auto dy_at = [&](int q) {
@@ -312,26 +338,43 @@
 
 extern "C" int pcacc_head_conv3x3_supported(int32_t c_in, int32_t c_out) { return hc_ok(1, 1, 1, c_in, c_out) ? 1 : 0; }
 
-extern "C" int pcacc_head_conv3x3_forward(const void *x, int32_t x_dtype, const float *w, const int64_t *w_strides, const float *bias, float *y,
-                                          int32_t n_img, int32_t h, int32_t wd, int32_t c_in, int32_t c_out, void *stream)
+static int hc_forward(const void *x, int32_t x_dtype, const float *w, const int64_t *w_strides, const float *bias, float *y, int32_t n_img, int32_t h,
+                      int32_t wd, int32_t c_in, int32_t c_out, void *stream, const HcBn *bn)
 {
     if (!x || !w || !w_strides || !y || !hc_ok(n_img, h, wd, c_in, c_out)) return PCACC_E_ARG;
+    if (bn && (x_dtype || !bn->mean || !bn->invstd)) return PCACC_E_ARG;
+    const HcBn bnv = bn ? *bn : HcBn{nullptr, nullptr, nullptr, nullptr, 0};
     const int tiles_y = (h + HC_TR - 1) / HC_TR, tiles_x = (wd + HC_TC - 1) / HC_TC;
     const int64_t n_tiles = (int64_t)n_img * tiles_y * tiles_x;
     const int grid = (int)(n_tiles < PCACC_CUS * 6 ? n_tiles : PCACC_CUS * 6);
 #define HC_FWD(CIV, COV)                                                                                                                        \
     do {                                                                                                                                        \
-        const size_t lds = (size_t)(HC_PH * HC_PW * CIV) * sizeof(float);                                                       \
-        auto kern = x_dtype ? head_conv_fwd_kernel<CIV, COV, true> : head_conv_fwd_kernel<CIV, COV, false>;                                     \
+        const size_t lds = (size_t)(HC_PH * HC_PW * CIV + (bn ? 2 * CIV : 0)) * sizeof(float);                                                 \
+        auto kern = bn ? head_conv_fwd_kernel<CIV, COV, false, true>                                                                            \
+                       : x_dtype ? head_conv_fwd_kernel<CIV, COV, true> : head_conv_fwd_kernel<CIV, COV, false>;                                \
         if (hipFuncSetAttribute(reinterpret_cast<const void *>(kern), hipFuncAttributeMaxDynamicSharedMemorySize, (int)lds) != hipSuccess)     \
             return PCACC_E_LAUNCH;                                                                                                              \
         hipLaunchKernelGGL(kern, dim3(grid), dim3(HC_THREADS), lds, pcacc_stream(stream), x, x_dtype, w, bias, y, n_img, h, wd, c_out, w_strides[0], \
-                           w_strides[1], w_strides[2], w_strides[3], tiles_y, tiles_x);                                                         \
+                           w_strides[1], w_strides[2], w_strides[3], tiles_y, tiles_x, bnv);                                                    \
     } while (0)
     if (c_in == 32 && c_out <= 2) HC_FWD(32, 2); else if (c_in == 32) HC_FWD(32, 4); else if (c_out <= 2) HC_FWD(64, 2); else HC_FWD(64, 4);
 #undef HC_FWD
     PCACC_CHECK_LAUNCH();
     return PCACC_OK;
+}
+
+extern "C" int pcacc_head_conv3x3_forward(const void *x, int32_t x_dtype, const float *w, const int64_t *w_strides, const float *bias, float *y,
+                                          int32_t n_img, int32_t h, int32_t wd, int32_t c_in, int32_t c_out, void *stream)
+{
+    return hc_forward(x, x_dtype, w, w_strides, bias, y, n_img, h, wd, c_in, c_out, stream, nullptr);
+}
+
+extern "C" int pcacc_head_conv3x3_forward_bn(const float *x, const float *mean, const float *invstd, const float *gamma, const float *beta, int32_t relu,
+                                             const float *w, const int64_t *w_strides, const float *bias, float *y, int32_t n_img, int32_t h, int32_t wd,
+                                             int32_t c_in, int32_t c_out, void *stream)
+{
+    const HcBn bn{mean, invstd, gamma, beta, relu != 0};
+    return hc_forward(x, 0, w, w_strides, bias, y, n_img, h, wd, c_in, c_out, stream, &bn);
 }
 
 extern "C" int pcacc_head_conv3x3_dgrad(const float *dy, const float *w, const int64_t *w_strides, void *dx, int32_t dx_dtype, int32_t n_img, int32_t h,
@@ -362,11 +405,13 @@
     return PCACC_OK;
 }
 
-extern "C" int pcacc_head_conv3x3_wgrad(const float *dy, const void *x, int32_t x_dtype, float *dw, float *db, int32_t n_img, int32_t h, int32_t wd,
-                                        int32_t c_in, int32_t c_out, void *workspace, size_t workspace_bytes, void *stream)
+static int hc_wgrad(const float *dy, const void *x, int32_t x_dtype, float *dw, float *db, int32_t n_img, int32_t h, int32_t wd, int32_t c_in,
+                    int32_t c_out, void *workspace, size_t workspace_bytes, void *stream, const HcBn *bn)
 {
     size_t need;
     if (!dy || !x || !dw || !workspace || pcacc_head_conv3x3_wgrad_workspace_bytes(n_img, h, wd, c_in, c_out, &need) != PCACC_OK) return PCACC_E_ARG;
+    if (bn && (x_dtype || !bn->mean || !bn->invstd)) return PCACC_E_ARG;
+    const HcBn bnv = bn ? *bn : HcBn{nullptr, nullptr, nullptr, nullptr, 0};
     if (workspace_bytes < need) return PCACC_E_WORKSPACE;
     hipStream_t st = pcacc_stream(stream);
     const int grid = hc_wgrad_grid(n_img, h, wd);
@@ -374,11 +419,12 @@
     float *partial = static_cast<float *>(workspace);
 #define HC_WG(CIV, COV)                                                                                                                         \
     do {                                                                                                                                        \
-        const size_t lds = (size_t)(HC_PH * HC_PW * CIV) * sizeof(float);                                                                       \
-        auto kern = x_dtype ? head_conv_wgrad_kernel<CIV, COV, true> : head_conv_wgrad_kernel<CIV, COV, false>;                                 \
+        const size_t lds = (size_t)(HC_PH * HC_PW * CIV + (bn ? 2 * CIV : 0)) * sizeof(float);                                                 \
+        auto kern = bn ? head_conv_wgrad_kernel<CIV, COV, false, true>                                                                          \
+                       : x_dtype ? head_conv_wgrad_kernel<CIV, COV, true> : head_conv_wgrad_kernel<CIV, COV, false>;                            \
         if (hipFuncSetAttribute(reinterpret_cast<const void *>(kern), hipFuncAttributeMaxDynamicSharedMemorySize, (int)lds) != hipSuccess)     \
             return PCACC_E_LAUNCH;                                                                                                              \
-        hipLaunchKernelGGL(kern, dim3(grid), dim3(HC_THREADS), lds, st, dy, x, x_dtype, partial, n_img, h, wd, c_out, tiles_y, tiles_x);        \
+        hipLaunchKernelGGL(kern, dim3(grid), dim3(HC_THREADS), lds, st, dy, x, x_dtype, partial, n_img, h, wd, c_out, tiles_y, tiles_x, bnv);   \
     } while (0)
     if (c_in == 32 && c_out <= 2) HC_WG(32, 2); else if (c_in == 32) HC_WG(32, 4); else if (c_out <= 2) HC_WG(64, 2); else HC_WG(64, 4);
 #undef HC_WG
@@ -387,3 +433,17 @@
     PCACC_CHECK_LAUNCH();
     return PCACC_OK;
 }
+
+extern "C" int pcacc_head_conv3x3_wgrad(const float *dy, const void *x, int32_t x_dtype, float *dw, float *db, int32_t n_img, int32_t h, int32_t wd,
+                                        int32_t c_in, int32_t c_out, void *workspace, size_t workspace_bytes, void *stream)
+{
+    return hc_wgrad(dy, x, x_dtype, dw, db, n_img, h, wd, c_in, c_out, workspace, workspace_bytes, stream, nullptr);
+}
+
+extern "C" int pcacc_head_conv3x3_wgrad_bn(const float *dy, const float *x, const float *mean, const float *invstd, const float *gamma, const float *beta,
+                                           int32_t relu, float *dw, float *db, int32_t n_img, int32_t h, int32_t wd, int32_t c_in, int32_t c_out,
+                                           void *workspace, size_t workspace_bytes, void *stream)
+{
+    const HcBn bn{mean, invstd, gamma, beta, relu != 0};
+    return hc_wgrad(dy, x, 0, dw, db, n_img, h, wd, c_in, c_out, workspace, workspace_bytes, stream, &bn);
+}
diff --git a/pcaccumulation_amd/native.py b/pcaccumulation_amd/native.py
--- a/pcaccumulation_amd/native.py
+++ b/pcaccumulation_amd/native.py
@@ -372,6 +372,14 @@
     out = torch.empty(tuple(a.shape[:-1]) + (ca + cb,), dtype=a.dtype, device=a.device)
     _check(lib().pcacc_cat2_rows(_dev(a, None, 'a'), int(ca * a.element_size()), _dev(b, None, 'b'), int(cb * b.element_size()), rows, _dev(out),
                                  _stream()), 'cat2_rows')
+    return out
+
+
+def gather_rows_bn(src, idx, bn):
+    out = torch.empty((idx.shape[0], src.shape[1]), dtype=torch.float32, device=src.device)
+    mean, invstd, gamma, beta, relu = _bn_ptrs(bn)
+    _check(lib().pcacc_gather_rows_bn(_dev(src, torch.float32, 'src'), int(src.shape[1]), _dev(idx, torch.int32, 'idx'), idx.shape[0], mean, invstd, gamma, beta,
+                                      relu, _dev(out), _stream()), 'gather_rows_bn')
     return out
 
 
@@ -1055,6 +1063,37 @@
     return dw, db
 
 
+def _bn_ptrs(bn):
+    mean, invstd, gamma, beta, relu = bn
+    return (_dev(mean, torch.float32, 'mean'), _dev(invstd, torch.float32, 'invstd'), _opt(gamma, torch.float32, 'gamma'), _opt(beta, torch.float32, 'beta'),
+            1 if relu else 0)
+
+
+def head_conv3x3_forward_bn(x_rows, bn, weight, bias):
+    n, h, w, c_in = x_rows.shape
+    c_out = weight.shape[0]
+    y = torch.empty((n, h, w, c_out), dtype=torch.float32, device=x_rows.device)
+    strides = (ctypes.c_int64 * 4)(*weight.stride())
+    mean, invstd, gamma, beta, relu = _bn_ptrs(bn)
+    _check(lib().pcacc_head_conv3x3_forward_bn(_dev(x_rows, torch.float32, 'x'), mean, invstd, gamma, beta, relu, ctypes.c_void_p(weight.data_ptr()), strides,
+                                               _opt(bias, torch.float32, 'bias'), _dev(y), int(n), int(h), int(w), int(c_in), int(c_out), _stream()),
+           'head_conv3x3_forward_bn')
+    return y
+
+
+def head_conv3x3_wgrad_bn(dy_rows, x_rows, bn, want_bias=True):
+    n, h, w, c_out = dy_rows.shape
+    c_in = x_rows.shape[3]
+    dw = torch.empty((c_out, c_in, 3, 3), dtype=torch.float32, device=dy_rows.device)
+    db = torch.empty((c_out,), dtype=torch.float32, device=dy_rows.device) if want_bias else None
+    ws = _workspace(lib().pcacc_head_conv3x3_wgrad_workspace_bytes, dy_rows.device, int(n), int(h), int(w), int(c_in), int(c_out))
+    mean, invstd, gamma, beta, relu = _bn_ptrs(bn)
+    _check(lib().pcacc_head_conv3x3_wgrad_bn(_dev(dy_rows, torch.float32, 'dy'), _dev(x_rows, torch.float32, 'x'), mean, invstd, gamma, beta, relu, _dev(dw),
+                                             _dev(db) if db is not None else None, int(n), int(h), int(w), int(c_in), int(c_out), _dev(ws),
+                                             ws.numel(), _stream()), 'head_conv3x3_wgrad_bn')
+    return dw, db
+
+
 def rows_split_supported(k, n):
     return k in (32, 64, 128) and n in (32, 64, 128)
 
@@ -1379,6 +1418,25 @@
                                             _opt(running_var, torch.float32, 'running_var'), 1 if relu else 0, _dev(y), _dev(y16), _dev(am), _dev(mean),
                                             _dev(invstd), _dev(ws), ws.numel(), _stream()), 'bn_rows_forward_dual')
     return y, y16, am, mean, invstd
+
+
+def bn_rows_stats(x, eps, momentum, running_mean, running_var):
+    rows, c = x.shape
+    mean = torch.empty((c,), dtype=torch.float32, device=x.device)
+    invstd = torch.empty((c,), dtype=torch.float32, device=x.device)
+    ws = _bn_ws(rows, c, x.device)
+    _check(lib().pcacc_bn_rows_stats(_dev(x, torch.float32, 'x'), rows, int(c), eps, momentum, _opt(running_mean, torch.float32, 'running_mean'),
+                                     _opt(running_var, torch.float32, 'running_var'), _dev(mean), _dev(invstd), _dev(ws), ws.numel(), _stream()),
+           'bn_rows_stats')
+    return mean, invstd
+
+
+def bn_rows_apply(x, bn):
+    rows, c = x.shape
+    y = torch.empty_like(x)
+    mean, invstd, gamma, beta, relu = _bn_ptrs(bn)
+    _check(lib().pcacc_bn_rows_apply(_dev(x, torch.float32, 'x'), rows, int(c), mean, invstd, gamma, beta, relu, _dev(y), _stream()), 'bn_rows_apply')
+    return y
 
 
 def bn_rows_backward(grad_y, x, gamma, save_mean, save_invstd, relu_beta=None, relu=False, want_amax=False):
diff --git a/pcaccumulation_amd/ops.py b/pcaccumulation_amd/ops.py
--- a/pcaccumulation_amd/ops.py
+++ b/pcaccumulation_amd/ops.py
@@ -1520,22 +1520,35 @@
 class _HeadConv3x3(torch.autograd.Function):
 
     @staticmethod
-    def forward(ctx, x_rows, weight, bias):
-        ctx.save_for_backward(x_rows, weight)
+    def forward(ctx, x_rows, weight, bias, gamma=None, beta=None, stats=None):
         ctx.has_bias = bias is not None
-        return native.head_conv3x3_forward(twin_or_self(x_rows), weight.detach(), bias.detach() if bias is not None else None)
+        ctx.stats = stats
+        if stats is None:
+            ctx.save_for_backward(x_rows, weight)
+            return native.head_conv3x3_forward(twin_or_self(x_rows), weight.detach(), bias.detach() if bias is not None else None)
+        ctx.save_for_backward(x_rows, weight, gamma, beta)
+        return native.head_conv3x3_forward_bn(x_rows, _bn_on_load(stats, gamma, beta), weight.detach(), bias.detach() if bias is not None else None)
 
     @staticmethod
     def backward(ctx, gy):
-        x_rows, weight = ctx.saved_tensors
+        x_rows, weight = ctx.saved_tensors[:2]
         gy = gy.contiguous().float()
-        gx = gw = gb = None
+        gx = gw = gb = gg = gbeta = None
+        if ctx.stats is not None:
+            gamma, beta = ctx.saved_tensors[2:]
+            bn = _bn_on_load(ctx.stats, gamma, beta)
+            if ctx.needs_input_grad[1] or (ctx.has_bias and ctx.needs_input_grad[2]):
+                gw, gb = native.head_conv3x3_wgrad_bn(gy, x_rows, bn, want_bias=ctx.has_bias)
+                gw = gw.to(weight.dtype)
+            if ctx.needs_input_grad[0] or ctx.needs_input_grad[3] or ctx.needs_input_grad[4]:
+                gx, gg, gbeta = _bn_on_load_backward(native.head_conv3x3_dgrad(gy, weight.detach(), x_rows.shape[3], x_rows.dtype), x_rows, bn)
+            return gx, gw, gb, gg, gbeta, None
         if ctx.needs_input_grad[0]:
             gx = native.head_conv3x3_dgrad(gy, weight.detach(), x_rows.shape[3], x_rows.dtype)
         if ctx.needs_input_grad[1] or (ctx.has_bias and ctx.needs_input_grad[2]):
             gw, gb = native.head_conv3x3_wgrad(gy, x_rows, want_bias=ctx.has_bias)
             gw = gw.to(weight.dtype)
-        return gx, gw, gb
+        return gx, gw, gb, None, None, None
 
 
 def head_conv3x3_available(x, conv):
@@ -1603,8 +1616,12 @@
 
 
 def conv3x3(x, conv, relu=False, premasked=False, input_relu=False):
+    if isinstance(x, NormalisedMap):
+        if not relu and head_conv3x3_available(x.x, conv):
+            return _HeadConv3x3.apply(x.x_rows, conv.weight, conv.bias, x.gamma, x.beta, x.stats).permute(0, 3, 1, 2)
+        x = x.tensor()
     if not relu and head_conv3x3_available(x, conv):
-        return _HeadConv3x3.apply(x.permute(0, 2, 3, 1), conv.weight, conv.bias).permute(0, 3, 1, 2)
+        return _HeadConv3x3.apply(x.permute(0, 2, 3, 1), conv.weight, conv.bias, None, None, None).permute(0, 3, 1, 2)
     mode = conv3x3_native(x, conv)
     if mode:
         xr = x.permute(0, 2, 3, 1)
@@ -1658,7 +1675,7 @@
 class _SparseConv3x3(torch.autograd.Function):
 
     @staticmethod
-    def forward(ctx, h_rows, weight, bias, cells):
+    def forward(ctx, h_rows, weight, bias, cells, gamma=None, beta=None, stats=None):
         n, H, W, C = h_rows.shape
         cells = cells.reshape(-1).long()
         x, y, img = cells % W, (cells // W) % H, cells // (W * H)
@@ -1666,20 +1683,27 @@
         yy, xx = (y[:, None, None] + d[None, :, None]).expand(-1, 3, 3), (x[:, None, None] + d[None, None, :]).expand(-1, 3, 3)
         ok = (yy >= 0) & (yy < H) & (xx >= 0) & (xx < W)
         idx = torch.where(ok, (img[:, None, None] * H + yy) * W + xx, torch.full_like(yy, -1)).reshape(-1).to(torch.int32)
-        patches = native.gather_rows(h_rows.reshape(-1, C), idx).view(-1, 9 * C)
+        if stats is None:
+            patches = native.gather_rows(h_rows.reshape(-1, C), idx).view(-1, 9 * C)
+        else:
+            patches = native.gather_rows_bn(h_rows.reshape(-1, C), idx, _bn_on_load(stats, gamma, beta)).view(-1, 9 * C)
         w2 = weight.detach().float().permute(2, 3, 1, 0).reshape(9 * C, -1)
         out = torch.addmm(bias.detach().float(), patches, w2) if bias is not None else patches @ w2
-        ctx.save_for_backward(patches, w2, idx)
+        ctx.stats = stats
+        if stats is None:
+            ctx.save_for_backward(patches, w2, idx)
+        else:
+            ctx.save_for_backward(patches, w2, idx, h_rows, gamma, beta)
         ctx.meta = (tuple(h_rows.shape), tuple(weight.shape), bias is not None)
         return out
 
     @staticmethod
     def backward(ctx, g):
-        patches, w2, idx = ctx.saved_tensors
+        patches, w2, idx = ctx.saved_tensors[:3]
         (n, H, W, C), wshape, has_bias = ctx.meta
         g = g.contiguous().float()
-        gh = gw = gb = None
-        if ctx.needs_input_grad[0]:
+        gh = gw = gb = gg = gbeta = None
+        if ctx.needs_input_grad[0] or (ctx.stats is not None and (ctx.needs_input_grad[4] or ctx.needs_input_grad[5])):
             gp = (g @ w2.t()).view(-1, C)
             cells = n * H * W
             if DETERMINISTIC and C % 4 == 0:
@@ -1699,7 +1723,10 @@
             gw = gw2.view(3, 3, wshape[1], wshape[0]).permute(3, 2, 0, 1).contiguous()
         if has_bias and ctx.needs_input_grad[2]:
             gb = g.sum(0)
-        return gh, gw, gb, None
+        if ctx.stats is not None and gh is not None:
+            x_rows, gamma, beta = ctx.saved_tensors[3:]
+            gh, gg, gbeta = _bn_on_load_backward(gh.contiguous(), x_rows, _bn_on_load(ctx.stats, gamma, beta))
+        return gh, gw, gb, None, gg, gbeta, None
 
 
 class SparseConvRows(object):
@@ -1709,8 +1736,11 @@
         self.is_cuda, self.device = h.is_cuda, h.device
 
     def at(self, cells):
+        if isinstance(self.h, NormalisedMap):
+            out = _SparseConv3x3.apply(self.h.x_rows, self.conv.weight, self.conv.bias, cells, self.h.gamma, self.h.beta, self.h.stats)
+            return out.view(tuple(cells.shape) + (out.shape[-1],))
         rows = self.h.permute(0, 2, 3, 1)
-        out = _SparseConv3x3.apply(rows if rows.is_contiguous() else rows.contiguous(), self.conv.weight, self.conv.bias, cells)
+        out = _SparseConv3x3.apply(rows if rows.is_contiguous() else rows.contiguous(), self.conv.weight, self.conv.bias, cells, None, None, None)
         return out.view(tuple(cells.shape) + (out.shape[-1],))
 
     def dense(self):
@@ -1999,3 +2029,66 @@
     rm, rv = (bn.running_mean, bn.running_var) if bn.track_running_stats else (None, None)
     y = _BatchNormRows.apply(rows, bn.weight, bn.bias, float(bn.eps), float(bn.momentum), rm, rv, relu)
     return y.view(n, h, w, c).permute(0, 3, 1, 2)
+
+
+def _bn_on_load(stats, gamma, beta):
+    mean, invstd, relu = stats
+    return (mean, invstd, gamma.detach() if gamma is not None else None, beta.detach() if beta is not None else None, relu)
+
+
+def _bn_on_load_backward(gh, x_rows, bn):
+    mean, invstd, gamma, beta, relu = bn
+    c = x_rows.shape[-1]
+    x2, g2 = x_rows.reshape(-1, c), gh.reshape(-1, c)
+    if _SPLIT:
+        gx, gg, gb, am = native.bn_rows_backward(g2, x2, gamma, mean, invstd, relu_beta=beta if relu else None, relu=relu, want_amax=True)
+        set_amax_tag(gx, am)
+    else:
+        gx, gg, gb = native.bn_rows_backward(g2, x2, gamma, mean, invstd, relu_beta=beta if relu else None, relu=relu)
+    return gx.view(x_rows.shape), (gg if gamma is not None else None), (gb if gamma is not None else None)
+
+
+class _BnMaterialise(torch.autograd.Function):
+
+    @staticmethod
+    def forward(ctx, x_rows, gamma, beta, stats):
+        ctx.stats = stats
+        ctx.save_for_backward(x_rows, gamma, beta)
+        return native.bn_rows_apply(x_rows.reshape(-1, x_rows.shape[-1]), _bn_on_load(stats, gamma, beta)).view(x_rows.shape)
+
+    @staticmethod
+    def backward(ctx, gy):
+        x_rows, gamma, beta = ctx.saved_tensors
+        gx, gg, gb = _bn_on_load_backward(gy.contiguous().float(), x_rows, _bn_on_load(ctx.stats, gamma, beta))
+        return gx, gg, gb, None
+
+
+class NormalisedMap(object):
+
+    def __init__(self, x, bn, relu):
+        self.x, self.x_rows = x, x.permute(0, 2, 3, 1)
+        n, h, w, c = self.x_rows.shape
+        self.gamma, self.beta = bn.weight, bn.bias
+        self.shape, self.dtype, self.device, self.is_cuda = x.shape, x.dtype, x.device, x.is_cuda
+        if bn.track_running_stats and bn.num_batches_tracked is not None:
+            bn.num_batches_tracked.add_(1)
+        rm, rv = (bn.running_mean, bn.running_var) if bn.track_running_stats else (None, None)
+        mean, invstd = native.bn_rows_stats(self.x_rows.detach().reshape(n * h * w, c), float(bn.eps), float(bn.momentum), rm, rv)
+        self.stats = (mean, invstd, bool(relu))
+
+    def dim(self):
+        return 4
+
+    def tensor(self):
+        return _BnMaterialise.apply(self.x_rows, self.gamma, self.beta, self.stats).permute(0, 3, 1, 2)
+
+
+def normalised_map(x, bn, relu=False):
+    if not (bn.training and x.is_cuda and x.dim() == 4 and bn.momentum is not None and x.dtype == torch.float32 and not torch.is_autocast_enabled()
+            and (bn.weight is None or bn.weight.dtype == torch.float32) and os.environ.get('PCACC_BN_ON_LOAD', '1') != '0'):
+        return None
+    rows = x.permute(0, 2, 3, 1)
+    n, h, w, c = rows.shape
+    if not rows.is_contiguous() or not native.bn_rows_supported(rows.reshape(n * h * w, c)) or n * h * w < MIN_ROWS_FUSED_LINEAR:
+        return None
+    return NormalisedMap(x, bn, relu)
diff --git a/pcaccumulation_amd/unet.py b/pcaccumulation_amd/unet.py
--- a/pcaccumulation_amd/unet.py
+++ b/pcaccumulation_amd/unet.py
@@ -127,16 +127,20 @@
     def forward(self, feats):
         conv0, bn, act, conv1 = self.seg_head
         fused = isinstance(act, nn.ReLU)
-        h = self.hidden(feats)
+        h = self.hidden(feats, lazy=True)
         return ops.conv3x3(h, conv1)
 
-    def hidden(self, feats):
+    def hidden(self, feats, lazy=False):
         conv0, bn, act, conv1 = self.seg_head
         fused = isinstance(act, nn.ReLU)
-        h = ops.batch_norm_nchw(ops.exit_mixed(ops.conv3x3(feats, conv0)), bn, relu=fused)
+        y = ops.exit_mixed(ops.conv3x3(feats, conv0))
+        h = ops.normalised_map(y, bn, relu=True) if lazy and fused else None
+        if h is not None:
+            return h
+        h = ops.batch_norm_nchw(y, bn, relu=fused)
         return h if fused else act(h)
 
     def sparse_rows(self, feats):
-        h = self.hidden(feats)
+        h = self.hidden(feats, lazy=True)
         conv1 = self.seg_head[3]
         return ops.SparseConvRows(h, conv1) if ops.sparse_conv_available(h, conv1) else ops.nchw_as_rows(ops.exit_mixed(ops.conv3x3(h, conv1)))
```
